# matter-labs/era-zkevm_test_harness

Measured on AMD Instinct MI355X. Metric: base-layer circuits/sec (2^20 rows); full-block synth wall-time 1/8 GPU, higher is better.
Workload: dtype u64 (Goldilocks, p = 2^64 - 2^32 + 1)

## Files before the change

### era_zkevm_test_harness_amd/csrc/ram_circuit_kernels.cuh

```cuda
#pragma once
#include "../../include/zkw_ram_circuit_spec.h"
#include "../../include/zkw_decommit_sorter_circuit_spec.h"
#include "../../include/zkw_events_sorter_circuit_spec.h"
#include "ram_kernels.cuh"
#include "public_input_kernels.cuh"
#include "closed_form_kernels.cuh"

namespace zkw {

struct SynthJob {
    const zkw_ram_instance* inst;
    const zkw_mem_query* sorted_q;
    const zkw_mem_query* unsorted_q;
    const u64* unsorted_caps;
    const u64* sorted_caps;
    const u64* u_mark;
    const u64* s_mark;
    const u64* challenges;
    const u64* gp_ckpt;
    u64* trace;
    u32* hist;
    u32* nd_tiles;
    const u64* public_input;
    const zkw_ram_instance* first_inst;
    u32 tail_clean;
};

constexpr int ROW_SLOTS[RC_NUM_ROW_TYPES] = RC_ROW_NUM_SLOTS_INIT;
constexpr int ROW_LOOKUPS[RC_NUM_ROW_TYPES] = RC_ROW_NUM_LOOKUPS_INIT;
static_assert(ROW_SLOTS[RC_ROW_PU] == 133 && ROW_SLOTS[RC_ROW_PS] == 130, "Poseidon2 rows: 130 gate variables (+3 spare in PU)");
static_assert(ROW_LOOKUPS[RC_ROW_PU] == 12 && ROW_LOOKUPS[RC_ROW_PS] == 12 && ROW_LOOKUPS[RC_ROW_A] == 12 &&
              ROW_LOOKUPS[RC_ROW_B] == 12 && ROW_LOOKUPS[RC_ROW_C] == 8 && ROW_LOOKUPS[RC_ROW_D] == 0,
              "lookup cells per cycle (56) are hard-wired in the fill kernels");
constexpr int LOOKUPS_PER_CYCLE = 56;

__device__ __forceinline__ u64 inv_or_zero(u64 x) { return gl::canon(x) ? gl::inv(x) : 0; }

struct RegsIn {
    const u64* uh;
    const u64* sh;
    u32 len;
};
__device__ __forceinline__ RegsIn regs_in(const zkw_ram_instance* in) {
    RegsIn r;
    const bool start = in->start_flag != 0;
    r.uh = start ? in->unsorted_queue_initial_state.head : in->hidden_fsm_input.current_unsorted_queue_state.head;
    r.sh = start ? in->sorted_queue_initial_state.head : in->hidden_fsm_input.current_sorted_queue_state.head;
    r.len = start ? in->unsorted_queue_initial_state.length : in->hidden_fsm_input.current_unsorted_queue_state.length;
    return r;
}

#define TR(col, row) trace[(size_t)(col) * n_rows + (row)]

__device__ __forceinline__ void zero_gap_row(u64* trace, size_t n_rows, size_t row) {
    for (int col = 0; col < RC_G + RC_L; col++) TR(col, row) = 0;
}
__device__ __forceinline__ void zero_gap_row_n(u64* trace, size_t n_rows, size_t row, int n_cols) {
    for (int col = 0; col < n_cols; col++) TR(col, row) = 0;
}

__device__ __forceinline__ void hist_bytes(u32* sh_hist, u32 x) {
    atomicAdd(&sh_hist[x & 0xFF], 1u);
    atomicAdd(&sh_hist[(x >> 8) & 0xFF], 1u);
    atomicAdd(&sh_hist[(x >> 16) & 0xFF], 1u);
    atomicAdd(&sh_hist[x >> 24], 1u);
}
__device__ __forceinline__ void put_bytes(u64* trace, size_t n_rows, size_t row, int col0, u32 x) {
    TR(col0, row) = x & 0xFF;
    TR(col0 + 1, row) = (x >> 8) & 0xFF;
    TR(col0 + 2, row) = (x >> 16) & 0xFF;
    TR(col0 + 3, row) = x >> 24;
}
__device__ __forceinline__ void hist_flush(u32* sh_hist, u32* g_hist) {
    __syncthreads();
    for (int t = threadIdx.x; t < 256; t += blockDim.x)
        if (sh_hist[t]) atomicAdd(&g_hist[t], sh_hist[t]);
}

__device__ __forceinline__ void fill_flattened_poseidon(u64* trace, size_t n_rows, size_t row, u64 s[12]) {
    int pos = 0;
#pragma unroll
    for (int k = 0; k < 12; k++) TR(pos++, row) = gl::canon(s[k]);
    p2::external(s);
    int r = 0;
    for (int k = 0; k < P2_HALF_FULL_ROUNDS; k++, r++) {
        p2::full_round(s, r);
#pragma unroll
        for (int j = 0; j < 12; j++) TR(pos + j, row) = gl::canon(s[j]);
        pos += 12;
    }
    for (int k = 0; k < P2_PARTIAL_ROUNDS; k++, r++) {
        s[0] = gl::pow7(gl::add_canon(s[0], p2::rc_at(12 * r)));
        TR(pos++, row) = gl::canon(s[0]);
        p2::internal(s);
    }
    for (int k = 0; k < P2_HALF_FULL_ROUNDS; k++, r++) {
        p2::full_round(s, r);
#pragma unroll
        for (int j = 0; j < 12; j++) TR(pos + j, row) = gl::canon(s[j]);
        pos += 12;
    }
}

struct CycleCtx {
    bool can_pop;
    zkw_mem_query q, pq;
    u64 es[8];
    u64 p_val[5];
    u32 p_ptr;
};

__device__ __forceinline__ void load_query(const zkw_mem_query* src, zkw_mem_query& dst) {
    const uint4* s = reinterpret_cast<const uint4*>(src);
    uint4* d = reinterpret_cast<uint4*>(&dst);
    d[0] = s[0]; d[1] = s[1]; d[2] = s[2];
}

__device__ __forceinline__ void cycle_ctx(const SynthJob& job, u32 i, CycleCtx& c) {
    const zkw_ram_instance* in = job.inst;
    const size_t first = in->first_item, m = in->num_items;
    c.can_pop = i < m;
    memset(&c.q, 0, sizeof c.q);
    memset(&c.pq, 0, sizeof c.pq);
#pragma unroll
    for (int k = 0; k < 8; k++) c.es[k] = 0;
    if (c.can_pop) {
        load_query(job.sorted_q + first + i, c.q);
        encode_mem_query(c.q, c.es);
    }
    if (i == 0) {
        const zkw_ram_fsm& f = in->hidden_fsm_input;
        c.pq.timestamp = f.previous_sorting_key[0]; c.pq.index = f.previous_sorting_key[1]; c.pq.page = f.previous_sorting_key[2];
        for (int k = 0; k < 8; k++) c.pq.value[k] = f.previous_value[k];
        c.pq.value_is_pointer = f.previous_is_ptr ? 1 : 0;
    } else if (i - 1 < m) {
        load_query(job.sorted_q + first + i - 1, c.pq);
    }
    u64 pe[8];
    encode_mem_query(c.pq, pe);
#pragma unroll
    for (int k = 0; k < 5; k++) c.p_val[k] = pe[3 + k];
    c.p_ptr = c.pq.value_is_pointer ? 1 : 0;
}

__device__ __forceinline__ void acc_before_pair(u64 fl, u64 fr, u64 ckpt_l, u64 ckpt_r, int lane, u64& pl, u64& pr) {
#pragma unroll
    for (int d = 1; d < 64; d <<= 1) {
        const u64 ol = __shfl_up(fl, d, 64), orr = __shfl_up(fr, d, 64);
        if (lane >= d) { fl = gl::mul(fl, ol); fr = gl::mul(fr, orr); }
        __builtin_amdgcn_sched_barrier(0);
    }
    const u64 el = __shfl_up(fl, 1, 64), er = __shfl_up(fr, 1, 64);
    pl = lane == 0 ? ckpt_l : gl::canon(gl::mul(ckpt_l, el));
    pr = lane == 0 ? ckpt_r : gl::canon(gl::mul(ckpt_r, er));
    __builtin_amdgcn_sched_barrier(0);
}

__device__ __forceinline__ void fill_row_A(const SynthJob& job, u32 i, u32 capacity, size_t n_rows, const zkw_mem_query& q,
                                           const u64 eu[8], const u64 es[8], u32* sh_hist) {
    u64* trace = job.trace;
    const size_t row = (size_t)RC_ROW_A * RC_REGION_STRIDE(capacity) + i;
    const bool live = i < capacity;
    const bool can_pop = live && i < job.inst->num_items;
    const int lane = threadIdx.x & 63;
    const u64* ckpt = job.gp_ckpt + 4 * (size_t)((u32)__builtin_amdgcn_readfirstlane((int)i) >> 6);
    if (live) {
#pragma unroll
        for (int k = 0; k < 8; k++) { TR(RC_A_eu0 + k, row) = eu[k]; TR(RC_A_ts + k, row) = es[k]; }
    }
    for (int r = 0; r < 2; r++) {
        const u64* ch = job.challenges + 9 * r;
        u64 lc = ch[8], rc = ch[8];
#pragma unroll
        for (int k = 0; k < 8; k++) {
            lc = gl::add(lc, gl::mul(eu[k], ch[k]));
            rc = gl::add(rc, gl::mul(es[k], ch[k]));
            __builtin_amdgcn_sched_barrier(0);
        }
        u64 pl, pr;
        acc_before_pair(can_pop ? lc : 1, can_pop ? rc : 1, ckpt[r], ckpt[2 + r], lane, pl, pr);
        if (live) {
            const u64 nl = gl::canon(gl::mul(pl, lc)), nr = gl::canon(gl::mul(pr, rc));
            const int o = r * (RC_A_lc1 - RC_A_lc0);
#pragma unroll
            for (int k = 1; k < 9; k++) TR(RC_A_G_c0_1 + (k - 1) + r * (RC_A_G_c1_1 - RC_A_G_c0_1), row) = ch[k];
            __builtin_amdgcn_sched_barrier(0);
            TR(RC_A_lc0 + o, row) = gl::canon(lc); TR(RC_A_P_lhs0 + o, row) = pl; TR(RC_A_nl0 + o, row) = nl;
            TR(RC_A_lhs0 + o, row) = can_pop ? nl : pl;
            TR(RC_A_rc0 + o, row) = gl::canon(rc); TR(RC_A_P_rhs0 + o, row) = pr; TR(RC_A_nr0 + o, row) = nr;
            TR(RC_A_rhs0 + o, row) = can_pop ? nr : pr;
        }
        __builtin_amdgcn_sched_barrier(0);
    }
    if (live) {
        const u64 rw = q.rw_flag ? 1 : 0, ptr = q.value_is_pointer ? 1 : 0;
        TR(RC_A_rw, row) = rw; TR(RC_A_ptr, row) = ptr; TR(RC_A_idx, row) = q.index;
        TR(RC_A_v2, row) = q.value[2]; TR(RC_A_v3, row) = q.value[3]; TR(RC_A_v0, row) = q.value[0];
        TR(RC_A_v5_b3c, row) = q.value[5] >> 24; TR(RC_A_can_pop, row) = can_pop ? 1 : 0;
        put_bytes(trace, n_rows, row, RC_A_v2_b0, q.value[2]);
        put_bytes(trace, n_rows, row, RC_A_v3_b0, q.value[3]);
        put_bytes(trace, n_rows, row, RC_A_v5_b0, q.value[5]);
        hist_bytes(sh_hist, q.value[2]); hist_bytes(sh_hist, q.value[3]); hist_bytes(sh_hist, q.value[5]);
        constexpr int NA = ROW_SLOTS[RC_ROW_A];
        if (!job.tail_clean) {
            for (int col = NA; col < RC_G; col++) TR(col, row) = 0;
            for (int col = RC_G + 12; col < RC_G + RC_L; col++) TR(col, row) = 0;
        }
    } else if (i < RC_REGION_STRIDE(capacity)) {
        if (!job.tail_clean) zero_gap_row(trace, n_rows, row);
    }
}

__device__ __forceinline__ void fill_row_B(const SynthJob& job, u32 i, u32 capacity, size_t n_rows, const zkw_mem_query& q,
                                           const u64 es[8], u32* sh_hist) {
    u64* trace = job.trace;
    const size_t row = (size_t)RC_ROW_B * RC_REGION_STRIDE(capacity) + i;
    if (i < capacity) {
        const zkw_ram_instance* in = job.inst;
        u32 p_ts = 0;
        if (i == 0) p_ts = in->hidden_fsm_input.previous_sorting_key[0];
        else if (i - 1 < in->num_items) p_ts = job.sorted_q[in->first_item + i - 1].timestamp;
        put_bytes(trace, n_rows, row, RC_B_v6_b0, q.value[6]);
        put_bytes(trace, n_rows, row, RC_B_v7_b0, q.value[7]);
        TR(RC_B_es4, row) = es[4]; TR(RC_B_v1, row) = q.value[1]; TR(RC_B_v5_b3c, row) = q.value[5] >> 24;
        TR(RC_B_es5, row) = es[5]; TR(RC_B_v2, row) = q.value[2];
        TR(RC_B_es6, row) = es[6]; TR(RC_B_v3, row) = q.value[3];
        const u32 d0 = q.timestamp - p_ts;
        TR(RC_B_d0, row) = d0; put_bytes(trace, n_rows, row, RC_B_d0_b0, d0);
        TR(RC_B_bw0, row) = q.timestamp < p_ts ? 1 : 0;
        TR(RC_B_ts, row) = q.timestamp; TR(RC_B_P_ts, row) = p_ts;
        hist_bytes(sh_hist, q.value[6]); hist_bytes(sh_hist, q.value[7]); hist_bytes(sh_hist, d0);
        constexpr int NB = ROW_SLOTS[RC_ROW_B];
        if (!job.tail_clean) {
            for (int col = NB; col < RC_G; col++) TR(col, row) = 0;
            for (int col = RC_G + 12; col < RC_G + RC_L; col++) TR(col, row) = 0;
        }
    } else if (i < RC_REGION_STRIDE(capacity)) {
        if (!job.tail_clean) zero_gap_row(trace, n_rows, row);
    }
}

template <int SIDE>
static __device__ __forceinline__ void k_ram_fill_poseidon(const VB& vb, const SynthJob* __restrict__ jobs, u32 capacity,
                                                          size_t n_rows) {
    __shared__ u32 sh_hist[256];
    for (int t = threadIdx.x; t < 256; t += blockDim.x) sh_hist[t] = 0;
    __syncthreads();
    const SynthJob job = jobs[vb.y];
    const u32 i = vb.x * blockDim.x + threadIdx.x;
    u64* trace = job.trace;
    const zkw_ram_instance* in = job.inst;
    const size_t first = in->first_item, m = in->num_items;
    const bool can_pop = i < capacity && i < m;
    const size_t row = (size_t)(SIDE == 0 ? RC_ROW_PU : RC_ROW_PS) * RC_REGION_STRIDE(capacity) + i;
    zkw_mem_query q;
    memset(&q, 0, sizeof q);
    u64 s[12];
#pragma unroll
    for (int k = 0; k < 8; k++) s[k] = 0;
    if (can_pop) {
        load_query(job.sorted_q + first + i, q);
        if (SIDE == 0) encode_raw_query(load_raw_query(job.unsorted_q + first + i), s); else encode_mem_query(q, s);
    }
    if (SIDE == 0) {
        u64 es[8];
        encode_mem_query(q, es);
        fill_row_A(job, i, capacity, n_rows, q, s, es, sh_hist);
    } else {
        fill_row_B(job, i, capacity, n_rows, q, s, sh_hist);
    }
    if (i < capacity) {
        if (SIDE == 0) {
            TR(RC_PU_idx, row) = q.index; TR(RC_PU_v0, row) = q.value[0]; TR(RC_PU_v1, row) = q.value[1];
            put_bytes(trace, n_rows, row, RC_PU_idx_b0, q.index);
            put_bytes(trace, n_rows, row, RC_PU_v0_b0, q.value[0]);
            put_bytes(trace, n_rows, row, RC_PU_v1_b0, q.value[1]);
            hist_bytes(sh_hist, q.index); hist_bytes(sh_hist, q.value[0]); hist_bytes(sh_hist, q.value[1]);
        } else {
            if (!job.tail_clean) for (int c = 130; c < RC_G; c++) TR(c, row) = 0;
            put_bytes(trace, n_rows, row, RC_PS_ts_b0, q.timestamp);
            put_bytes(trace, n_rows, row, RC_PS_page_b0, q.page);
            put_bytes(trace, n_rows, row, RC_PS_v4_b0, q.value[4]);
            hist_bytes(sh_hist, q.timestamp); hist_bytes(sh_hist, q.page); hist_bytes(sh_hist, q.value[4]);
        }
        if (!job.tail_clean) for (int c = RC_G + 12; c < RC_G + RC_L; c++) TR(c, row) = 0;
        __builtin_amdgcn_sched_barrier(0);
        const RegsIn ri = regs_in(in);
        const u64* caps = SIDE == 0 ? job.unsorted_caps : job.sorted_caps;
        const u64* prev_cap = i == 0 ? (SIDE == 0 ? ri.uh : ri.sh) + 8 : caps + 4 * (first + (i - 1 < m ? i - 1 : m - 1));
#pragma unroll
        for (int k = 0; k < 4; k++) s[8 + k] = prev_cap[k];
        fill_flattened_poseidon(trace, n_rows, row, s);
    } else if (i < RC_REGION_STRIDE(capacity)) {
        if (!job.tail_clean) zero_gap_row(trace, n_rows, row);
    }
    hist_flush(sh_hist, job.hist);
}

__device__ __forceinline__ bool nd_flag(bool can_pop, const zkw_mem_query& q) {
    return can_pop && q.timestamp == 0 && q.page == RC_HEAP_PAGE && q.rw_flag && !q.value_is_pointer;
}

static __device__ __forceinline__ void k_ram_nd_tiles(const VB& vb, const SynthJob* __restrict__ jobs, u32 capacity) {
    __shared__ u32 sh[4];
    const SynthJob job = jobs[vb.y];
    const u32 i = vb.x * blockDim.x + threadIdx.x;
    const zkw_ram_instance* in = job.inst;
    bool f = false;
    if (i < capacity && i < in->num_items) {
        zkw_mem_query q;
        load_query(job.sorted_q + in->first_item + i, q);
        f = nd_flag(true, q);
    }
    u32 cnt = __popcll(__ballot(f));
    if ((threadIdx.x & 63) == 0) sh[threadIdx.x >> 6] = cnt;
    __syncthreads();
    if (threadIdx.x == 0) job.nd_tiles[vb.x] = sh[0] + sh[1] + sh[2] + sh[3];
}
static __device__ __forceinline__ void k_ram_nd_scan(const VB& vb, const SynthJob* __restrict__ jobs, int n_jobs, u32 n_tiles) {
    u32* t = jobs[vb.x].nd_tiles;
    const int lane = threadIdx.x;
    u32 acc = 0;
    for (u32 base = 0; base < n_tiles; base += 64) {
        const u32 k = base + lane;
        const u32 v = k < n_tiles ? t[k] : 0;
        u32 incl = v;
        for (int off = 1; off < 64; off <<= 1) {
            const u32 up = __shfl_up(incl, off);
            if (lane >= off) incl += up;
        }
        if (k < n_tiles) t[k] = acc + incl - v;
        acc += __shfl(incl, 63);
    }
}

static __device__ __forceinline__ void k_ram_fill_C(const VB& vb, const SynthJob* __restrict__ jobs, u32 capacity, size_t n_rows) {
    __shared__ u32 sh_hist[256];
    __shared__ u32 sh_wave[4];
    sh_hist[threadIdx.x] = 0;
    __syncthreads();
    const SynthJob job = jobs[vb.y];
    const u32 i = vb.x * blockDim.x + threadIdx.x;
    const bool live = i < capacity;
    CycleCtx c;
    c.can_pop = false;
    bool nd = false;
    if (live) {
        cycle_ctx(job, i, c);
        nd = nd_flag(c.can_pop, c.q);
    }
    const unsigned long long bal = __ballot(nd);
    const int lane = threadIdx.x & 63, wave = threadIdx.x >> 6;
    if (lane == 0) sh_wave[wave] = __popcll(bal);
    __syncthreads();
    u32 before = __popcll(bal & ((1ull << lane) - 1));
    for (int w = 0; w < wave; w++) before += sh_wave[w];
    if (live) {
        u64* trace = job.trace;
        const zkw_ram_instance* in = job.inst;
        const size_t row = (size_t)RC_ROW_C * RC_REGION_STRIDE(capacity) + i;
        const u64 rw = c.q.rw_flag ? 1 : 0, ptr = c.q.value_is_pointer ? 1 : 0;
        const u64 bw0 = c.q.timestamp < c.pq.timestamp ? 1 : 0;
        const u64 t1 = (u64)c.pq.index + bw0, bw1 = (u64)c.q.index < t1 ? 1 : 0;
        const u32 d1 = (u32)((u64)c.q.index - t1);
        const u64 t2 = (u64)c.pq.page + bw1, bw2 = (u64)c.q.page < t2 ? 1 : 0;
        const u32 d2 = (u32)((u64)c.q.page - t2);
        TR(RC_C_d1, row) = d1; put_bytes(trace, n_rows, row, RC_C_d1_b0, d1);
        TR(RC_C_d2, row) = d2; put_bytes(trace, n_rows, row, RC_C_d2_b0, d2);
        hist_bytes(sh_hist, d1); hist_bytes(sh_hist, d2);
        TR(RC_C_bw1, row) = bw1; TR(RC_C_bw2, row) = bw2; TR(RC_C_bw0, row) = bw0;
        TR(RC_C_idx, row) = c.q.index; TR(RC_C_P_idx, row) = c.pq.index;
        TR(RC_C_page, row) = c.q.page; TR(RC_C_P_page, row) = c.pq.page;
        TR(RC_C_can_pop, row) = c.can_pop ? 1 : 0;
        u64 x[14];
        x[0] = gl::canon(gl::sub(c.q.index, c.pq.index));
        x[1] = gl::canon(gl::sub(c.q.page, c.pq.page));
        const u64 val[5] = {c.es[3], c.es[4], c.es[5], c.es[6], c.es[7]};
#pragma unroll
        for (int k = 0; k < 5; k++) { x[2 + k] = gl::canon(gl::sub(val[k], c.p_val[k])); x[7 + k] = val[k]; }
        x[12] = c.q.timestamp;
        x[13] = gl::canon(gl::sub(c.q.page, RC_HEAP_PAGE));
        u64 pre[14], acc = 1;
#pragma unroll
        for (int k = 0; k < 14; k++) { pre[k] = acc; acc = gl::mul(acc, x[k] ? x[k] : 1); }
        u64 inv = gl::inv(acc), w[14];
#pragma unroll
        for (int k = 13; k >= 0; k--) {
            w[k] = x[k] ? gl::canon(gl::mul(inv, pre[k])) : 0;
            inv = gl::mul(inv, x[k] ? x[k] : 1);
        }
        const u64 z_idx = x[0] == 0, z_page = x[1] == 0, same = z_idx & z_page;
        TR(RC_C_w_idx, row) = w[0]; TR(RC_C_z_idx, row) = z_idx;
        TR(RC_C_w_page, row) = w[1]; TR(RC_C_z_page, row) = z_page; TR(RC_C_same, row) = same;
        const int C_VAL[5] = {RC_C_es3, RC_C_es4, RC_C_es5, RC_C_es6, RC_C_v4};
        const int C_PVAL[5] = {RC_C_P_es3, RC_C_P_es4, RC_C_P_es5, RC_C_P_es6, RC_C_P_v4};
        const int C_WEQ[5] = {RC_C_w_eq0, RC_C_w_eq1, RC_C_w_eq2, RC_C_w_eq3, RC_C_w_eq4};
        const int C_ZEQ[5] = {RC_C_z_eq0, RC_C_z_eq1, RC_C_z_eq2, RC_C_z_eq3, RC_C_z_eq4};
        const int C_WZ[5] = {RC_C_w_z0, RC_C_w_z1, RC_C_w_z2, RC_C_w_z3, RC_C_w_z4};
        const int C_ZZ[5] = {RC_C_z_z0, RC_C_z_z1, RC_C_z_z2, RC_C_z_z3, RC_C_z_z4};
        u64 zeq[5], zz[5];
#pragma unroll
        for (int k = 0; k < 5; k++) {
            zeq[k] = x[2 + k] == 0; zz[k] = x[7 + k] == 0;
            TR(C_VAL[k], row) = val[k]; TR(C_PVAL[k], row) = c.p_val[k];
            TR(C_WEQ[k], row) = w[2 + k]; TR(C_ZEQ[k], row) = zeq[k];
            TR(C_WZ[k], row) = w[7 + k]; TR(C_ZZ[k], row) = zz[k];
        }
        const u64 peq = ptr == c.p_ptr, eq_a = zeq[0] & zeq[1] & zeq[2], value_equal = eq_a & zeq[3] & zeq[4] & peq;
        const u64 zz_a = zz[0] & zz[1] & zz[2], all_zero = zz_a & zz[3] & zz[4] & (1 - ptr);
        TR(RC_C_ptr, row) = ptr; TR(RC_C_P_ptr, row) = c.p_ptr; TR(RC_C_peq, row) = peq;
        TR(RC_C_eq_a, row) = eq_a; TR(RC_C_value_equal, row) = value_equal;
        TR(RC_C_zz_a, row) = zz_a; TR(RC_C_all_zero, row) = all_zero; TR(RC_C_rw, row) = rw;
        TR(RC_C_ts, row) = c.q.timestamp; TR(RC_C_w_ts, row) = w[12]; TR(RC_C_z_ts, row) = x[12] == 0;
        TR(RC_C_w_heap, row) = w[13]; TR(RC_C_z_heap, row) = x[13] == 0; TR(RC_C_nd, row) = nd ? 1 : 0;
        const u64 p_cnt = (u64)in->hidden_fsm_input.num_nondeterministic_writes + job.nd_tiles[vb.x] + before;
        TR(RC_C_P_cnt, row) = p_cnt; TR(RC_C_cnt, row) = p_cnt + (nd ? 1 : 0);
        constexpr int NC = ROW_SLOTS[RC_ROW_C];
        if (!job.tail_clean) {
            for (int col = NC; col < RC_G; col++) TR(col, row) = 0;
            for (int col = RC_G + 8; col < RC_G + RC_L; col++) TR(col, row) = 0;
        }
    } else if (i < RC_REGION_STRIDE(capacity)) {
        if (!job.tail_clean) zero_gap_row(job.trace, n_rows, (size_t)RC_ROW_C * RC_REGION_STRIDE(capacity) + i);
    }
    if (vb.x == 0 && threadIdx.x == 0)
        for (int l = 5; l < 8; l++) { hist_bytes(sh_hist, job.inst->hidden_fsm_input.previous_value[l]); hist_bytes(sh_hist, job.inst->hidden_fsm_output.previous_value[l]); }
    hist_flush(sh_hist, job.hist);
}

__device__ __forceinline__ void ram_boundary_block(const SynthJob& job, u32 capacity, size_t n_rows);
constexpr int RC_D_TILES = 4;
static __device__ __forceinline__ void k_ram_fill_D(const VB& vb, const SynthJob* __restrict__ jobs, u32 n_jobs, u32 n_tiles, u32 capacity, size_t n_rows) {
    if (vb.x < n_jobs) {
        __builtin_amdgcn_s_setprio(3);
        ram_boundary_block(jobs[vb.x], capacity, n_rows);
        return;
    }
    const SynthJob& job = jobs[(vb.x - n_jobs) / n_tiles];
    const u32 i0 = ((vb.x - n_jobs) % n_tiles) * (RC_D_TILES * 256) + threadIdx.x;
    const size_t rs = RC_REGION_STRIDE(capacity);
    u64* trace = job.trace;
    const zkw_ram_instance* in = job.inst;
    const size_t m = in->num_items;
    const RegsIn ri = regs_in(in);
    u64 len[RC_D_TILES], pre[RC_D_TILES], w[RC_D_TILES];
    u64 acc = 1;
#pragma unroll
    for (int k = 0; k < RC_D_TILES; k++) {
        const u32 i = i0 + 256 * k;
        len[k] = (u64)ri.len - (i < m ? i : m);
        pre[k] = acc;
        acc = gl::mul(acc, len[k] ? len[k] : 1);
    }
    acc = gl::inv(acc);
#pragma unroll
    for (int k = RC_D_TILES - 1; k >= 0; k--) {
        w[k] = len[k] ? gl::canon(gl::mul(acc, pre[k])) : 0;
        acc = gl::mul(acc, len[k] ? len[k] : 1);
    }
#pragma unroll
    for (int k = 0; k < RC_D_TILES; k++) {
        const u32 i = i0 + 256 * k;
        if (i >= capacity) {
            if (i < rs && !job.tail_clean) zero_gap_row(job.trace, n_rows, (size_t)RC_ROW_D * rs + i);
            continue;
        }
        const size_t row = (size_t)RC_ROW_D * rs + i;
        const size_t rPU = (size_t)RC_ROW_PU * rs + i, rPS = (size_t)RC_ROW_PS * rs + i;
        const bool can_pop = i < m;
        const u64 p_len = len[k];
        const u64 w_len = w[k], z_len = p_len == 0;
        TR(RC_D_P_len_u, row) = p_len; TR(RC_D_w_lu, row) = w_len; TR(RC_D_z_lu, row) = z_len;
        TR(RC_D_P_len_s, row) = p_len; TR(RC_D_w_ls, row) = w_len; TR(RC_D_z_ls, row) = z_len;
        TR(RC_D_can_pop, row) = can_pop ? 1 : 0;
        TR(RC_D_len_u, row) = p_len - (can_pop ? 1 : 0); TR(RC_D_len_s, row) = p_len - (can_pop ? 1 : 0);
        const size_t p = i - 1 < m ? i - 1 : m - 1, rPUp = (size_t)RC_ROW_PU * rs + p, rPSp = (size_t)RC_ROW_PS * rs + p;
#pragma unroll
        for (int e = 0; e < 12; e++) {
            const u64 uo = TR(RC_PU_uo0 + e, rPU);
            const u64 so = TR(RC_PS_so0 + e, rPS);
            const u64 a = i == 0 ? ri.uh[e] : TR(RC_PU_uo0 + e, rPUp), b = i == 0 ? ri.sh[e] : TR(RC_PS_so0 + e, rPSp);
            const int o = 3 * e;
            TR(RC_D_uo0 + o, row) = uo; TR(RC_D_P_uh0 + o, row) = a; TR(RC_D_uh0 + o, row) = can_pop ? uo : a;
            TR(RC_D_so0 + o, row) = so; TR(RC_D_P_sh0 + o, row) = b; TR(RC_D_sh0 + o, row) = can_pop ? so : b;
        }
        constexpr int ND = ROW_SLOTS[RC_ROW_D];
        if (!job.tail_clean) for (int col = ND; col < RC_G + RC_L; col++) TR(col, row) = 0;
    }
}

constexpr int TAIL_CHUNKS = 8;
constexpr int RC_BOUNDARY_ROWS = RC_NUM_ROW_TYPES - RC_ROWS_PER_CYCLE;
constexpr int RC_CF_LOOKUP_CELLS = 24;
static_assert(RC_BOUNDARY_ROWS % 2 == 0, "the tail's 16-byte stores start below the boundary rows");
static __device__ __forceinline__ void k_ram_fill_tail(const VB& vb, const SynthJob* __restrict__ jobs, u32 capacity, size_t n_rows) {
    constexpr u32 PER_JOB = (RC_G + RC_L + 1) * TAIL_CHUNKS;
    const u32 bid = vb.x % PER_JOB;
    const SynthJob& job = jobs[vb.x / PER_JOB];
    u64* trace = job.trace;
    const int col = bid / TAIL_CHUNKS, ch = bid % TAIL_CHUNKS;
    if (col < RC_G + RC_L) {
        if (job.tail_clean) return;
        const size_t bnd = (size_t)RC_BOUNDARY_ROW(capacity) + RC_BOUNDARY_ROWS;
        const size_t n_pairs = (n_rows - bnd) / 2;
        const size_t per = (n_pairs + TAIL_CHUNKS - 1) / TAIL_CHUNKS, lo = ch * per, hi = lo + per < n_pairs ? lo + per : n_pairs;
        ulonglong2* c2 = reinterpret_cast<ulonglong2*>(trace + (size_t)col * n_rows + bnd);
        const ulonglong2 z = make_ulonglong2(0, 0);
        for (size_t k = lo + threadIdx.x; k < hi; k += 256) c2[k] = z;
        return;
    }
    u64* m = trace + (size_t)RC_MULT_COL * n_rows;
    const size_t per = (n_rows + TAIL_CHUNKS - 1) / TAIL_CHUNKS, lo = ch * per, hi = lo + per < n_rows ? lo + per : n_rows;
    for (size_t r = lo + threadIdx.x; r < (job.tail_clean && hi > 256 ? (lo < 256 ? 256 : lo) : hi); r += 256) {
        u64 v = 0;
        if (r < 256) {
            v = job.hist[r];
            if (r == 0) v += (u64)RC_L * n_rows - (u64)LOOKUPS_PER_CYCLE * capacity - RC_CF_LOOKUP_CELLS;
        }
        m[r] = v;
    }
}

static __constant__ rc_link c_links[RC_NUM_LINKS] = RC_LINKS_INIT;
static __constant__ uint8_t c_is_poseidon[RC_NUM_ROW_TYPES] = RC_ROW_IS_POSEIDON_INIT;
ZKW_CF_TABLES(RC, rc)

__device__ __forceinline__ void ram_fill_register_rows(const SynthJob& job, u32 capacity, size_t n_rows) {
    u64* trace = job.trace;
    const zkw_ram_instance* in = job.inst;
    const zkw_ram_fsm& fi = in->hidden_fsm_input;
    const size_t first = in->first_item, m = in->num_items;
    const size_t bin = (size_t)RC_BOUNDARY_ROW(capacity) + RC_ROWOFF_BND_IN, bout = bin - RC_ROWOFF_BND_IN + RC_ROWOFF_BND_OUT;
    const RegsIn ri = regs_in(in);
    for (int k = 0; k < 12; k++) { TR(RC_BND_IN_uh0 + k, bin) = ri.uh[k]; TR(RC_BND_IN_sh0 + k, bin) = ri.sh[k]; }
    TR(RC_BND_IN_len_u, bin) = ri.len; TR(RC_BND_IN_len_s, bin) = ri.len;
    for (int r = 0; r < 2; r++) { TR(RC_BND_IN_lhs0 + r, bin) = fi.lhs_accumulator[r]; TR(RC_BND_IN_rhs0 + r, bin) = fi.rhs_accumulator[r]; }
    zkw_mem_query pq;
    memset(&pq, 0, sizeof pq);
    for (int k = 0; k < 8; k++) pq.value[k] = fi.previous_value[k];
    u64 pe[8];
    encode_mem_query(pq, pe);
    TR(RC_BND_IN_ts, bin) = fi.previous_sorting_key[0]; TR(RC_BND_IN_idx, bin) = fi.previous_sorting_key[1];
    TR(RC_BND_IN_page, bin) = fi.previous_sorting_key[2];
    TR(RC_BND_IN_es3, bin) = pe[3]; TR(RC_BND_IN_es4, bin) = pe[4]; TR(RC_BND_IN_es5, bin) = pe[5];
    TR(RC_BND_IN_es6, bin) = pe[6]; TR(RC_BND_IN_v4, bin) = pe[7];
    TR(RC_BND_IN_ptr, bin) = fi.previous_is_ptr ? 1 : 0; TR(RC_BND_IN_cnt, bin) = fi.num_nondeterministic_writes;
    for (int r = 0; r < 2; r++)
        for (int k = 1; k < 9; k++) TR(RC_BND_IN_G_c0_1 + 8 * r + (k - 1), bin) = job.challenges[9 * r + k];
    const size_t last = first + m - 1;
    const bool padded = m < capacity;
    const u64 len_out = (u64)ri.len - m;
    for (int k = 0; k < 12; k++) {
        TR(RC_BND_OUT_uh0 + k, bout) = job.u_mark[k];
        TR(RC_BND_OUT_sh0 + k, bout) = job.s_mark[k];
        TR(RC_BND_OUT_tail_u0 + k, bout) = in->unsorted_queue_initial_state.tail[k];
        TR(RC_BND_OUT_tail_s0 + k, bout) = in->sorted_queue_initial_state.tail[k];
    }
    TR(RC_BND_OUT_len_u, bout) = len_out; TR(RC_BND_OUT_len_s, bout) = len_out;
    for (int r = 0; r < 2; r++) {
        TR(RC_BND_OUT_lhs0 + r, bout) = in->hidden_fsm_output.lhs_accumulator[r];
        TR(RC_BND_OUT_rhs0 + r, bout) = in->hidden_fsm_output.rhs_accumulator[r];
    }
    zkw_mem_query lq;
    memset(&lq, 0, sizeof lq);
    if (!padded) lq = job.sorted_q[last];
    u64 le[8];
    encode_mem_query(lq, le);
    TR(RC_BND_OUT_ts, bout) = lq.timestamp; TR(RC_BND_OUT_idx, bout) = lq.index; TR(RC_BND_OUT_page, bout) = lq.page;
    TR(RC_BND_OUT_es3, bout) = le[3]; TR(RC_BND_OUT_es4, bout) = le[4]; TR(RC_BND_OUT_es5, bout) = le[5];
    TR(RC_BND_OUT_es6, bout) = le[6]; TR(RC_BND_OUT_v4, bout) = le[7];
    TR(RC_BND_OUT_ptr, bout) = lq.value_is_pointer ? 1 : 0;
    TR(RC_BND_OUT_cnt, bout) = TR(RC_C_cnt, (size_t)RC_ROW_C * RC_REGION_STRIDE(capacity) + capacity - 1);
    TR(RC_BND_OUT_completion, bout) = in->completion_flag ? 1 : 0;
    TR(RC_BND_OUT_w_end, bout) = inv_or_zero(len_out); TR(RC_BND_OUT_z_end, bout) = len_out == 0;
}

__device__ __forceinline__ void ram_value_row(u64* trace, size_t n_rows, size_t row, int v0, int b0, int e3) {
    zkw_mem_query q;
    memset(&q, 0, sizeof q);
    for (int k = 0; k < 8; k++) q.value[k] = (u32)TR(v0 + k, row);
    for (int l = 5; l < 8; l++)
        for (int k = 0; k < 4; k++) {
            const u64 b = (q.value[l] >> (8 * k)) & 0xFF;
            TR(b0 + 4 * (l - 5) + k, row) = b;
        }
    if (e3 < 0) return;
    u64 e[8];
    encode_mem_query(q, e);
    for (int k = 0; k < 4; k++) TR(e3 + k, row) = e[3 + k];
}

__device__ __forceinline__ void ram_boundary_block(const SynthJob& job, u32 capacity, size_t n_rows) {
    {
        u64* trace = job.trace;
        const size_t bnd = (size_t)RC_BOUNDARY_ROW(capacity);
        for (int k = threadIdx.x; k < (RC_G + RC_L) * RC_BOUNDARY_ROWS; k += CF_THREADS) TR(k / RC_BOUNDARY_ROWS, bnd + k % RC_BOUNDARY_ROWS) = 0;
    }
    __syncthreads();
    __shared__ u64 sh_oi[RAM_INPUT_ENC_LEN], sh_fi[RAM_FSM_ENC_LEN], sh_fo[RAM_FSM_ENC_LEN], sh_flags[2];
    if (threadIdx.x == 0) ram_fill_register_rows(job, capacity, n_rows);
    if (threadIdx.x == 64) {
        int m = put_queue12(job.first_inst->unsorted_queue_initial_state, sh_oi);
        m += put_queue12(job.first_inst->sorted_queue_initial_state, sh_oi + m);
        sh_oi[m] = job.first_inst->non_deterministic_bootloader_memory_snapshot_length;
    }
    if (threadIdx.x == 128) ram_encode_fsm(job.inst->hidden_fsm_input, sh_fi);
    if (threadIdx.x == 192) {
        ram_encode_fsm(job.inst->hidden_fsm_output, sh_fo);
        sh_flags[0] = job.inst->start_flag ? 1 : 0;
        sh_flags[1] = job.inst->completion_flag ? 1 : 0;
    }
    __syncthreads();
    const CfSpec S = ZKW_CF_SPEC(RC, rc, c_is_poseidon);
    const CfSources src = {sh_oi, sh_fi, sh_fo, sh_flags, nullptr};
    u64* trace = job.trace;
    cf_fill_block(S, trace, n_rows, (size_t)RC_BOUNDARY_ROW(capacity), src, [&](int rt, size_t row) {
        if (threadIdx.x != 0) return;
        if (rt == RC_ROW_VIN) ram_value_row(trace, n_rows, row, RC_VIN_VIN_v0, RC_VIN_VIN_v5_b0, RC_VIN_VIN_e3);
        if (rt == RC_ROW_VOUT) ram_value_row(trace, n_rows, row, RC_VOUT_VOUT_v0, RC_VOUT_VOUT_v5_b0, -1);
    });
}

static __constant__ rc_term c_terms[RC_NUM_TERMS] = RC_TERMS_INIT;
static __constant__ rc_constraint c_cons[RC_NUM_CONSTRAINTS] = RC_CONSTRAINTS_INIT;
static __constant__ uint16_t c_row_first[RC_NUM_ROW_TYPES + 1] = RC_ROW_FIRST_CONSTRAINT_INIT;
static __constant__ rc_term c_ds_terms[DS_NUM_TERMS] = DS_TERMS_INIT;
static __constant__ rc_constraint c_ds_cons[DS_NUM_CONSTRAINTS] = DS_CONSTRAINTS_INIT;
static __constant__ uint16_t c_ds_row_first[DS_NUM_ROW_TYPES + 1] = DS_ROW_FIRST_CONSTRAINT_INIT;
static __constant__ uint8_t c_ds_is_poseidon[DS_NUM_ROW_TYPES] = DS_ROW_IS_POSEIDON_INIT;
static __constant__ rc_link c_ds_links[DS_NUM_LINKS] = DS_LINKS_INIT;

struct SpecRam {
    static constexpr int G = RC_G, L = RC_L, ROWS_PER_CYCLE = RC_ROWS_PER_CYCLE, NUM_ROW_TYPES = RC_NUM_ROW_TYPES, NUM_LINKS = RC_NUM_LINKS;
    static constexpr int OFF_BIN = RC_ROWOFF_BND_IN, OFF_BOUT = RC_ROWOFF_BND_OUT;
    __device__ static const rc_term* terms() { return c_terms; }
    __device__ static const rc_constraint* cons() { return c_cons; }
    __device__ static const uint16_t* row_first() { return c_row_first; }
    __device__ static const uint8_t* is_poseidon() { return c_is_poseidon; }
    __device__ static const rc_link* links() { return c_links; }
};
ZKW_CF_TABLES(DS, ds)
struct SpecDecommitSorter {
    static constexpr int G = DS_G, L = DS_L, ROWS_PER_CYCLE = DS_ROWS_PER_CYCLE, NUM_ROW_TYPES = DS_NUM_ROW_TYPES, NUM_LINKS = DS_NUM_LINKS;
    static constexpr int OFF_BIN = DS_ROWOFF_BND_IN, OFF_BOUT = DS_ROWOFF_BND_OUT;
    __device__ static const rc_term* terms() { return c_ds_terms; }
    __device__ static const rc_constraint* cons() { return c_ds_cons; }
    __device__ static const uint16_t* row_first() { return c_ds_row_first; }
    __device__ static const uint8_t* is_poseidon() { return c_ds_is_poseidon; }
    __device__ static const rc_link* links() { return c_ds_links; }
    ZKW_CF_SPEC_MEMBERS(DS, ds)
};
static __constant__ rc_term c_es_terms[ES_NUM_TERMS] = ES_TERMS_INIT;
static __constant__ rc_constraint c_es_cons[ES_NUM_CONSTRAINTS] = ES_CONSTRAINTS_INIT;
static __constant__ uint16_t c_es_row_first[ES_NUM_ROW_TYPES + 1] = ES_ROW_FIRST_CONSTRAINT_INIT;
static __constant__ uint8_t c_es_is_poseidon[ES_NUM_ROW_TYPES] = ES_ROW_IS_POSEIDON_INIT;
static __constant__ rc_link c_es_links[ES_NUM_LINKS] = ES_LINKS_INIT;
ZKW_CF_TABLES(ES, es)
struct SpecEventsSorter {
    static constexpr int G = ES_G, L = ES_L, ROWS_PER_CYCLE = ES_ROWS_PER_CYCLE, NUM_ROW_TYPES = ES_NUM_ROW_TYPES, NUM_LINKS = ES_NUM_LINKS;
    static constexpr int OFF_BIN = ES_ROWOFF_BND_IN, OFF_BOUT = ES_ROWOFF_BND_OUT;
    __device__ static const rc_term* terms() { return c_es_terms; }
    __device__ static const rc_constraint* cons() { return c_es_cons; }
    __device__ static const uint16_t* row_first() { return c_es_row_first; }
    __device__ static const uint8_t* is_poseidon() { return c_es_is_poseidon; }
    __device__ static const rc_link* links() { return c_es_links; }
    ZKW_CF_SPEC_MEMBERS(ES, es)
};

struct CheckResult {
    unsigned long long violations;
    unsigned long long first_bad;
};

// ... 136 lines not shown
```

### era_zkevm_test_harness_amd/csrc/ram_kernels.cuh

```cuda
#pragma once
#include "../../include/zkw_types.h"
#include "poseidon2.cuh"

namespace zkw {
using gl::u32;
using gl::u64;

__device__ __forceinline__ void encode_mem_query(const zkw_mem_query& q, u64 out[8]) {
    const u32* v = q.value;
    out[0] = q.timestamp;
    out[1] = q.page;
    out[2] = (u64)q.index | ((u64)(q.rw_flag ? 1 : 0) << 32) | ((u64)(q.value_is_pointer ? 1 : 0) << 33);
    u64 b5 = v[5], b6 = v[6], b7 = v[7];
    out[3] = (u64)v[0] | ((b5 & 0xFFFFFF) << 32);
    out[4] = (u64)v[1] | ((b5 >> 24) << 32) | ((b6 & 0xFFFF) << 40);
    out[5] = (u64)v[2] | ((b6 >> 16) << 32) | ((b7 & 0xFF) << 48);
    out[6] = (u64)v[3] | ((b7 >> 8) << 32);
    out[7] = v[4];
}

static __device__ __forceinline__ void k_encode_mem(const VB& vb, const zkw_mem_query* __restrict__ q, size_t n,
                                                    u64* __restrict__ enc) {
    size_t i = (size_t)vb.x * blockDim.x + threadIdx.x;
    size_t stride = (size_t)vb.nx * blockDim.x;
// ... 286 lines not shown
    }
    return v;
}

template <int W, int REPS>
static __device__ __forceinline__ void k_gp_local(const VB& vb, const GpSeg* __restrict__ segs,
                                                       const GpTile* __restrict__ tiles,
                                                       u64* __restrict__ tile_aggr ) {
    __shared__ u64 sh_ch[REPS][W + 1];
    __shared__ u64 sh_wave[REPS][GP_BLOCK / 64];
    const GpTile t = tiles[vb.x];
    const GpSeg seg = segs[t.seg];
    const int tid = threadIdx.x, lane = tid & 63, wave = tid >> 6;
    for (int k = tid; k < REPS * (W + 1); k += GP_BLOCK) sh_ch[k / (W + 1)][k % (W + 1)] = seg.chal[k];
    __syncthreads();
    u64 carry[REPS];
#pragma unroll
    for (int r = 0; r < REPS; r++) carry[r] = 1;
    const u64 base = (u64)t.tile * GP_TILE;
    for (int slab = 0; slab < GP_SLABS; slab++) {
        const u64 row = base + (u64)slab * GP_BLOCK + tid;
        const bool live = row < seg.n;
        u64 term[REPS];
#pragma unroll
        for (int r = 0; r < REPS; r++) term[r] = 1;
        if (live) {
            u64 e[W];
            if (W == 8 && seg.rows == nullptr) {
                u64 e8[8];
                encode_raw_query(load_raw_query(seg.mem_q + (seg.perm ? seg.perm[row] : row)), e8);
#pragma unroll
                for (int k = 0; k < (W < 8 ? W : 8); k++) e[k] = e8[k];
            } else {
                const ulonglong2* src = reinterpret_cast<const ulonglong2*>(seg.rows + row * W);
#pragma unroll
                for (int k = 0; k < W / 2; k++) { ulonglong2 w = src[k]; e[2 * k] = w.x; e[2 * k + 1] = w.y; }
            }
#pragma unroll
            for (int r = 0; r < REPS; r++) {
                u64 acc = sh_ch[r][W];
#pragma unroll
                for (int k = 0; k < W; k++) acc = gl::add(acc, gl::mul(e[k], sh_ch[r][k]));
                term[r] = acc;
            }
        }
#pragma unroll
        for (int r = 0; r < REPS; r++) {
            u64 v = wave_scan_mul(term[r], lane);
            if (lane == 63) sh_wave[r][wave] = v;
            __syncthreads();
            u64 pre = carry[r];
            for (int w = 0; w < wave; w++) pre = gl::mul(pre, sh_wave[r][w]);
            v = gl::mul(v, pre);
            if (live) seg.z[(u64)r * seg.n + row] = v;
            u64 tot = carry[r];
            for (int w = 0; w < GP_BLOCK / 64; w++) tot = gl::mul(tot, sh_wave[r][w]);
            carry[r] = tot;
            __syncthreads();
        }
    }
    if (tid == 0) {
#pragma unroll
        for (int r = 0; r < REPS; r++) tile_aggr[(u64)vb.x * REPS + r] = carry[r];
    }
}

template <int REPS>
static __device__ __forceinline__ void k_gp_tiles(const VB& vb, const GpSeg* __restrict__ segs, int n_segs, u64* __restrict__ tile_aggr) {
    int j = vb.x * blockDim.x + threadIdx.x;
    if (j >= n_segs * REPS) return;
    const GpSeg seg = segs[j / REPS];
    const int r = j % REPS;
    u64 acc = 1;
    for (u32 t = 0; t < seg.n_tiles; t++) {
        u64* p = tile_aggr + (u64)(seg.first_tile + t) * REPS + r;
        u64 v = *p;
        *p = acc;
        acc = gl::mul(acc, v);
    }
}

template <int REPS>
static __device__ __forceinline__ void k_gp_apply(const VB& vb, const GpSeg* __restrict__ segs,
                                                       const GpTile* __restrict__ tiles,
                                                       const u64* __restrict__ tile_prefix) {
    const GpTile t = tiles[vb.x];
    const GpSeg seg = segs[t.seg];
    const u64 base = (u64)t.tile * GP_TILE;
#pragma unroll
    for (int r = 0; r < REPS; r++) {
        const u64 pre = tile_prefix[(u64)vb.x * REPS + r];
        u64* z = seg.z + (u64)r * seg.n;
        for (int slab = 0; slab < GP_SLABS; slab++) {
            const u64 row = base + (u64)slab * GP_BLOCK + threadIdx.x;
            if (row < seg.n) z[row] = gl::canon(gl::mul(z[row], pre));
        }
    }
}

static __device__ __forceinline__ void k_ram_sort_keys(const VB& vb, const zkw_mem_query* __restrict__ q, size_t n, u32* __restrict__ ts,
                                u64* __restrict__ cell, u32* __restrict__ iota, const u64* __restrict__ seg_off,
                                int n_segs) {
    size_t i = (size_t)vb.x * blockDim.x + threadIdx.x;
    if (i >= n) return;
    ts[i] = q[i].timestamp;
    cell[i] = ((u64)q[i].page << 32) | q[i].index;
    iota[i] = (u32)i;
    (void)seg_off; (void)n_segs;
}

static __device__ __forceinline__ void k_gather_u32_by_u32(const VB& vb, const u32* __restrict__ src, const u32* __restrict__ idx, size_t n,
                                    u32* __restrict__ dst) {
    size_t i = (size_t)vb.x * blockDim.x + threadIdx.x;
    if (i < n) dst[i] = src[idx[i]];
}

static __device__ __forceinline__ void k_gather_u64_by_u32(const VB& vb, const u64* __restrict__ src, const u32* __restrict__ idx, size_t n,
                                    u64* __restrict__ dst) {
    size_t i = (size_t)vb.x * blockDim.x + threadIdx.x;
    if (i < n) dst[i] = src[idx[i]];
}

static __device__ __forceinline__ void k_gather_encode(const VB& vb, const zkw_mem_query* __restrict__ q,
                                                       const u32* __restrict__ perm, size_t n,
                                                       zkw_mem_query* __restrict__ sorted_q,
                                                       u64* __restrict__ sorted_enc) {
    size_t i = (size_t)vb.x * blockDim.x + threadIdx.x;
    if (i >= n) return;
    const uint4* src = reinterpret_cast<const uint4*>(q + perm[i]);
    uint4 w0 = src[0], w1 = src[1], w2 = src[2];
    uint4* dq = reinterpret_cast<uint4*>(sorted_q + i);
    dq[0] = w0; dq[1] = w1; dq[2] = w2;
    zkw_mem_query m;
    uint4* dm = reinterpret_cast<uint4*>(&m);
    dm[0] = w0; dm[1] = w1; dm[2] = w2;
    if (!sorted_enc) return;
    u64 e[8];
    encode_mem_query(m, e);
    ulonglong2* o = reinterpret_cast<ulonglong2*>(sorted_enc + 8 * i);
    o[0] = make_ulonglong2(e[0], e[1]); o[1] = make_ulonglong2(e[2], e[3]);
    o[2] = make_ulonglong2(e[4], e[5]); o[3] = make_ulonglong2(e[6], e[7]);
}

struct RamBlock {
    const zkw_mem_query* sorted_q;
    const u32* sorted_perm;
    const u64* u_marks;
    const u64* s_marks;
    const u64* lhs_z;
    const u64* rhs_z;
    zkw_ram_instance* instances;
    u32* nondet_prefix;
    u64* gp_ckpt;
    u64 n;
    u32 capacity;
    u32 num_nondet_heap_queries;
};

__device__ __forceinline__ void copy12(u64* dst, const u64* src) {
    for (int k = 0; k < 12; k++) dst[k] = src[k];
}

static __device__ __forceinline__ void k_ram_count_nondet(const VB& vb, const RamBlock* __restrict__ blocks) {
    const RamBlock b = blocks[vb.y];
    const u64 n_inst = (b.n + b.capacity - 1) / b.capacity;
    __shared__ u32 sh[4];
    for (u64 inst = vb.x; inst < n_inst; inst += vb.nx) {
        const u64 lo = inst * b.capacity, hi = lo + b.capacity < b.n ? lo + b.capacity : b.n;
        u32 cnt = 0;
        for (u64 i = lo + threadIdx.x; i < hi; i += blockDim.x) {
            const zkw_mem_query* q = b.sorted_q + b.sorted_perm[i];
            cnt += (q->rw_flag && q->timestamp == 0 && q->page == ZKW_BOOTLOADER_HEAP_PAGE) ? 1u : 0u;
        }
        for (int d = 32; d > 0; d >>= 1) cnt += __shfl_down(cnt, d, 64);
        if ((threadIdx.x & 63) == 0) sh[threadIdx.x >> 6] = cnt;
        __syncthreads();
        if (threadIdx.x == 0) b.nondet_prefix[inst] = sh[0] + sh[1] + sh[2] + sh[3];
        __syncthreads();
    }
}

static __device__ __forceinline__ void k_ram_instances(const VB& vb, const RamBlock* __restrict__ blocks) {
    const RamBlock b = blocks[vb.y];
    const u64 n_inst = (b.n + b.capacity - 1) / b.capacity;
    const u64 idx = (u64)vb.x * blockDim.x + threadIdx.x;
    if (idx >= n_inst) return;
    const u64 n = b.n, lo = idx * b.capacity, hi = lo + b.capacity < n ? lo + b.capacity : n;
    zkw_ram_instance& w = b.instances[idx];
    memset(&w, 0, sizeof w);
    w.start_flag = idx == 0;
    w.completion_flag = idx == n_inst - 1;
    w.first_item = lo;
    w.num_items = hi - lo;
    const u64* u_final = b.u_marks + 12 * (n_inst - 1);
    const u64* s_final = b.s_marks + 12 * (n_inst - 1);
    copy12(w.unsorted_queue_initial_state.tail, u_final);
    w.unsorted_queue_initial_state.length = (u32)n;
    copy12(w.sorted_queue_initial_state.tail, s_final);
    w.sorted_queue_initial_state.length = (u32)n;
    w.non_deterministic_bootloader_memory_snapshot_length = b.num_nondet_heap_queries;

    u32 nondet_before = 0;
    for (u64 k = 0; k < idx; k++) nondet_before += b.nondet_prefix[k];

    auto fill = [&](zkw_ram_fsm& f, u64 end , u32 nondet) {
        const u64 l = end - 1;
        for (int r = 0; r < 2; r++) { f.lhs_accumulator[r] = b.lhs_z[r * n + l]; f.rhs_accumulator[r] = b.rhs_z[r * n + l]; }
        copy12(f.current_unsorted_queue_state.head, b.u_marks + 12 * (l / b.capacity));
        copy12(f.current_unsorted_queue_state.tail, u_final);
        f.current_unsorted_queue_state.length = (u32)(n - end);
        copy12(f.current_sorted_queue_state.head, b.s_marks + 12 * (l / b.capacity));
        copy12(f.current_sorted_queue_state.tail, s_final);
        f.current_sorted_queue_state.length = (u32)(n - end);
        const zkw_mem_query* q = b.sorted_q + b.sorted_perm[l];
        f.previous_sorting_key[0] = q->timestamp; f.previous_sorting_key[1] = q->index; f.previous_sorting_key[2] = q->page;
        f.previous_full_key[0] = q->index; f.previous_full_key[1] = q->page;
        for (int k = 0; k < 8; k++) f.previous_value[k] = q->value[k];
        f.previous_is_ptr = q->value_is_pointer ? 1 : 0;
        f.num_nondeterministic_writes = nondet;
    };
    if (idx == 0) {
        for (int r = 0; r < 2; r++) { w.hidden_fsm_input.lhs_accumulator[r] = 1; w.hidden_fsm_input.rhs_accumulator[r] = 1; }
    } else {
        fill(w.hidden_fsm_input, lo, nondet_before);
    }
    fill(w.hidden_fsm_output, hi, nondet_before + b.nondet_prefix[idx]);
    if ((hi - lo) % b.capacity != 0) {
        zkw_ram_fsm& f = w.hidden_fsm_output;
        for (int k = 0; k < 3; k++) f.previous_sorting_key[k] = 0;
        for (int k = 0; k < 2; k++) f.previous_full_key[k] = 0;
        for (int k = 0; k < 8; k++) f.previous_value[k] = 0;
        f.previous_is_ptr = 0;
    }
}

static __device__ __forceinline__ void k_ram_gp_ckpt(const VB& vb, const RamBlock* __restrict__ blocks) {
    const RamBlock b = blocks[vb.y];
    const u64 n_inst = (b.n + b.capacity - 1) / b.capacity, groups = (b.capacity + 63) / 64;
    const u64 j = (u64)vb.x * blockDim.x + threadIdx.x;
    if (j >= n_inst * groups) return;
    const u64 idx = j / groups, g = j % groups;
    const zkw_ram_instance& in = b.instances[idx];
    const u64 first = in.first_item, m = in.num_items;
    u64* out = b.gp_ckpt + 4 * j;
    for (int r = 0; r < 2; r++) {
        const u64 at = (u64)r * b.n + first + (64 * g - 1 < m ? 64 * g - 1 : m - 1);
        out[r] = g == 0 ? in.hidden_fsm_input.lhs_accumulator[r] : b.lhs_z[at];
        out[2 + r] = g == 0 ? in.hidden_fsm_input.rhs_accumulator[r] : b.rhs_z[at];
    }
}

static __device__ __forceinline__ void k_tails_expand(const VB& vb, const u64* __restrict__ enc, const u64* __restrict__ caps,
                                                     const u64* __restrict__ offsets, int n_queues, size_t n,
                                                     u64* __restrict__ tails) {
    const size_t i = (size_t)vb.x * blockDim.x + threadIdx.x;
    if (i >= n) return;
    int lo = 0, hi = n_queues;
    while (hi - lo > 1) {
        const int mid = (lo + hi) >> 1;
        if (offsets[mid] <= i) lo = mid; else hi = mid;
    }
    u64 s[12];
#pragma unroll
    for (int k = 0; k < 8; k++) s[k] = enc[8 * i + k];
    const bool first = offsets[lo] == i;
#pragma unroll
    for (int k = 0; k < 4; k++) s[8 + k] = first ? 0 : caps[4 * (i - 1) + k];
    p2::permute(s);
#pragma unroll
    for (int k = 0; k < 12; k++) tails[12 * i + k] = gl::canon(s[k]);
}

}
```

### era_zkevm_test_harness_amd/csrc/zkw_api.hip

```cpp
#include "zkw_ctx.h"
#include "circuit_check_host.h"
#include "closed_forms_host.h"
#include "callstack_kernels.cuh"
#include "vm_kernels.cuh"
#include "radix_sort.cuh"

static thread_local std::string g_last_error;

#undef fail
int zkw_fail(int code, const char* fmt, ...) {
    char buf[512];
    va_list ap;
    va_start(ap, fmt);
    vsnprintf(buf, sizeof buf, fmt, ap);
    va_end(ap);
    g_last_error = buf;
    return code;
}

#define fail zkw_fail

struct AllocCache {
    static constexpr size_t SMALL_MAX = size_t(256) << 20;
    static constexpr int MAX_DEV = 16;
// ... 783 lines not shown
                                         uint64_t* tails) {
    uint64_t offsets[2] = {0, n};
    return zkw_queue_push_chain_full_batch(ctx, enc, offsets, 1, tail_in, tails);
}

extern "C" int zkw_fs_challenges(zkw_ctx* ctx, const uint64_t* tail_u, uint32_t len_u, const uint64_t* tail_s,
                                 uint32_t len_s, int state_w, int n_chal, uint64_t* out) {
    if (!ctx || !tail_u || !tail_s || !out) return fail(ZKW_ERR_INVALID, "zkw_fs_challenges: null argument");
    if ((state_w != 4 && state_w != 12) || n_chal < 1 || n_chal > 64)
        return fail(ZKW_ERR_INVALID, "zkw_fs_challenges: state_w must be 4 or 12, 1 <= n_chal <= 64");
    HIP_TRY(hipSetDevice(ctx->device));
    const u64 *d_u = nullptr, *d_s = nullptr;
    u64* d_out = nullptr;
    ZKW_TRY(ctx->in("fs_u", tail_u, (size_t)state_w, &d_u));
    ZKW_TRY(ctx->in("fs_s", tail_s, (size_t)state_w, &d_s));
    ZKW_TRY(ctx->out("fs_out", out, (size_t)2 * n_chal, &d_out));
    std::vector<FsJob> jobs(1);
    jobs[0] = FsJob{d_u, d_s, len_u, len_s, d_out};
    ZKW_TRY(dev_fs(ctx, jobs, state_w, n_chal));
    ZKW_TRY(ctx->finish_out(out, d_out, (size_t)2 * n_chal));
    return ctx->sync_if_host();
}

extern "C" int zkw_grand_product_chains(zkw_ctx* ctx, const uint64_t* lhs, const uint64_t* rhs, size_t n, int width,
                                        const uint64_t* challenges, int n_reps, uint64_t* lhs_z, uint64_t* rhs_z) {
    if (!ctx || !challenges || (n && (!lhs || !rhs || !lhs_z || !rhs_z)))
        return fail(ZKW_ERR_INVALID, "zkw_grand_product_chains: null argument");
    if ((width != 8 && width != 20) || (n_reps != 1 && n_reps != 2))
        return fail(ZKW_ERR_INVALID, "zkw_grand_product_chains: width must be 8 or 20, n_reps 1 or 2");
    HIP_TRY(hipSetDevice(ctx->device));
    if (n == 0) return ZKW_OK;
    const u64 *d_l = nullptr, *d_r = nullptr, *d_c = nullptr;
    u64 *d_lz = nullptr, *d_rz = nullptr;
    ZKW_TRY(ctx->in("gp_lhs", lhs, n * width, &d_l));
    ZKW_TRY(ctx->in("gp_rhs", rhs, n * width, &d_r));
    ZKW_TRY(ctx->in("gp_chal", challenges, (size_t)n_reps * (width + 1), &d_c));
    ZKW_TRY(ctx->out("gp_lz", lhs_z, n * n_reps, &d_lz));
    ZKW_TRY(ctx->out("gp_rz", rhs_z, n * n_reps, &d_rz));
    std::vector<GpSeg> segs(2);
    segs[0] = GpSeg{d_l, d_lz, d_c, n, 0, 0};
    segs[1] = GpSeg{d_r, d_rz, d_c, n, 0, 0};
    ZKW_TRY(dev_grand_products(ctx, segs, width, n_reps));
    ZKW_TRY(ctx->finish_out(lhs_z, d_lz, n * n_reps));
    ZKW_TRY(ctx->finish_out(rhs_z, d_rz, n * n_reps));
    ZKW_TRY(ctx->sync_if_host());
    if (ctx->ptr_mode == ZKW_PTR_HOST)
        for (int r = 0; r < n_reps; r++)
            if (lhs_z[(size_t)r * n + n - 1] != rhs_z[(size_t)r * n + n - 1])
                return fail(ZKW_ERR_CHECK_FAILED, "grand products differ in repetition %d (utils.rs:685-696)", r);
    return ZKW_OK;
}

extern "C" int zkw_encode_log_queries(zkw_ctx* ctx, const zkw_log_query* q, size_t n, const uint32_t* ext_ts,
                                      uint64_t* enc) {
    if (!ctx || (n && (!q || !enc))) return fail(ZKW_ERR_INVALID, "zkw_encode_log_queries: null argument");
    HIP_TRY(hipSetDevice(ctx->device));
    if (n == 0) return ZKW_OK;
    const zkw_log_query* d_q = nullptr;
    const u32* d_e = nullptr;
    u64* d_enc = nullptr;
    ZKW_TRY(ctx->in("lenc_q", q, n, &d_q));
    if (ext_ts) ZKW_TRY(ctx->in("lenc_ts", ext_ts, n, &d_e));
    ZKW_TRY(ctx->out("lenc_out", enc, n * 20, &d_enc));
    { Prof _p(ctx, "k_encode_log"); ZKW_LAUNCH(ctx, k_encode_log, blocks_for(n, 256), 256, d_q, n, d_e, d_enc); }
    ZKW_TRY(launch_check("k_encode_log"));
    ZKW_TRY(ctx->finish_out(enc, d_enc, n * 20));
    return ctx->sync_if_host();
}

extern "C" int zkw_encode_decommit_queries(zkw_ctx* ctx, const zkw_decommit_query* q, size_t n, uint64_t* enc) {
    if (!ctx || (n && (!q || !enc))) return fail(ZKW_ERR_INVALID, "zkw_encode_decommit_queries: null argument");
    HIP_TRY(hipSetDevice(ctx->device));
    if (n == 0) return ZKW_OK;
    const zkw_decommit_query* d_q = nullptr;
    u64* d_enc = nullptr;
    ZKW_TRY(ctx->in("denc_q", q, n, &d_q));
    ZKW_TRY(ctx->out("denc_out", enc, n * 8, &d_enc));
    { Prof _p(ctx, "k_encode_decommit"); ZKW_LAUNCH(ctx, k_encode_decommit, blocks_for(n, 256), 256, d_q, n, d_enc); }
    ZKW_TRY(launch_check("k_encode_decommit"));
    ZKW_TRY(ctx->finish_out(enc, d_enc, n * 8));
    return ctx->sync_if_host();
}

int dev_log_chains(zkw_ctx* ctx, const u64* d_enc, size_t total, std::vector<LogChainJob>& jobs) {
    const int key = ctx->chain_service && !ctx->batched() ? ctx->next_chain_key() : 0;
    if (total == 0 || jobs.empty()) { if (ctx->chain_service && !ctx->batched()) chain_service_of(ctx->device)->skip(key); return ZKW_OK; }
    u64* d_pre = nullptr;
    ZKW_TRY(ctx->scratch_t<u64>("log_pre", total * 4, &d_pre));
    { Prof _p(ctx, "k_log_prehash"); ZKW_LAUNCH(ctx, k_log_prehash, blocks_for(total, 128), 128, d_enc, total, d_pre); }
    ZKW_TRY(launch_check("k_log_prehash"));
    for (auto& j : jobs) j.pre = d_pre + (j.enc - d_enc) / 20 * 4;
    if (ctx->batched()) return zkw_batch_chains(ctx->batch, nullptr, 0, jobs.data(), jobs.size());
    if (ctx->chain_service) return chain_service_run(ctx, nullptr, &jobs, "k_chain_log", key);
    LogChainJob* d_jobs = nullptr;
    ZKW_TRY(ctx->upload("log_chain_jobs", jobs, &d_jobs));
    const int n_jobs = (int)jobs.size();
    { Prof _p(ctx, "k_chain_log"); hipLaunchKernelGGL(k_chain_log, dim3((n_jobs + 3) / 4), dim3(64), 0, ctx->stream, d_jobs, n_jobs); }
    return launch_check("k_chain_log");
}

extern "C" int zkw_queue_push_chain_log_batch(zkw_ctx* ctx, const uint64_t* enc, const uint64_t* offsets,
                                              size_t n_queues, const uint64_t* tails_in, uint64_t* old_tails,
                                              uint64_t* new_tails) {
    if (!ctx || !offsets) return fail(ZKW_ERR_INVALID, "zkw_queue_push_chain_log_batch: null argument");
    HIP_TRY(hipSetDevice(ctx->device));
    for (size_t k = 0; k < n_queues; k++)
        if (offsets[k + 1] < offsets[k]) return fail(ZKW_ERR_INVALID, "offsets must be non-decreasing");
    const size_t base = n_queues ? offsets[0] : 0, total = n_queues ? offsets[n_queues] - base : 0;
    if (total && (!enc || !new_tails)) return fail(ZKW_ERR_INVALID, "null enc/new_tails");
    const u64 *d_enc = nullptr, *d_tin = nullptr;
    u64 *d_old = nullptr, *d_new = nullptr;
    ZKW_TRY(ctx->in("lchain_enc", enc + base * 20, total * 20, &d_enc));
    if (tails_in) ZKW_TRY(ctx->in("lchain_tin", tails_in, n_queues * 4, &d_tin));
    if (old_tails) ZKW_TRY(ctx->out("lchain_old", old_tails + base * 4, total * 4, &d_old));
    ZKW_TRY(ctx->out("lchain_new", new_tails + base * 4, total * 4, &d_new));
    std::vector<LogChainJob> jobs(n_queues);
    for (size_t k = 0; k < n_queues; k++) {
        const size_t lo = offsets[k] - base;
        jobs[k] = LogChainJob{d_enc + lo * 20, nullptr, d_old ? d_old + lo * 4 : nullptr, d_new + lo * 4,
                              d_tin ? d_tin + 4 * k : nullptr, offsets[k + 1] - offsets[k]};
    }
    ZKW_TRY(dev_log_chains(ctx, d_enc, total, jobs));
    if (old_tails) ZKW_TRY(ctx->finish_out(old_tails + base * 4, d_old, total * 4));
    ZKW_TRY(ctx->finish_out(new_tails + base * 4, d_new, total * 4));
    return ctx->sync_if_host();
}

extern "C" int zkw_queue_push_chain_log(zkw_ctx* ctx, const uint64_t* enc, size_t n, const uint64_t tail_in[4],
                                        uint64_t* old_tails, uint64_t* new_tails) {
    uint64_t offsets[2] = {0, n};
    return zkw_queue_push_chain_log_batch(ctx, enc, offsets, 1, tail_in, old_tails, new_tails);
}

struct zkw_ram_witness {
    zkw_ctx* ctx = nullptr;
    std::vector<uint64_t> offsets;
    std::vector<uint64_t> inst_offsets;
    uint32_t capacity = 0;
    size_t total = 0, n_instances = 0;
    zkw_mem_query* sorted_q = nullptr;
    bool sorted_valid = false;
    u32* perm = nullptr;
    const zkw_mem_query* unsorted_q = nullptr;
    zkw_mem_query* owned_q = nullptr;
    u64 *unsorted_enc = nullptr, *sorted_enc = nullptr;
    bool enc_valid = false;
    u64 *unsorted_caps = nullptr, *sorted_caps = nullptr, *unsorted_marks = nullptr, *sorted_marks = nullptr;
    u64 *unsorted_tails = nullptr, *sorted_tails = nullptr;
    bool tails_valid = false;
    u64 *challenges = nullptr, *lhs_z = nullptr, *rhs_z = nullptr;
    bool z_valid = false;
    u64 *zbuf_l = nullptr, *zbuf_r = nullptr;
    u64* gp_ckpt = nullptr;
    zkw_mem_query* sq_win = nullptr;
    size_t zcap = 0, sqcap = 0;
    zkw_ram_instance* instances = nullptr;
    u32* nondet_counts = nullptr;
    u64 *compact_forms = nullptr, *public_inputs = nullptr;

    void release() {
        void* ptrs[] = {sorted_q, perm, owned_q, unsorted_enc, sorted_enc, unsorted_caps, sorted_caps, unsorted_marks, sorted_marks,
                        unsorted_tails, sorted_tails, challenges,
                        lhs_z,    rhs_z,        instances,  nondet_counts, compact_forms, public_inputs, zbuf_l, zbuf_r, sq_win, gp_ckpt};
        for (void* p : ptrs)
            if (p) dev_free(p);
        sorted_q = nullptr;
        sorted_valid = false;
        perm = nullptr;
        owned_q = nullptr;
        unsorted_q = nullptr;
        enc_valid = false;
        unsorted_enc = sorted_enc = unsorted_tails = sorted_tails = challenges = lhs_z = rhs_z = nullptr;
        unsorted_caps = sorted_caps = unsorted_marks = sorted_marks = nullptr;
        tails_valid = false;
        z_valid = false;
        zbuf_l = zbuf_r = nullptr;
        gp_ckpt = nullptr;
        sq_win = nullptr;
        zcap = sqcap = 0;
        instances = nullptr;
        nondet_counts = nullptr;
        compact_forms = public_inputs = nullptr;
    }
};

extern "C" void zkw_ram_witness_free(zkw_ram_witness* w);
static inline size_t ram_gp_groups(uint32_t capacity) { return ((size_t)capacity + 63) / 64; }
static int ram_alloc(zkw_ram_witness* w, size_t n_blocks) {
    const size_t t = w->total, ni = w->n_instances;
    HIP_TRY(dev_malloc((void**)&w->perm, (t + 1) * sizeof(u32)));
    HIP_TRY(dev_malloc((void**)&w->unsorted_caps, (t + 1) * 4 * sizeof(u64)));
    HIP_TRY(dev_malloc((void**)&w->sorted_caps, (t + 1) * 4 * sizeof(u64)));
    HIP_TRY(dev_malloc((void**)&w->unsorted_marks, (ni + 1) * 12 * sizeof(u64)));
    HIP_TRY(dev_malloc((void**)&w->sorted_marks, (ni + 1) * 12 * sizeof(u64)));
    HIP_TRY(dev_malloc((void**)&w->challenges, (n_blocks + 1) * 18 * sizeof(u64)));
    {
        size_t max_block = 0;
        for (size_t b = 0; b + 1 < w->offsets.size(); b++) max_block = std::max(max_block, (size_t)(w->offsets[b + 1] - w->offsets[b]));
        size_t window = (size_t)1 << 26, sq_window = (size_t)1 << 22;
        if (const char* e = getenv("ZKW_Z_WINDOW_ITEMS")) window = sq_window = (size_t)strtoull(e, nullptr, 10);
        w->zcap = std::max(max_block, std::min(t, window));
        w->sqcap = std::max(max_block, std::min(t, sq_window));
        HIP_TRY(dev_malloc((void**)&w->zbuf_l, (w->zcap + 1) * 2 * sizeof(u64)));
        HIP_TRY(dev_malloc((void**)&w->zbuf_r, (w->zcap + 1) * 2 * sizeof(u64)));
        HIP_TRY(dev_malloc((void**)&w->sq_win, (w->sqcap + 1) * sizeof(zkw_mem_query)));
    }
    HIP_TRY(dev_malloc((void**)&w->gp_ckpt, (ni * ram_gp_groups(w->capacity) + 1) * 4 * sizeof(u64)));
    HIP_TRY(dev_malloc((void**)&w->instances, (ni + 1) * sizeof(zkw_ram_instance)));
    HIP_TRY(dev_malloc((void**)&w->nondet_counts, (ni + 1) * sizeof(u32)));
    HIP_TRY(dev_malloc((void**)&w->compact_forms, (ni + 1) * COMPACT_FORM_LEN * sizeof(u64)));
    HIP_TRY(dev_malloc((void**)&w->public_inputs, (ni + 1) * 4 * sizeof(u64)));
    return ZKW_OK;
}

__device__ __forceinline__ u32 block_of_position(const u64* __restrict__ offsets, int n_blocks, size_t i) {
    int lo = 0, hi = n_blocks;
    while (hi - lo > 1) {
        int mid = (lo + hi) >> 1;
        if (offsets[mid] <= i) lo = mid; else hi = mid;
    }
    return (u32)lo;
}

static __device__ __forceinline__ void k_ram_key_ranges(const VB& vb, const zkw_mem_query* __restrict__ q, size_t n, u32* __restrict__ maxima) {
    u32 t = 0, p = 0, x = 0;
    for (size_t i = (size_t)vb.x * blockDim.x + threadIdx.x; i < n; i += (size_t)vb.nx * blockDim.x) {
        t = max(t, q[i].timestamp);
        p = max(p, q[i].page);
        x = max(x, q[i].index);
    }
    for (int o = 32; o > 0; o >>= 1) {
        t = max(t, (u32)__shfl_xor((int)t, o));
        p = max(p, (u32)__shfl_xor((int)p, o));
        x = max(x, (u32)__shfl_xor((int)x, o));
    }
    if ((threadIdx.x & 63) == 0) {
        atomicMax(maxima + 0, t);
        atomicMax(maxima + 1, p);
        atomicMax(maxima + 2, x);
    }
}

static __device__ __forceinline__ void k_ram_packed_keys(const VB& vb, const zkw_mem_query* __restrict__ q, size_t n, const u64* __restrict__ offsets,
                                  int n_blocks, unsigned bits_p, unsigned bits_i, unsigned bits_t,
                                  u64* __restrict__ key, u32* __restrict__ iota) {
    size_t i = (size_t)vb.x * blockDim.x + threadIdx.x;
    if (i >= n) return;
    u64 k = n_blocks > 1 ? block_of_position(offsets, n_blocks, i) : 0;
    k = (k << bits_p) | q[i].page;
    k = (k << bits_i) | q[i].index;
    k = (k << bits_t) | q[i].timestamp;
    key[i] = k;
    iota[i] = (u32)i;
}

static __device__ __forceinline__ void k_ram_packed_cells(const VB& vb, const u64* __restrict__ cell, const u32* __restrict__ perm, size_t n,
                                   const u64* __restrict__ offsets, int n_blocks, unsigned bits_p, unsigned bits_i,
                                   u64* __restrict__ key) {
    size_t i = (size_t)vb.x * blockDim.x + threadIdx.x;
    if (i >= n) return;
    const u32 src = perm[i];
    const u64 c = cell[src];
    u64 k = n_blocks > 1 ? block_of_position(offsets, n_blocks, src) : 0;
    k = (k << bits_p) | (c >> 32);
    k = (k << bits_i) | (c & 0xFFFFFFFFu);
    key[i] = k;
}

static __device__ __forceinline__ void k_block_ids(const VB& vb, const u64* __restrict__ offsets, int n_blocks, size_t n, u32* __restrict__ ids) {
    size_t i = (size_t)vb.x * blockDim.x + threadIdx.x;
    if (i < n) ids[i] = block_of_position(offsets, n_blocks, i);
}

static unsigned bits_in_use(u32 x) { return x ? 32u - (unsigned)__builtin_clz(x) : 0u; }

static int ram_sort(zkw_ctx* ctx, const zkw_mem_query* d_q, size_t total, const std::vector<uint64_t>& offsets,
                    void* work_a, void* work_b, u32** perm_out) {
    const size_t n_blocks = offsets.size() - 1;
    size_t tmp_bytes = radix_temp_bytes(total);
    u32* ts = static_cast<u32*>(work_a);
    u32 *k32 = ts + total, *v0 = k32 + total, *v1 = v0 + total;
    u64* cell = reinterpret_cast<u64*>(v1 + total);
    u64* k64a = cell + total;
    u64* k64b = static_cast<u64*>(work_b);
    void* tmp = nullptr;
    const size_t tmp_off = (total * 8 + 255) & ~(size_t)255;
    if (tmp_off + tmp_bytes <= total * 32) tmp = static_cast<char*>(work_b) + tmp_off;
    else ZKW_TRY(ctx->scratch("sort_tmp", tmp_bytes + 256, &tmp));
    const unsigned grid = blocks_for(total, 256);

    void* d_max_v = nullptr;
    ZKW_TRY(ctx->scratch("sort_max", 256, &d_max_v));
    u32* d_max = static_cast<u32*>(d_max_v);
    HIP_TRY(ctx->memset_async(d_max, 0, 16));
    { Prof _p(ctx, "k_ram_key_ranges");
      const unsigned g = grid < 4096 ? grid : 4096;
      ZKW_LAUNCH(ctx, k_ram_key_ranges, g, 256, d_q, total, d_max); }
    ZKW_TRY(launch_check("k_ram_key_ranges"));
    u32 maxima[4];
    ZKW_TRY(ctx->read_small(maxima, d_max, 16));
    const unsigned bits_t = bits_in_use(maxima[0]), bits_p = bits_in_use(maxima[1]), bits_i = bits_in_use(maxima[2]);
    unsigned bits_b = 0;
    while ((1ull << bits_b) < n_blocks) bits_b++;
    u64* d_off = nullptr;
    if (n_blocks > 1) ZKW_TRY(ctx->upload("sort_off", offsets, &d_off));

    if (bits_b + bits_p + bits_i + bits_t <= 64) {
        const unsigned bits = bits_b + bits_p + bits_i + bits_t;
        { Prof _p(ctx, "k_ram_packed_keys");
          ZKW_LAUNCH(ctx, k_ram_packed_keys, grid, 256, d_q, total, d_off, (int)n_blocks, bits_p, bits_i, bits_t, k64a, v0); }
        ZKW_TRY(launch_check("k_ram_packed_keys"));
        { Prof _p(ctx, "radix_sort"); ZKW_TRY(radix_sort_pairs<u64>(ctx, tmp, tmp_bytes, k64a, k64b, v0, v1, total, bits ? bits : 1)); }
        *perm_out = v1;
        return ZKW_OK;
    }

    { Prof _p(ctx, "k_ram_sort_keys"); ZKW_LAUNCH(ctx, k_ram_sort_keys, grid, 256, d_q, total, ts, cell, v0, (const u64*)nullptr, 0); }
    ZKW_TRY(launch_check("k_ram_sort_keys"));
    { Prof _p(ctx, "radix_sort"); ZKW_TRY(radix_sort_pairs<u32>(ctx, tmp, tmp_bytes, ts, k32, v0, v1, total, bits_t ? bits_t : 1)); }
    if (bits_b + bits_p + bits_i <= 64) {
        const unsigned bits = bits_b + bits_p + bits_i;
        { Prof _p(ctx, "k_ram_packed_cells");
          ZKW_LAUNCH(ctx, k_ram_packed_cells, grid, 256, cell, v1, total, d_off, (int)n_blocks, bits_p, bits_i, k64a); }
        ZKW_TRY(launch_check("k_ram_packed_cells"));
        { Prof _p(ctx, "radix_sort"); ZKW_TRY(radix_sort_pairs<u64>(ctx, tmp, tmp_bytes, k64a, k64b, v1, v0, total, bits ? bits : 1)); }
        *perm_out = v0;
        return ZKW_OK;
    }
    { Prof _p(ctx, "k_gather_u64_by_u32"); ZKW_LAUNCH(ctx, k_gather_u64_by_u32, grid, 256, cell, v1, total, k64a); }
    ZKW_TRY(launch_check("k_gather_u64_by_u32"));
    { Prof _p(ctx, "radix_sort"); ZKW_TRY(radix_sort_pairs<u64>(ctx, tmp, tmp_bytes, k64a, k64b, v1, v0, total, 64)); }
    { Prof _p(ctx, "k_block_ids"); ZKW_LAUNCH(ctx, k_block_ids, grid, 256, d_off, (int)n_blocks, total, ts); }
    ZKW_TRY(launch_check("k_block_ids"));
    { Prof _p(ctx, "k_gather_u32_by_u32"); ZKW_LAUNCH(ctx, k_gather_u32_by_u32, grid, 256, ts, v0, total, k32); }
    ZKW_TRY(launch_check("k_gather_u32_by_u32"));
    { Prof _p(ctx, "radix_sort"); ZKW_TRY(radix_sort_pairs<u32>(ctx, tmp, tmp_bytes, k32, ts, v0, v1, total, bits_b)); }
    *perm_out = v1;
    return ZKW_OK;
}

static int ram_gp_blocks(zkw_ctx* ctx, const zkw_ram_witness* w, size_t b0, size_t b1, u64* dst_l, u64* dst_r) {
    std::vector<GpSeg> segs;
    segs.reserve(2 * (b1 - b0));
    const size_t base = w->offsets[b0];
    for (size_t b = b0; b < b1; b++) {
        const size_t lo = w->offsets[b], n = w->offsets[b + 1] - lo;
        segs.push_back(GpSeg{nullptr, dst_l + 2 * (lo - base), w->challenges + 18 * b, n, 0, 0, w->unsorted_q + lo});
        segs.push_back(GpSeg{nullptr, dst_r + 2 * (lo - base), w->challenges + 18 * b, n, 0, 0, w->unsorted_q, w->perm + lo});
    }
    return dev_grand_products(ctx, segs, 8, 2);
}

static int ram_run(zkw_ctx* ctx, zkw_ram_witness* w, const zkw_mem_query* d_q, const uint32_t* n_nondet) {
    const size_t n_blocks = w->offsets.size() - 1, total = w->total;
    if (ctx->ptr_mode == ZKW_PTR_DEVICE) {
        w->unsorted_q = d_q;
    } else {
        if (!w->owned_q) HIP_TRY(dev_malloc((void**)&w->owned_q, (total + 1) * sizeof(zkw_mem_query)));
        HIP_TRY(ctx->copy_async(w->owned_q, d_q, total * sizeof(zkw_mem_query), hipMemcpyDeviceToDevice));
        w->unsorted_q = w->owned_q;
    }
    u32* perm = nullptr;
    ZKW_TRY(ram_sort(ctx, d_q, total, w->offsets, w->unsorted_caps, w->sorted_caps, &perm));
    w->tails_valid = false;
    w->enc_valid = false;
    w->sorted_valid = false;
    HIP_TRY(ctx->copy_async(w->perm, perm, total * sizeof(u32), hipMemcpyDeviceToDevice));
    std::vector<ChainJob> chains;
    chains.reserve(2 * n_blocks);
    for (size_t b = 0; b < n_blocks; b++) {
        const size_t lo = w->offsets[b], n = w->offsets[b + 1] - lo;
        const size_t io = w->inst_offsets[b];
        chains.push_back(ChainJob{nullptr, nullptr, nullptr, n, w->unsorted_caps + 4 * lo, w->unsorted_marks + 12 * io, w->capacity, w->unsorted_q + lo});
        chains.push_back(ChainJob{nullptr, nullptr, nullptr, n, w->sorted_caps + 4 * lo, w->sorted_marks + 12 * io, w->capacity, w->unsorted_q, w->perm + lo});
    }
    ZKW_TRY(dev_chains(ctx, chains));
    std::vector<FsJob> fs(n_blocks);
    for (size_t b = 0; b < n_blocks; b++) {
        const size_t lo = w->offsets[b], n = w->offsets[b + 1] - lo;
        const size_t last_inst = w->inst_offsets[b + 1] - 1;
        fs[b] = FsJob{w->unsorted_marks + 12 * last_inst, w->sorted_marks + 12 * last_inst, (u32)n, (u32)n,
                      w->challenges + 18 * b};
    }
    ZKW_TRY(dev_fs(ctx, fs, 12, 9));
    w->z_valid = false;
    for (size_t b0 = 0; b0 < n_blocks;) {
        size_t b1 = b0 + 1;
        while (b1 < n_blocks && w->offsets[b1 + 1] - w->offsets[b0] <= w->zcap) b1++;
        ZKW_TRY(ram_gp_blocks(ctx, w, b0, b1, w->zbuf_l, w->zbuf_r));
        const size_t base = w->offsets[b0];
        std::vector<RamBlock> blocks(b1 - b0);
        size_t max_inst = 0;
        for (size_t b = b0; b < b1; b++) {
            const size_t lo = w->offsets[b], n = w->offsets[b + 1] - lo;
            const size_t n_inst = w->inst_offsets[b + 1] - w->inst_offsets[b];
            if (n_inst > max_inst) max_inst = n_inst;
            blocks[b - b0] = RamBlock{w->unsorted_q,
                                      w->perm + lo,
                                      w->unsorted_marks + 12 * w->inst_offsets[b],
                                      w->sorted_marks + 12 * w->inst_offsets[b],
                                      w->zbuf_l + 2 * (lo - base),
                                      w->zbuf_r + 2 * (lo - base),
                                      w->instances + w->inst_offsets[b],
                                      w->nondet_counts + w->inst_offsets[b],
                                      w->gp_ckpt + 4 * ram_gp_groups(w->capacity) * w->inst_offsets[b],
                                      n,
                                      w->capacity,
                                      n_nondet ? n_nondet[b] : 0u};
        }
        RamBlock* d_blocks = nullptr;
        ZKW_TRY(ctx->upload("ram_blocks", blocks, &d_blocks));
        const unsigned gx = (unsigned)(max_inst < 64 ? max_inst : 64), gy = (unsigned)(b1 - b0);
        { Prof _p(ctx, "k_ram_count_nondet"); ZKW_LAUNCH_2D(ctx, k_ram_count_nondet, gx, gy, 256, d_blocks); }
        ZKW_TRY(launch_check("k_ram_count_nondet"));
        { Prof _p(ctx, "k_ram_instances"); ZKW_LAUNCH_2D(ctx, k_ram_instances, blocks_for(max_inst, 64), gy, 64, d_blocks); }
        ZKW_TRY(launch_check("k_ram_instances"));
        { Prof _p(ctx, "k_ram_gp_ckpt"); ZKW_LAUNCH_2D(ctx, k_ram_gp_ckpt, blocks_for(max_inst * ram_gp_groups(w->capacity), 256), gy, 256, d_blocks); }
        ZKW_TRY(launch_check("k_ram_gp_ckpt"));
        b0 = b1;
    }
    const size_t ni = w->n_instances;
    { Prof _p(ctx, "k_ram_commitments"); ZKW_LAUNCH(ctx, k_ram_commitments, blocks_for(4 * ni, 64), 64, w->instances, ni, w->compact_forms); }
    ZKW_TRY(launch_check("k_ram_commitments"));
    { Prof _p(ctx, "k_commit_encodings"); ZKW_LAUNCH(ctx, k_commit_encodings, blocks_for(ni, 64), 64, w->compact_forms, ni, (u32)COMPACT_FORM_LEN, w->public_inputs); }
    return launch_check("k_commit_encodings");
}

extern "C" int zkw_ram_build_instances_batch(zkw_ctx* ctx, const zkw_mem_query* q, const uint64_t* block_offsets,
                                             size_t n_blocks, uint32_t capacity, const uint32_t* n_nondet,
                                             zkw_ram_witness** out) {
    if (!ctx || !q || !block_offsets || !out || n_blocks == 0 || capacity == 0)
        return fail(ZKW_ERR_INVALID, "zkw_ram_build_instances_batch: bad argument");
    HIP_TRY(hipSetDevice(ctx->device));
    const uint64_t base = block_offsets[0];
    std::vector<uint64_t> offs(n_blocks + 1), ioffs(n_blocks + 1, 0);
    for (size_t b = 0; b <= n_blocks; b++) offs[b] = block_offsets[b] - base;
    for (size_t b = 0; b < n_blocks; b++) {
        if (block_offsets[b + 1] <= block_offsets[b])
            return fail(ZKW_ERR_INVALID, "block %zu is empty: the VM must have made memory requests "
                                         "(W/ram_permutation.rs:43-46)", b);
        ioffs[b + 1] = ioffs[b] + (offs[b + 1] - offs[b] + capacity - 1) / capacity;
    }
    const size_t total = offs[n_blocks];
    if (total >= (1ull << 32)) return fail(ZKW_ERR_INVALID, "more than 2^32-1 queries in one batch");
    zkw_ram_witness* w = *out;
    if (w && (w->ctx != ctx || w->offsets != offs || w->capacity != capacity)) {
        zkw_ram_witness_free(w);
        w = nullptr;
        *out = nullptr;
    }
    if (!w) {
        w = new zkw_ram_witness();
        w->ctx = ctx;
        w->offsets = offs;
        w->inst_offsets = ioffs;
        w->capacity = capacity;
        w->total = total;
        w->n_instances = ioffs[n_blocks];
        int rc = ram_alloc(w, n_blocks);
        if (rc != ZKW_OK) {
            w->release();
            delete w;
            return rc;
        }
    }
    const zkw_mem_query* d_q = nullptr;
    int rc = ctx->in("ram_q", q + base, total, &d_q);
    if (rc == ZKW_OK) rc = ram_run(ctx, w, d_q, n_nondet);
    if (rc == ZKW_OK) rc = ctx->sync_if_host();
    if (rc != ZKW_OK) {
        if (!*out) {
            w->release();
            delete w;
        }
        return rc;
    }
    if (!*out) ctx_retain(ctx);
    *out = w;
    return ZKW_OK;
}

extern "C" int zkw_ram_build_instances(zkw_ctx* ctx, const zkw_mem_query* q, size_t n, uint32_t capacity,
                                       uint32_t num_non_deterministic_heap_queries, zkw_ram_witness** out) {
    uint64_t offsets[2] = {0, n};
    return zkw_ram_build_instances_batch(ctx, q, offsets, 1, capacity, &num_non_deterministic_heap_queries, out);
}

extern "C" size_t zkw_ram_witness_num_instances(const zkw_ram_witness* w) { return w ? w->n_instances : 0; }
extern "C" size_t zkw_ram_witness_num_items(const zkw_ram_witness* w) { return w ? w->total : 0; }

static int ram_sorted_queries(const zkw_ram_witness* cw) {
    zkw_ram_witness* w = const_cast<zkw_ram_witness*>(cw);
    if (w->sorted_valid) return ZKW_OK;
    zkw_ctx* ctx = w->ctx;
    HIP_TRY(hipSetDevice(ctx->device));
    const size_t t = w->total;
    if (!w->sorted_q && dev_malloc((void**)&w->sorted_q, (t + 1) * sizeof(zkw_mem_query)) != hipSuccess)
        return fail(ZKW_ERR_OOM, "no room for the sorted queries (%zu bytes): read ZKW_RAM_SORTED_QUERIES from a smaller batch", t * sizeof(zkw_mem_query));
    { Prof _p(ctx, "k_gather_encode"); ZKW_LAUNCH(ctx, k_gather_encode, blocks_for(t, 256), 256, w->unsorted_q, w->perm, t, w->sorted_q, (u64*)nullptr); }
    ZKW_TRY(launch_check("k_gather_encode"));
    w->sorted_valid = true;
    return ZKW_OK;
}

static int ram_full_chains(const zkw_ram_witness* cw) {
    zkw_ram_witness* w = const_cast<zkw_ram_witness*>(cw);
    if (w->z_valid) return ZKW_OK;
    zkw_ctx* ctx = w->ctx;
    HIP_TRY(hipSetDevice(ctx->device));
    const size_t t = w->total;
    if (!w->lhs_z) {
        if (dev_malloc((void**)&w->lhs_z, (t + 1) * 16) != hipSuccess || dev_malloc((void**)&w->rhs_z, (t + 1) * 16) != hipSuccess)
            return fail(ZKW_ERR_OOM, "no room for the grand-product chains (%zu bytes): read ZKW_RAM_*_Z from a smaller batch", 2 * t * 16);
    }
    ZKW_TRY(ram_gp_blocks(ctx, w, 0, w->offsets.size() - 1, w->lhs_z, w->rhs_z));
    w->z_valid = true;
    return ZKW_OK;
}

static int ram_encodings(const zkw_ram_witness* cw) {
    zkw_ram_witness* w = const_cast<zkw_ram_witness*>(cw);
    if (w->enc_valid) return ZKW_OK;
    zkw_ctx* ctx = w->ctx;
    HIP_TRY(hipSetDevice(ctx->device));
    const size_t t = w->total;
    if (!w->unsorted_enc) {
        if (dev_malloc((void**)&w->unsorted_enc, (t + 1) * 64) != hipSuccess || dev_malloc((void**)&w->sorted_enc, (t + 1) * 64) != hipSuccess)
            return fail(ZKW_ERR_OOM, "no room for the materialised encodings (%zu bytes): read ZKW_RAM_*_ENC from a smaller batch", 2 * t * 64);
    }
    ZKW_TRY(ram_sorted_queries(cw));
    ZKW_TRY(dev_encode(ctx, w->unsorted_q, t, w->unsorted_enc));
    ZKW_TRY(dev_encode(ctx, w->sorted_q, t, w->sorted_enc));
    w->enc_valid = true;
    return ZKW_OK;
}

static int ram_full_tails(const zkw_ram_witness* cw) {
    zkw_ram_witness* w = const_cast<zkw_ram_witness*>(cw);
    if (w->tails_valid) return ZKW_OK;
    ZKW_TRY(ram_encodings(cw));
    zkw_ctx* ctx = w->ctx;
    HIP_TRY(hipSetDevice(ctx->device));
    const size_t t = w->total;
    if (!w->unsorted_tails) {
        if (dev_malloc((void**)&w->unsorted_tails, (t + 1) * 96) != hipSuccess || dev_malloc((void**)&w->sorted_tails, (t + 1) * 96) != hipSuccess)
            return fail(ZKW_ERR_OOM, "no room for the expanded queue tails (%zu bytes): read ZKW_RAM_*_TAILS from a smaller batch", 2 * t * 96);
    }
    u64* d_off = nullptr;
    ZKW_TRY(ctx->upload("tails_off", w->offsets, &d_off));
    const int nq = (int)(w->offsets.size() - 1);
    { Prof _p(ctx, "k_tails_expand"); ZKW_LAUNCH(ctx, k_tails_expand, blocks_for(t, 64), 64, w->unsorted_enc, w->unsorted_caps, d_off, nq, t, w->unsorted_tails); }
    ZKW_TRY(launch_check("k_tails_expand"));
    { Prof _p(ctx, "k_tails_expand"); ZKW_LAUNCH(ctx, k_tails_expand, blocks_for(t, 64), 64, w->sorted_enc, w->sorted_caps, d_off, nq, t, w->sorted_tails); }
    ZKW_TRY(launch_check("k_tails_expand"));
    w->tails_valid = true;
    return ZKW_OK;
}

static const void* ram_array(const zkw_ram_witness* w, int what, size_t* bytes, bool materialize = true, int* rc = nullptr) {
    const size_t t = w->total, nb = w->offsets.size() - 1;
    int st = ZKW_OK;
    const void* p = nullptr;
#define RAM_LAZY(fn, field) do { if (materialize) { st = fn(w); if (st == ZKW_OK) p = w->field; } } while (0)
    switch (what) {
        case ZKW_RAM_SORTED_QUERIES: *bytes = t * sizeof(zkw_mem_query); RAM_LAZY(ram_sorted_queries, sorted_q); break;
        case ZKW_RAM_UNSORTED_ENC: *bytes = t * 64; RAM_LAZY(ram_encodings, unsorted_enc); break;
        case ZKW_RAM_SORTED_ENC: *bytes = t * 64; RAM_LAZY(ram_encodings, sorted_enc); break;
        case ZKW_RAM_UNSORTED_TAILS: *bytes = t * 96; RAM_LAZY(ram_full_tails, unsorted_tails); break;
        case ZKW_RAM_SORTED_TAILS: *bytes = t * 96; RAM_LAZY(ram_full_tails, sorted_tails); break;
        case ZKW_RAM_CHALLENGES: *bytes = nb * 18 * 8; p = w->challenges; break;
        case ZKW_RAM_LHS_Z: *bytes = t * 16; RAM_LAZY(ram_full_chains, lhs_z); break;
        case ZKW_RAM_RHS_Z: *bytes = t * 16; RAM_LAZY(ram_full_chains, rhs_z); break;
        case ZKW_RAM_INSTANCES: *bytes = w->n_instances * sizeof(zkw_ram_instance); p = w->instances; break;
        case ZKW_RAM_COMPACT_FORMS: *bytes = w->n_instances * COMPACT_FORM_LEN * 8; p = w->compact_forms; break;
        case ZKW_RAM_PUBLIC_INPUTS: *bytes = w->n_instances * 32; p = w->public_inputs; break;
        case ZKW_RAM_GP_CKPT: *bytes = w->n_instances * ram_gp_groups(w->capacity) * 32; p = w->gp_ckpt; break;
        default: *bytes = 0; st = ZKW_ERR_INVALID; break;
    }
#undef RAM_LAZY
    if (rc) *rc = st;
    return p;
}

extern "C" size_t zkw_ram_witness_bytes(const zkw_ram_witness* w, int what) {
    size_t b = 0;
    if (w) (void)ram_array(w, what, &b, false);
    return b;
}

extern "C" const void* zkw_ram_witness_device_ptr(const zkw_ram_witness* w, int what) {
    size_t b = 0;
    return w ? ram_array(w, what, &b) : nullptr;
}

extern "C" int zkw_ram_witness_get(const zkw_ram_witness* w, int what, void* dst, size_t dst_bytes) {
    if (!w || !dst) return fail(ZKW_ERR_INVALID, "zkw_ram_witness_get: null argument");
    size_t bytes = 0;
    int st = ZKW_OK;
    const void* src = ram_array(w, what, &bytes, true, &st);
    if (st == ZKW_ERR_INVALID) return fail(ZKW_ERR_INVALID, "zkw_ram_witness_get: unknown array %d", what);
    if (st != ZKW_OK) return st;
    if (!src) return fail(ZKW_ERR_INVALID, "zkw_ram_witness_get: array %d is empty", what);
    if (dst_bytes < bytes) return fail(ZKW_ERR_INVALID, "zkw_ram_witness_get: need %zu bytes, got %zu", bytes, dst_bytes);
    zkw_ctx* ctx = w->ctx;
    HIP_TRY(hipSetDevice(ctx->device));
    HIP_TRY(ctx->copy_async(dst, src, bytes, ctx->ptr_mode == ZKW_PTR_DEVICE ? hipMemcpyDeviceToDevice : hipMemcpyDeviceToHost));
    return ctx->sync_if_host();
}

extern "C" void zkw_ram_witness_free(zkw_ram_witness* w) {
    if (!w) return;
    (void)hipSetDevice(w->ctx->device);
    (void)hipStreamSynchronize(w->ctx->stream);
    w->release();
    zkw_ctx* owner = w->ctx;
    delete w;
    ctx_release(owner);
}


extern "C" int zkw_trace_create_with_columns(zkw_ctx* ctx, size_t n_rows, size_t n_cols, size_t n_slots, zkw_trace** out) {
    if (!ctx || !out || n_rows < 256 || n_slots == 0 || n_cols == 0 || n_cols > 4096)
        return fail(ZKW_ERR_INVALID, "zkw_trace_create: bad argument");
    HIP_TRY(hipSetDevice(ctx->device));
    zkw_trace* t = new zkw_trace();
    t->ctx = ctx;
    t->n_rows = n_rows;
    t->n_cols = n_cols;
    t->n_slots = n_slots;
    t->slot_tag.reset(new std::atomic<uint64_t>[n_slots]);
    for (size_t k = 0; k < n_slots; k++) t->slot_tag[k].store(0, std::memory_order_relaxed);
    hipError_t e = dev_malloc((void**)&t->data, t->slot_elems() * n_slots * sizeof(u64));
    if (e != hipSuccess) {
        delete t;
        return fail(ZKW_ERR_OOM, "zkw_trace_create: hipMalloc of %zu bytes failed: %s",
                    n_cols * n_rows * n_slots * 8, hipGetErrorString(e));
    }
    ctx_retain(ctx);
    *out = t;
    return ZKW_OK;
}

extern "C" int zkw_trace_create(zkw_ctx* ctx, size_t n_rows, size_t n_slots, zkw_trace** out) {
    return zkw_trace_create_with_columns(ctx, n_rows, RC_COLS, n_slots, out);
}

extern "C" void zkw_trace_free(zkw_trace* t) {
    if (!t) return;
    (void)hipSetDevice(t->ctx->device);
    (void)hipStreamSynchronize(t->ctx->stream);
    if (t->data) dev_free(t->data);
    zkw_ctx* owner = t->ctx;
    delete t;
    ctx_release(owner);
}

extern "C" size_t zkw_trace_num_rows(const zkw_trace* t) { return t ? t->n_rows : 0; }
extern "C" size_t zkw_trace_num_cols(const zkw_trace* t) { return t ? t->n_cols : 0; }
extern "C" size_t zkw_trace_num_slots(const zkw_trace* t) { return t ? t->n_slots : 0; }
extern "C" const uint64_t* zkw_trace_device_ptr(const zkw_trace* t, size_t slot) {
    if (!t || slot >= t->n_slots) return nullptr;
    return t->slot_for_write(slot, 0);
}

extern "C" int zkw_trace_get(const zkw_trace* t, size_t slot, uint32_t first_col, uint32_t n_cols, uint64_t* dst) {
    if (!t || !dst || slot >= t->n_slots || (size_t)first_col + n_cols > t->n_cols) return fail(ZKW_ERR_INVALID, "zkw_trace_get: bad argument");
    zkw_ctx* ctx = t->ctx;
    HIP_TRY(hipSetDevice(ctx->device));
    const u64* src = t->data + slot * t->slot_elems() + (size_t)first_col * t->n_rows;
    HIP_TRY(ctx->copy_async(dst, src, (size_t)n_cols * t->n_rows * sizeof(u64), ctx->ptr_mode == ZKW_PTR_DEVICE ? hipMemcpyDeviceToDevice : hipMemcpyDeviceToHost));
    return ctx->sync_if_host();
}

extern "C" int zkw_ram_synthesize(zkw_ctx* ctx, const zkw_ram_witness* w, size_t first_instance, size_t n_instances,
                                  zkw_trace* t, size_t first_slot) {
    if (!ctx || !w || !t || w->ctx != ctx || t->ctx->device != ctx->device) return fail(ZKW_ERR_INVALID, "zkw_ram_synthesize: bad argument");
    if (first_instance + n_instances > w->n_instances) return fail(ZKW_ERR_INVALID, "instance range out of bounds");
    if (n_instances > t->n_slots) return fail(ZKW_ERR_INVALID, "more instances (%zu) than trace slots (%zu)", n_instances, t->n_slots);
    const u32 capacity = w->capacity;
    const size_t n_rows = t->n_rows;
    if (RC_MIN_ROWS(capacity) > n_rows)
        return fail(ZKW_ERR_INVALID, "capacity %u needs %llu rows, trace has %zu", capacity,
                    (unsigned long long)RC_MIN_ROWS(capacity), n_rows);
    if (n_rows & 1) return fail(ZKW_ERR_INVALID, "trace length must be even (it is a power of two in every circuit)");
    if (n_instances == 0) return ZKW_OK;
    HIP_TRY(hipSetDevice(ctx->device));
    const size_t n_blocks = w->offsets.size() - 1;
    size_t b_first = 0;
    while (b_first + 1 < n_blocks && w->inst_offsets[b_first + 1] <= first_instance) b_first++;
    size_t b_end = b_first + 1;
    while (b_end < n_blocks && w->inst_offsets[b_end] < first_instance + n_instances) b_end++;
    const size_t win = w->sqcap;
    if (w->offsets[b_end] - w->offsets[b_first] > win) {
        size_t b_mid = b_first + 1;
        while (b_mid + 1 < b_end && w->offsets[b_mid + 1] - w->offsets[b_first] <= win) b_mid++;
        const size_t n_head = w->inst_offsets[b_mid] - first_instance;
        ZKW_TRY(zkw_ram_synthesize(ctx, w, first_instance, n_head, t, first_slot));
        return zkw_ram_synthesize(ctx, w, first_instance + n_head, n_instances - n_head, t, first_slot + n_head);
    }
    const size_t z_base = w->offsets[b_first];
    {
        const size_t cnt = w->offsets[b_end] - z_base;
        Prof _p(ctx, "k_gather_encode");
        ZKW_LAUNCH(ctx, k_gather_encode, blocks_for(cnt, 256), 256, w->unsorted_q, w->perm + z_base, cnt, w->sq_win, (u64*)nullptr);
    }
    ZKW_TRY(launch_check("k_gather_encode"));
    const u32 rstride = (u32)RC_REGION_STRIDE(capacity);
    const u32 n_tiles = (rstride + 255) / 256;
    u32 *d_hist = nullptr, *d_nd = nullptr;
    ZKW_TRY(ctx->scratch_t<u32>("synth_hist", n_instances * 256, &d_hist));
    ZKW_TRY(ctx->scratch_t<u32>("synth_nd", n_instances * n_tiles, &d_nd));
    HIP_TRY(ctx->memset_async(d_hist, 0, n_instances * 256 * sizeof(u32)));
    SlotClaims claims(t);
    std::vector<SynthJob> jobs(n_instances);
    size_t b = b_first;
    for (size_t k = 0; k < n_instances; k++) {
        const size_t idx = first_instance + k;
        while (b + 1 < n_blocks && w->inst_offsets[b + 1] <= idx) b++;
        const size_t lo = w->offsets[b];
        SynthJob& j = jobs[k];
        j.inst = w->instances + idx;
        j.sorted_q = w->sq_win + (lo - z_base);
        j.unsorted_q = w->unsorted_q + lo;
        j.unsorted_caps = w->unsorted_caps + 4 * lo;
        j.sorted_caps = w->sorted_caps + 4 * lo;
        j.u_mark = w->unsorted_marks + 12 * idx;
        j.s_mark = w->sorted_marks + 12 * idx;
        j.challenges = w->challenges + 18 * b;
        j.gp_ckpt = w->gp_ckpt + 4 * ram_gp_groups(capacity) * idx;
        {
            const uint64_t tag = ((uint64_t)ZKW_CIRCUIT_RAM_PERMUTATION << 56) ^ ((uint64_t)capacity << 24) ^ (uint64_t)n_rows ^ 0x5A00000000000000ull;
            const size_t slot = (first_slot + k) % t->n_slots;
            bool clean = false;
            j.trace = claims.claim(slot, tag, &clean);
            j.tail_clean = clean;
        }
        j.hist = d_hist + 256 * k;
        j.nd_tiles = d_nd + (size_t)n_tiles * k;
        j.public_input = w->public_inputs + 4 * idx;
        j.first_inst = w->instances + w->inst_offsets[b];
    }
    SynthJob* d_jobs = nullptr;
    ZKW_TRY(ctx->upload("synth_jobs", jobs, &d_jobs));
    const unsigned nj = (unsigned)n_instances;
    const dim3 g64((rstride + 63) / 64, nj), g256(n_tiles, nj);
    { Prof _p(ctx, "k_ram_nd_tiles"); ZKW_LAUNCH_D(ctx, (k_ram_nd_tiles), "k_ram_nd_tiles", g256, 256, 0, d_jobs, capacity); }
    ZKW_TRY(launch_check("k_ram_nd_tiles"));
    { Prof _p(ctx, "k_ram_nd_scan"); ZKW_LAUNCH(ctx, k_ram_nd_scan, nj, 64, d_jobs, (int)nj, n_tiles); }
    ZKW_TRY(launch_check("k_ram_nd_scan"));
    { Prof _p(ctx, "k_ram_fill_poseidon"); ZKW_LAUNCH_D(ctx, (k_ram_fill_poseidon<0>), "k_ram_fill_poseidon", g64, 64, 0, d_jobs, capacity, n_rows); }
    ZKW_TRY(launch_check("k_ram_fill_poseidon<0>"));
    { Prof _p(ctx, "k_ram_fill_poseidon"); ZKW_LAUNCH_D(ctx, (k_ram_fill_poseidon<1>), "k_ram_fill_poseidon", g64, 64, 0, d_jobs, capacity, n_rows); }
    ZKW_TRY(launch_check("k_ram_fill_poseidon<1>"));
    { Prof _p(ctx, "k_ram_fill_C"); ZKW_LAUNCH_D(ctx, (k_ram_fill_C), "k_ram_fill_C", g256, 256, 0, d_jobs, capacity, n_rows); }
    ZKW_TRY(launch_check("k_ram_fill_C"));
    { Prof _p(ctx, "k_ram_fill_D"); const unsigned d_tiles = (unsigned)((rstride + RC_D_TILES * 256 - 1) / (RC_D_TILES * 256));
      ZKW_LAUNCH(ctx, k_ram_fill_D, nj * (d_tiles + 1), 256, d_jobs, nj, d_tiles, capacity, n_rows); }
    ZKW_TRY(launch_check("k_ram_fill_D"));
    { Prof _p(ctx, "k_ram_fill_tail"); ZKW_LAUNCH(ctx, k_ram_fill_tail, nj * ((RC_G + RC_L + 1) * TAIL_CHUNKS), 256, d_jobs, capacity, n_rows); }
    ZKW_TRY(launch_check("k_ram_fill_tail"));
    return claims.commit_if(ctx->sync_if_host());
}


extern "C" int zkw_ram_check_satisfied(zkw_ctx* ctx, const zkw_trace* t, size_t slot, uint32_t capacity,
                                       uint64_t* n_violations, uint64_t* first_bad) {
    if (!ctx || !t || t->ctx->device != ctx->device || slot >= t->n_slots || !n_violations)
        return fail(ZKW_ERR_INVALID, "zkw_ram_check_satisfied: bad argument");
    if (RC_MIN_ROWS(capacity) > t->n_rows) return fail(ZKW_ERR_INVALID, "capacity does not fit the trace");
    return check_satisfied<SpecRam>(ctx, t, slot, capacity, n_violations, first_bad);
}

extern "C" int zkw_decommit_sorter_check_satisfied(zkw_ctx* ctx, const zkw_trace* t, size_t slot, uint32_t capacity,
                                                   uint64_t* n_violations, uint64_t* first_bad) {
    if (!ctx || !t || t->ctx->device != ctx->device || slot >= t->n_slots || !n_violations)
        return fail(ZKW_ERR_INVALID, "zkw_decommit_sorter_check_satisfied: bad argument");
    if (DS_MIN_ROWS(capacity) > t->n_rows) return fail(ZKW_ERR_INVALID, "capacity does not fit the trace");
    return check_satisfied<SpecDecommitSorter>(ctx, t, slot, capacity, n_violations, first_bad);
}

extern "C" int zkw_closed_form_public_inputs(zkw_ctx* ctx, uint8_t circuit_type, const void* instances, size_t n, uint64_t* compact,
                                             uint64_t* public_inputs) {
    if (!ctx || !compact || !public_inputs || (n && !instances)) return fail(ZKW_ERR_INVALID, "zkw_closed_form_public_inputs: null argument");
    if (n == 0) return ZKW_OK;
    HIP_TRY(hipSetDevice(ctx->device));
    switch (circuit_type) {
        case 3: return closed_form_from_records<CfDecommitter>(ctx, instances, n, compact, public_inputs);
        case 5: return closed_form_from_records<CfPrecompile<ZKW_PRECOMPILE_KECCAK256>>(ctx, instances, n, compact, public_inputs);
        case 6: return closed_form_from_records<CfPrecompile<ZKW_PRECOMPILE_SHA256>>(ctx, instances, n, compact, public_inputs);
        case 7: return closed_form_from_records<CfPrecompile<ZKW_PRECOMPILE_ECRECOVER>>(ctx, instances, n, compact, public_inputs);
        case 10: return closed_form_from_records<CfStorageApplication>(ctx, instances, n, compact, public_inputs);
        case 13: return closed_form_from_records<CfLinearHasher>(ctx, instances, n, compact, public_inputs);
        default: break;
    }
    return fail(ZKW_ERR_INVALID, "zkw_closed_form_public_inputs: circuit type %u keeps its compact forms in its witness (2, 4, 8, 9, 11, 12) "
                                 "or is not a base-layer circuit with a closed form here", (unsigned)circuit_type);
}

extern "C" int zkw_commit_encodings(zkw_ctx* ctx, const uint64_t* enc, size_t n_items, uint32_t item_len, uint64_t* out) {
    if (!ctx || !out || (n_items && item_len && !enc)) return fail(ZKW_ERR_INVALID, "zkw_commit_encodings: null argument");
    if (n_items == 0) return ZKW_OK;
    HIP_TRY(hipSetDevice(ctx->device));
    const u64* d_enc = nullptr;
    u64* d_out = nullptr;
    ZKW_TRY(ctx->in("ce_enc", enc, n_items * item_len + 1, &d_enc));
    ZKW_TRY(ctx->out("ce_out", out, n_items * 4, &d_out));
    { Prof _p(ctx, "k_commit_encodings"); ZKW_LAUNCH(ctx, k_commit_encodings, blocks_for(n_items, 64), 64, d_enc, n_items, item_len, d_out); }
    ZKW_TRY(launch_check("k_commit_encodings"));
    ZKW_TRY(ctx->finish_out(out, d_out, n_items * 4));
    return ctx->sync_if_host();
}

extern "C" int zkw_encode_recursion_requests(zkw_ctx* ctx, uint64_t circuit_type, const uint64_t* public_inputs, size_t n,
                                             uint64_t* enc) {
    if (!ctx || !enc || !public_inputs) return fail(ZKW_ERR_INVALID, "zkw_encode_recursion_requests: null argument");
    if (n == 0) return ZKW_OK;
    HIP_TRY(hipSetDevice(ctx->device));
    const u64* d_pi = nullptr;
    u64* d_enc = nullptr;
    ZKW_TRY(ctx->in("rr_pi", public_inputs, n * 4, &d_pi));
    ZKW_TRY(ctx->out("rr_enc", enc, n * 8, &d_enc));
    { Prof _p(ctx, "k_encode_recursion"); ZKW_LAUNCH(ctx, k_encode_recursion, blocks_for(n, 64), 64, circuit_type, d_pi, n, d_enc); }
    ZKW_TRY(launch_check("k_encode_recursion"));
    ZKW_TRY(ctx->finish_out(enc, d_enc, n * 8));
    return ctx->sync_if_host();
}

extern "C" int zkw_encode_callstack_entries(zkw_ctx* ctx, const zkw_callstack_entry* entries, size_t n, uint64_t* enc) {
    if (!ctx || !enc || !entries) return fail(ZKW_ERR_INVALID, "zkw_encode_callstack_entries: null argument");
    if (n == 0) return ZKW_OK;
    HIP_TRY(hipSetDevice(ctx->device));
    const zkw_callstack_entry* d_e = nullptr;
    u64* d_enc = nullptr;
    ZKW_TRY(ctx->in("cs_e", entries, n, &d_e));
    ZKW_TRY(ctx->out("cs_enc", enc, n * 32, &d_enc));
    { Prof _p(ctx, "k_encode_callstack"); hipLaunchKernelGGL(k_encode_callstack, dim3(blocks_for(n, 64)), dim3(64), 0, ctx->stream, d_e, n, d_enc); }
    ZKW_TRY(launch_check("k_encode_callstack"));
    ZKW_TRY(ctx->finish_out(enc, d_enc, n * 32));
    return ctx->sync_if_host();
}

extern "C" int zkw_callstack_simulate(zkw_ctx* ctx, const uint8_t* is_push, size_t n_ops, const zkw_callstack_entry* pushed,
                                      size_t n_pushed, uint64_t* previous_state, uint64_t* new_state, uint32_t* depth,
                                      uint64_t* round_states, uint32_t* entry_index) {
    if (!ctx || !is_push || !previous_state || !new_state || !depth || !round_states || !entry_index || (n_pushed && !pushed))
        return fail(ZKW_ERR_INVALID, "zkw_callstack_simulate: null argument");
    if (n_ops == 0) return ZKW_OK;
    if (n_ops >= (1ull << 31)) return fail(ZKW_ERR_INVALID, "too many stack operations");
    HIP_TRY(hipSetDevice(ctx->device));
    const uint8_t* d_ops = nullptr;
    const zkw_callstack_entry* d_e = nullptr;
    ZKW_TRY(ctx->in("st_ops", is_push, n_ops, &d_ops));
    if (n_pushed) ZKW_TRY(ctx->in("st_e", pushed, n_pushed, &d_e));
    u32 *d_depth = nullptr, *d_rank = nullptr, *d_meta = nullptr, *d_pd = nullptr, *d_pid = nullptr, *d_sd = nullptr, *d_sid = nullptr,
        *d_parent = nullptr, *d_node = nullptr;
    u64* d_rounds = nullptr;
    void* tmp = nullptr;
    const size_t tmp_bytes = radix_temp_bytes(n_ops);
    ZKW_TRY(ctx->scratch_t<u32>("st_depth", n_ops, &d_depth));
    ZKW_TRY(ctx->scratch_t<u32>("st_rank", n_ops, &d_rank));
    ZKW_TRY(ctx->scratch_t<u32>("st_meta", 4, &d_meta));
    ZKW_TRY(ctx->scratch_t<u32>("st_pd", n_ops, &d_pd));
    ZKW_TRY(ctx->scratch_t<u32>("st_pid", n_ops, &d_pid));
    ZKW_TRY(ctx->scratch_t<u32>("st_sd", n_ops, &d_sd));
    ZKW_TRY(ctx->scratch_t<u32>("st_sid", n_ops, &d_sid));
    ZKW_TRY(ctx->scratch_t<u32>("st_parent", n_ops, &d_parent));
    ZKW_TRY(ctx->scratch_t<u32>("st_node", n_ops, &d_node));
    ZKW_TRY(ctx->scratch_t<u64>("st_rounds", n_ops * 48, &d_rounds));
    ZKW_TRY(ctx->scratch("st_tmp", tmp_bytes + 256, &tmp));
    u64 *d_prefix = nullptr, *d_totals = nullptr;
    ZKW_TRY(ctx->scratch_t<u64>("st_prefix", 2 * (n_ops + 1), &d_prefix));
    ZKW_TRY(ctx->scratch_t<u64>("st_totals", 2, &d_totals));
    HIP_TRY(ctx->memset_async(d_meta, 0, 4 * sizeof(u32)));
    ZKW_TRY((sum_prefix<2>(ctx, "k_stack_prefix", StackDelta{d_ops}, n_ops, d_prefix, d_totals)));
    { Prof _p(ctx, "k_stack_depth"); hipLaunchKernelGGL(k_stack_depth, dim3(blocks_for(n_ops, 256)), dim3(256), 0, ctx->stream, d_ops, n_ops, d_prefix, d_depth, d_rank, d_meta); }
    ZKW_TRY(launch_check("k_stack_depth"));
    u32 meta[3];
    ZKW_TRY(ctx->read_small(meta, d_meta, sizeof meta));
    if (meta[2]) return fail(ZKW_ERR_INVALID, "pop from the empty callstack (circuit_encodings/src/lib.rs:619)");
    const u32 n_push = meta[0], max_depth = meta[1];
    if (n_push > n_pushed) return fail(ZKW_ERR_INVALID, "%u pushes but only %zu entries", n_push, n_pushed);
    const unsigned grid = blocks_for(n_ops, 256);
    if (n_push) {
        { Prof _p(ctx, "k_stack_push_keys"); hipLaunchKernelGGL(k_stack_push_keys, dim3(grid), dim3(256), 0, ctx->stream, d_ops, n_ops, d_depth, d_rank, d_pd, d_pid); }
        ZKW_TRY(launch_check("k_stack_push_keys"));
        unsigned bits = 1;
        while ((1ull << bits) <= max_depth) bits++;
        { Prof _p(ctx, "radix_sort"); ZKW_TRY(radix_sort_pairs<u32>(ctx, tmp, tmp_bytes, d_pd, d_sd, d_pid, d_sid, n_push, bits)); }
    }
    { Prof _p(ctx, "k_stack_links"); hipLaunchKernelGGL(k_stack_links, dim3(grid), dim3(256), 0, ctx->stream, d_ops, n_ops, d_depth, d_rank, d_sd, d_sid, d_meta, d_parent, d_node); }
    ZKW_TRY(launch_check("k_stack_links"));
    for (u32 d = 1; d <= max_depth; d++) {
        Prof _p(ctx, "k_stack_level");
        hipLaunchKernelGGL(k_stack_level, dim3(blocks_for(n_push, 64)), dim3(64), 0, ctx->stream, d_e, d_pd, d_parent, d_meta, d, d_rounds);
    }
    ZKW_TRY(launch_check("k_stack_level"));
    u64 *d_prev = nullptr, *d_new = nullptr, *d_rs = nullptr;
    u32 *d_dep = nullptr, *d_idx = nullptr;
    ZKW_TRY(ctx->out("st_o_prev", previous_state, n_ops * 12, &d_prev));
    ZKW_TRY(ctx->out("st_o_new", new_state, n_ops * 12, &d_new));
    ZKW_TRY(ctx->out("st_o_rs", round_states, n_ops * 48, &d_rs));
    ZKW_TRY(ctx->out("st_o_dep", depth, n_ops, &d_dep));
    ZKW_TRY(ctx->out("st_o_idx", entry_index, n_ops, &d_idx));
    { Prof _p(ctx, "k_stack_emit"); hipLaunchKernelGGL(k_stack_emit, dim3(grid), dim3(256), 0, ctx->stream, d_ops, n_ops, d_depth, d_parent, d_node, d_rounds, d_meta, d_prev, d_new, d_dep, d_rs, d_idx); }
    ZKW_TRY(launch_check("k_stack_emit"));
    ZKW_TRY(ctx->finish_out(previous_state, d_prev, n_ops * 12));
    ZKW_TRY(ctx->finish_out(new_state, d_new, n_ops * 12));
    ZKW_TRY(ctx->finish_out(round_states, d_rs, n_ops * 48));
    ZKW_TRY(ctx->finish_out(depth, d_dep, n_ops));
    ZKW_TRY(ctx->finish_out(entry_index, d_idx, n_ops));
    return ctx->sync_if_host();
}

// ... 63 lines not shown
```

### era_zkevm_test_harness_amd/csrc/zkw_ctx.h

```cpp
#pragma once
#include <hip/hip_runtime.h>

#include <algorithm>
#include <atomic>
#include <chrono>
#include <condition_variable>
#include <memory>
#include <mutex>
#include <thread>

#include <cstdarg>
#include <cstdio>
#include <cstdlib>
#include <cstring>
#include <map>
#include <string>
#include <vector>

#include "../../include/zkw.h"
#include "zkw_internal.h"
#include "zkw_batch.h"
#include "ram_kernels.cuh"
#include "log_kernels.cuh"
#include "../../include/zkw_ram_circuit_spec.h"

using namespace zkw;

#define fail zkw_fail

hipError_t zkw_cache_alloc(int pinned_host, void** p, size_t bytes);
void zkw_cache_release(int pinned_host, void* p);
static inline hipError_t dev_malloc(void** p, size_t bytes) { return zkw_cache_alloc(0, p, bytes); }
template <class T> static inline hipError_t dev_malloc(T** p, size_t bytes) { return zkw_cache_alloc(0, (void**)p, bytes); }
static inline void dev_free(void* p) { zkw_cache_release(0, p); }
static inline hipError_t pin_malloc(void** p, size_t bytes) { return zkw_cache_alloc(1, p, bytes); }
static inline void pin_free(void* p) { zkw_cache_release(1, p); }
hipError_t zkw_pool_stream_acquire(hipStream_t* s);
void zkw_pool_stream_release(hipStream_t s);

#define HIP_TRY(expr)                                                                               \
    do {                                                                                            \
        hipError_t _e = (expr);                                                                     \
        if (_e != hipSuccess)                                                                       \
            return fail(_e == hipErrorOutOfMemory ? ZKW_ERR_OOM : ZKW_ERR_HIP, "%s failed: %s (%s:%d)", \
                        #expr, hipGetErrorString(_e), __FILE__, __LINE__);                          \
    } while (0)

#define ZKW_TRY(expr)            \
    do {                         \
        int _rc = (expr);        \
        if (_rc != ZKW_OK) return _rc; \
    } while (0)

struct DevBuf {
    void* p = nullptr;
    size_t cap = 0;
};

struct HostStage {
    void* p = nullptr;
    size_t cap = 0;
    hipEvent_t ev = nullptr;
    bool pending = false;
};

struct zkw_ctx {
    int device = 0;
    hipStream_t own_stream = nullptr;
    hipStream_t stream = nullptr;
    int ptr_mode = ZKW_PTR_HOST;
    zkw_batch* batch = nullptr;
    bool batched() const { return batch && zkw_batch_in_fiber(batch); }
    hipError_t memset_async(void* p, int value, size_t bytes) {
        if (batched()) { zkw_batch_memset(batch, p, value, bytes); return hipSuccess; }
        return hipMemsetAsync(p, value, bytes, stream);
    }
    hipError_t copy_async(void* dst, const void* src, size_t bytes, hipMemcpyKind kind) {
        if (batched()) {
            if (kind == hipMemcpyDeviceToDevice) zkw_batch_copy_d2d(batch, dst, src, bytes);
            else if (kind == hipMemcpyHostToDevice) zkw_batch_copy_h2d(batch, dst, src, bytes);
            else if (kind == hipMemcpyDeviceToHost) zkw_batch_copy_d2h(batch, dst, src, bytes);
            else return hipErrorInvalidValue;
            return hipSuccess;
        }
        return hipMemcpyAsync(dst, src, bytes, kind, stream);
    }
    hipError_t sync_stream() {
        if (batched()) return zkw_batch_sync(batch) == ZKW_OK ? hipSuccess : hipErrorUnknown;
        if (side_stream && side_join() != ZKW_OK) return hipErrorUnknown;
        return hipStreamSynchronize(stream);
    }
    hipStream_t chain_stream = nullptr;
    hipEvent_t chain_ev_a = nullptr, chain_ev_b = nullptr;
    hipStream_t side_stream = nullptr;
    hipEvent_t side_ev_fork = nullptr, side_ev_join = nullptr;
    int side_fork(hipStream_t* out) {
        if (!side_ev_fork) {
            HIP_TRY(hipEventCreateWithFlags(&side_ev_fork, hipEventDisableTiming));
            HIP_TRY(hipEventCreateWithFlags(&side_ev_join, hipEventDisableTiming));
        }
        if (!side_stream) HIP_TRY(zkw_pool_stream_acquire(&side_stream));
        HIP_TRY(hipEventRecord(side_ev_fork, stream));
        HIP_TRY(hipStreamWaitEvent(side_stream, side_ev_fork, 0));
        *out = side_stream;
        return ZKW_OK;
    }
    int side_join() {
        if (!side_stream) return ZKW_OK;
        hipStream_t s = side_stream;
        side_stream = nullptr;
        const hipError_t e1 = hipEventRecord(side_ev_join, s);
        const hipError_t e2 = e1 == hipSuccess ? hipStreamWaitEvent(stream, side_ev_join, 0) : e1;
        if (e2 != hipSuccess) (void)hipStreamSynchronize(s);
        zkw_pool_stream_release(s);
        HIP_TRY(e2);
        return ZKW_OK;
    }
    std::atomic<long> children{0};
    std::atomic<bool> destroy_requested{false};
    std::atomic<bool> destroying{false};
    bool chain_service = false;
    int chain_tag = 0, chain_seq = 0;
    int next_chain_key() { return chain_tag ? chain_tag * 4096 + (chain_seq++ & 4095) : 0; }
    int chain_form = 0;
    int netlist_fill_form = 0;
    std::map<std::string, DevBuf> pool;
    std::map<std::string, HostStage> stages;
    bool profiling = false;
    struct ProfSpan { const char* name; hipEvent_t a, b; };
    std::vector<ProfSpan> spans;
    std::vector<hipEvent_t> free_events;
    std::map<std::string, std::pair<double, uint64_t>> prof_totals;

    hipEvent_t prof_event() {
        if (!free_events.empty()) { hipEvent_t e = free_events.back(); free_events.pop_back(); return e; }
        hipEvent_t e = nullptr;
        (void)hipEventCreate(&e);
        return e;
    }
    int prof_collect() {
        if (spans.empty()) return ZKW_OK;
        HIP_TRY(hipStreamSynchronize(stream));
        for (auto& sp : spans) {
            float ms = 0;
            if (hipEventElapsedTime(&ms, sp.a, sp.b) == hipSuccess) {
                auto& t = prof_totals[sp.name];
                t.first += ms;
                t.second += 1;
            }
            free_events.push_back(sp.a);
            free_events.push_back(sp.b);
        }
        spans.clear();
        return ZKW_OK;
    }

    int scratch(const char* name, size_t bytes, void** out) {
        DevBuf& b = pool[name];
        if (b.cap < bytes) {
            if (b.p) {
                retired_dev.push_back(b.p);
                b.p = nullptr;
                b.cap = 0;
            }
            size_t want = bytes + bytes / 8 + 256;
            HIP_TRY(dev_malloc(&b.p, want));
            b.cap = want;
        }
        *out = b.p;
        return ZKW_OK;
    }
    template <class T>
    int scratch_t(const char* name, size_t count, T** out) {
        void* p = nullptr;
        ZKW_TRY(scratch(name, count * sizeof(T) + 16, &p));
        *out = static_cast<T*>(p);
        return ZKW_OK;
    }
    template <class T>
    int upload(const char* name, const std::vector<T>& h, T** out) {
        if (batched()) {
            *out = static_cast<T*>(zkw_batch_upload(batch, h.data(), h.size() * sizeof(T), alignof(T) > 16 ? alignof(T) : 16));
            return *out ? ZKW_OK : ZKW_ERR_OOM;
        }
        ZKW_TRY(scratch_t<T>(name, h.size() ? h.size() : 1, out));
        if (h.empty()) return ZKW_OK;
        const size_t bytes = h.size() * sizeof(T);
        HostStage& st = stages[name];
        if (st.pending) {
            HIP_TRY(hipEventSynchronize(st.ev));
            st.pending = false;
        }
        if (st.cap < bytes) {
            if (st.p) retired_host.push_back(st.p);
            st.p = nullptr;
            st.cap = 0;
            HIP_TRY(pin_malloc(&st.p, bytes + bytes / 2 + 256));
            st.cap = bytes + bytes / 2 + 256;
        }
        if (!st.ev) HIP_TRY(hipEventCreateWithFlags(&st.ev, hipEventDisableTiming));
        memcpy(st.p, h.data(), bytes);
        HIP_TRY(hipMemcpyAsync(*out, st.p, bytes, hipMemcpyHostToDevice, stream));
        HIP_TRY(hipEventRecord(st.ev, stream));
        st.pending = true;
        return ZKW_OK;
    }
    template <class T>
    int in(const char* name, const T* src, size_t count, const T** out) {
        if (ptr_mode == ZKW_PTR_DEVICE || count == 0) {
            *out = src;
            return ZKW_OK;
        }
        T* d = nullptr;
        ZKW_TRY(scratch_t<T>(name, count, &d));
        HIP_TRY(copy_async(d, src, count * sizeof(T), hipMemcpyHostToDevice));
        *out = d;
        return ZKW_OK;
    }
    template <class T>
    int out(const char* name, T* dst, size_t count, T** dev) {
        if (ptr_mode == ZKW_PTR_DEVICE) {
            *dev = dst;
            return ZKW_OK;
        }
        return scratch_t<T>(name, count ? count : 1, dev);
    }
    template <class T>
    int finish_out(T* dst, const T* dev, size_t count) {
        if (ptr_mode == ZKW_PTR_DEVICE || count == 0) return ZKW_OK;
        HIP_TRY(copy_async(dst, dev, count * sizeof(T), hipMemcpyDeviceToHost));
        return ZKW_OK;
    }
    int sync_if_host() {
        if (ptr_mode == ZKW_PTR_HOST) HIP_TRY(sync_stream());
        return ZKW_OK;
    }
    void* pinned_rb = nullptr;
    size_t pinned_rb_cap = 0;
    int read_small(void* dst, const void* src, size_t bytes) {
        if (batched()) {
            zkw_batch_copy_d2h(batch, dst, src, bytes);
            return zkw_batch_sync(batch);
        }
        if (pinned_rb_cap < bytes) {
            if (pinned_rb) retired_host.push_back(pinned_rb);
            pinned_rb = nullptr;
            pinned_rb_cap = 0;
            const size_t want = bytes < 4096 ? 4096 : bytes;
            HIP_TRY(pin_malloc(&pinned_rb, want));
            pinned_rb_cap = want;
        }
        HIP_TRY(hipMemcpyAsync(pinned_rb, src, bytes, hipMemcpyDeviceToHost, stream));
        HIP_TRY(hipStreamSynchronize(stream));
        memcpy(dst, pinned_rb, bytes);
        return ZKW_OK;
    }
    std::vector<void*> retired_dev, retired_host;
};

struct Prof {
    zkw_ctx* c;
    hipEvent_t b = nullptr;
    Prof(zkw_ctx* ctx, const char* name) : c(ctx) {
        if (!c->profiling || c->batched()) return;
        hipEvent_t a = c->prof_event();
        b = c->prof_event();
        (void)hipEventRecord(a, c->stream);
        c->spans.push_back(zkw_ctx::ProfSpan{name, a, b});
    }
    ~Prof() {
        if (b) (void)hipEventRecord(b, c->stream);
    }
};

static inline int launch_check(const char* what) {
    hipError_t e = hipGetLastError();
    if (e != hipSuccess) return fail(ZKW_ERR_HIP, "launch of %s failed: %s", what, hipGetErrorString(e));
    return ZKW_OK;
}

template <auto Body, int BS>
struct Launcher {
    using S = LaunchSig<decltype(Body)>;
    template <class... A>
    static int go(zkw_ctx* ctx, const char* name, dim3 grid, size_t lds_bytes, const A&... a) {
        if (grid.x == 0 || grid.y == 0 || grid.z == 0) return ZKW_OK;
        if (ctx->batched()) {
            typename S::T t;
            S::pack(t, a...);
            zkw_batch_launch(ctx->batch, S::template desc<Body, BS>(name), grid, lds_bytes, &t);
            return ZKW_OK;
        }
        S::template single<Body, BS>(ctx->stream, grid, lds_bytes, a...);
        return launch_check(name);
    }
    static int allow_dynamic_lds(int bytes) {
        HIP_TRY(hipFuncSetAttribute(S::template single_fn<Body, BS>(), hipFuncAttributeMaxDynamicSharedMemorySize, bytes));
        HIP_TRY(hipFuncSetAttribute(S::template desc<Body, BS>("")->multi_fn, hipFuncAttributeMaxDynamicSharedMemorySize, bytes));
        return ZKW_OK;
    }
};
#define ZKW_LAUNCH(ctx, kernel, gx, bs, ...) ZKW_TRY((Launcher<&kernel, bs>::go(ctx, #kernel, dim3((unsigned)(gx)), 0, __VA_ARGS__)))
#define ZKW_LAUNCH_2D(ctx, kernel, gx, gy, bs, ...) ZKW_TRY((Launcher<&kernel, bs>::go(ctx, #kernel, dim3((unsigned)(gx), (unsigned)(gy)), 0, __VA_ARGS__)))
#define ZKW_LAUNCH_T(ctx, kernel, name, gx, bs, ...) ZKW_TRY((Launcher<&kernel, bs>::go(ctx, name, dim3((unsigned)(gx)), 0, __VA_ARGS__)))
#define ZKW_LAUNCH_D(ctx, kernel, name, grid, bs, lds, ...) ZKW_TRY((Launcher<&kernel, bs>::go(ctx, name, grid, lds, __VA_ARGS__)))

static __device__ __forceinline__ void k_zero_strip(const VB& vb, u64* __restrict__ base, size_t pitch, size_t width) {
    const size_t i = (size_t)vb.x * blockDim.x + threadIdx.x;
    if (i < width) base[(size_t)vb.y * pitch + i] = 0;
}
static inline int zero_netlist_slot(zkw_ctx* ctx, u64* trace, size_t n_rows, size_t g, size_t lookup_cols, size_t n_cols, size_t used_rows) {
    HIP_TRY(hipMemsetAsync(trace, 0, g * n_rows * sizeof(u64), ctx->stream));
    if (used_rows < n_rows) {
        ZKW_LAUNCH_2D(ctx, k_zero_strip, (unsigned)((n_rows - used_rows + 255) / 256), (unsigned)lookup_cols, 256,
                           trace + g * n_rows + used_rows, n_rows, n_rows - used_rows);
        ZKW_TRY(launch_check("k_zero_strip"));
    }
    HIP_TRY(hipMemsetAsync(trace + (g + lookup_cols) * n_rows, 0, (n_cols - g - lookup_cols) * n_rows * sizeof(u64), ctx->stream));
    return ZKW_OK;
}

static inline unsigned blocks_for(size_t n, unsigned bs) { return (unsigned)((n + bs - 1) / bs); }

void ctx_retain(zkw_ctx* ctx);
zkw_ctx* zkw_ctx_create_in_batch(int device_id, zkw_batch* b);
void zkw_ctx_leave_batch(zkw_ctx* ctx, void* stream);

void ctx_release(zkw_ctx* ctx);

struct zkw_trace {
    zkw_ctx* ctx = nullptr;
    size_t n_rows = 0, n_cols = RC_COLS, n_slots = 0;
    u64* data = nullptr;
    size_t slot_elems() const { return n_cols * n_rows; }
    std::unique_ptr<std::atomic<uint64_t>[]> slot_tag;
    u64* slot_for_write(size_t slot, uint64_t tag) const {
        slot_tag[slot].store(tag, std::memory_order_relaxed);
        return data + slot * slot_elems();
    }
    uint64_t tag_of(size_t slot) const { return slot_tag[slot].load(std::memory_order_relaxed); }
};

struct SlotClaims {
    struct Claim { const zkw_trace* t; size_t slot; uint64_t tag; };
    const zkw_trace* t;
    std::vector<Claim> pending;
    explicit SlotClaims(const zkw_trace* tr = nullptr) : t(tr) {}
    u64* claim(size_t slot, uint64_t tag, bool* clean) { return claim(t, slot, tag, clean); }
    u64* claim(const zkw_trace* tr, size_t slot, uint64_t tag, bool* clean) {
        *clean = tr->tag_of(slot) == tag;
        pending.push_back(Claim{tr, slot, tag});
        return tr->slot_for_write(slot, 0);
    }
    void commit() {
        for (auto& p : pending) p.t->slot_for_write(p.slot, p.tag);
        pending.clear();
    }
    int commit_if(int rc) {
        if (rc == ZKW_OK) commit();
        return rc;
    }
};


int dev_encode(zkw_ctx* ctx, const zkw_mem_query* q, size_t n, u64* enc);
int dev_chains(zkw_ctx* ctx, const std::vector<ChainJob>& jobs);
int dev_fs(zkw_ctx* ctx, const std::vector<FsJob>& jobs, int state_w, int n_chal);
int dev_grand_products(zkw_ctx* ctx, std::vector<GpSeg>& segs, int width, int n_reps);
int dev_log_chains(zkw_ctx* ctx, const u64* d_enc, size_t total, std::vector<LogChainJob>& jobs);
int zkw_launch_chain_full(hipStream_t st, const ChainJob* d_jobs, int n_jobs);
int zkw_launch_chain_log(hipStream_t st, const LogChainJob* d_jobs, int n_jobs);
```

### era_zkevm_test_harness_amd/native.py

```python
import ctypes as C
import os

os.environ.setdefault("GPU_MAX_HW_QUEUES", "8")

import numpy as np

_HERE = os.path.dirname(os.path.abspath(__file__))
LIB_PATH = os.environ.get("ZKW_LIB", os.path.join(_HERE, "libzkw.so"))

OK, ERR_INVALID, ERR_NO_DEVICE, ERR_HIP, ERR_OOM, ERR_CHECK_FAILED = 0, -1, -2, -3, -4, -5
PTR_HOST, PTR_DEVICE = 0, 1
(RAM_SORTED_QUERIES, RAM_UNSORTED_ENC, RAM_SORTED_ENC, RAM_UNSORTED_TAILS, RAM_SORTED_TAILS, RAM_CHALLENGES,
 RAM_LHS_Z, RAM_RHS_Z, RAM_INSTANCES, RAM_COMPACT_FORMS, RAM_PUBLIC_INPUTS, RAM_GP_CKPT) = range(12)

_vp, _sz, _u32, _u64p, _int = C.c_void_p, C.c_size_t, C.c_uint32, C.c_void_p, C.c_int
SYMBOLS = [
    ("zkw_process_init", _int, []),
    ("zkw_create", _vp, [_int]),
    ("zkw_destroy", None, [_vp]),
    ("zkw_last_error", C.c_char_p, []),
    ("zkw_set_stream", _int, [_vp, _vp]),
    ("zkw_set_chain_stream", _int, [_vp, _vp]),
    ("zkw_set_pointer_mode", _int, [_vp, _int]),
    ("zkw_synchronize", _int, [_vp]),
    ("zkw_set_chain_form", _int, [_vp, _int]),
    ("zkw_set_netlist_fill_form", _int, [_vp, _int]),
    ("zkw_set_chain_service", _int, [_vp, _int]),
    ("zkw_set_chain_tag", _int, [_vp, _int]),
    ("zkw_chain_service_expect", _int, [_int, _int]),
    ("zkw_buffer_alloc", _int, [_vp, _int, C.c_size_t, C.POINTER(C.c_void_p)]),
    ("zkw_buffer_free", None, [_int, _vp]),
    ("zkw_stream_acquire", _int, [_vp, C.POINTER(C.c_void_p)]),
    ("zkw_stream_release", None, [_vp, _vp]),
    ("zkw_trim_caches", None, []),
    ("zkw_block_linear_hasher_instance", _int, [_vp, _vp]),
    ("zkw_setup_copy_permutation", _int, [C.c_uint8, C.c_uint32, _sz, _vp, _vp]),
    ("zkw_check_copy_permutation", _int, [_vp, _vp, _sz, _vp, C.c_uint32, _vp, _vp]),
    ("zkw_ntt", _int, [_vp, _vp, _vp, _u32, _sz, _int]),
    ("zkw_lde", _int, [_vp, _vp, _u32, _sz, _u32, _vp]),
    ("zkw_merkle_tree_words", _sz, [_sz, _u32]),
    ("zkw_merkle_tree_with_cap", _int, [_vp, _vp, _sz, _sz, _sz, _u32, _vp, _vp]),
    ("zkw_setup_lookup_tables", _int, [C.c_uint8, _sz, _vp, _vp]),
    ("zkw_setup_num_columns", _int, [C.c_uint8, _vp]),
    ("zkw_setup_columns", _int, [_vp, C.c_uint8, _u32, _u32, _vp]),
    ("zkw_setup_commit", _int, [_vp, C.c_uint8, _u32, _u32, _u32, _u32, _vp]),
    ("zkw_setup_row_selectors", _int, [C.c_uint8, C.c_uint32, _sz, _vp]),
    ("zkw_vm_trace_build", _int, [_vp, _vp, _sz, _vp, _sz, _vp, _sz, C.POINTER(_vp)]),
    ("zkw_vm_trace_count", _sz, [_vp, _int]),
    ("zkw_vm_trace_ptr", _vp, [_vp, _int]),
    ("zkw_vm_trace_get", _int, [_vp, _int, _vp, _sz]),
    ("zkw_vm_trace_info", _int, [_vp, _vp]),
    ("zkw_vm_trace_streams", _int, [_vp, _vp]),
    ("zkw_vm_trace_free", None, [_vp]),
    ("zkw_recursion_queue_split", _int, [_vp, _sz, C.c_uint32, _vp, _sz, _vp]),
    ("zkw_vk_commitment", _int, [_vp, _vp, _sz, _vp]),
    ("zkw_compute_leaf_params", _int, [_vp, C.c_uint8, _vp, _vp, _sz, _vp]),
    ("zkw_leaf_vks_and_params_commitment", _int, [_vp, _vp, _vp]),
    ("zkw_create_leaf_witnesses", _int, [_vp, _vp, _vp, _sz, _vp, _vp, _vp, _vp, _vp, _sz, _vp]),
    ("zkw_create_node_witnesses", _int, [_vp, C.c_uint8, _vp, _vp, _vp, _sz, _vp, _vp, _vp, _sz, _vp]),
    ("zkw_closed_form_public_inputs", _int, [_vp, C.c_uint8, _vp, C.c_size_t, _vp, _vp]),
    ("zkw_version", C.c_char_p, []),
    ("zkw_circuit_geometry_of", _int, [C.c_uint8, _vp]),
    ("zkw_circuit_layout_of", _int, [C.c_uint8, _u32, _vp]),
    ("zkw_circuit_fill_bytes", _int, [C.c_uint8, _u32, _sz, C.POINTER(C.c_uint64), C.POINTER(C.c_uint64)]),
    ("zkw_profile_enable", _int, [_vp, _int]),
    ("zkw_profile_reset", _int, [_vp]),
    ("zkw_profile_get", _int, [_vp, C.c_char_p, C.POINTER(C.c_double), C.POINTER(C.c_uint64)]),
    ("zkw_profile_names", _int, [_vp, C.c_char_p, _sz]),
    ("zkw_encode_memory_queries", _int, [_vp, _vp, _sz, _u64p]),
    ("zkw_queue_push_chain_full", _int, [_vp, _u64p, _sz, _u64p, _u64p]),
    ("zkw_queue_push_chain_full_batch", _int, [_vp, _u64p, _u64p, _sz, _u64p, _u64p]),
    ("zkw_encode_log_queries", _int, [_vp, _vp, _sz, _vp, _u64p]),
    ("zkw_encode_decommit_queries", _int, [_vp, _vp, _sz, _u64p]),
    ("zkw_queue_push_chain_log_batch", _int, [_vp, _u64p, _u64p, _sz, _u64p, _u64p, _u64p]),
    ("zkw_queue_push_chain_log", _int, [_vp, _u64p, _sz, _u64p, _u64p, _u64p]),
    ("zkw_fs_challenges", _int, [_vp, _u64p, _u32, _u64p, _u32, _int, _int, _u64p]),
    ("zkw_grand_product_chains", _int, [_vp, _u64p, _u64p, _sz, _int, _u64p, _int, _u64p, _u64p]),
    ("zkw_ram_build_instances", _int, [_vp, _vp, _sz, _u32, _u32, C.POINTER(_vp)]),
    ("zkw_ram_build_instances_batch", _int, [_vp, _vp, _u64p, _sz, _u32, _vp, C.POINTER(_vp)]),
    ("zkw_ram_witness_num_instances", _sz, [_vp]),
    ("zkw_ram_witness_num_items", _sz, [_vp]),
    ("zkw_ram_witness_bytes", _sz, [_vp, _int]),
    ("zkw_ram_witness_device_ptr", _vp, [_vp, _int]),
    ("zkw_ram_witness_get", _int, [_vp, _int, _vp, _sz]),
    ("zkw_ram_witness_free", None, [_vp]),
    ("zkw_decommit_sorter_build", _int, [_vp, _vp, _sz, _u32, _vp, C.POINTER(_vp)]),
    ("zkw_decommit_sorter_prepare", _int, [_vp, _vp, _sz, _u32, _vp, C.POINTER(_vp)]),
    ("zkw_decommit_sorter_finish", _int, [_vp, _vp]),
    ("zkw_decommit_witness_num_instances", _sz, [_vp]),
    ("zkw_decommit_witness_num_dedup", _sz, [_vp]),
    ("zkw_decommit_witness_bytes", _sz, [_vp, _int]),
    ("zkw_decommit_witness_device_ptr", _vp, [_vp, _int]),
    ("zkw_decommit_witness_get", _int, [_vp, _int, _vp, _sz]),
    ("zkw_decommit_witness_free", None, [_vp]),
    ("zkw_events_sorter_build", _int, [_vp, _vp, _sz, _u32, _vp, C.POINTER(_vp)]),
    ("zkw_events_witness_num_instances", _sz, [_vp]),
    ("zkw_events_witness_num_results", _sz, [_vp]),
    ("zkw_events_witness_bytes", _sz, [_vp, _int]),
    ("zkw_events_witness_device_ptr", _vp, [_vp, _int]),
    ("zkw_events_witness_get", _int, [_vp, _int, _vp, _sz]),
    ("zkw_events_witness_free", None, [_vp]),
    ("zkw_log_demux_build", _int, [_vp, _vp, _sz, _u32, _vp, C.POINTER(_vp)]),
    ("zkw_demux_witness_num_instances", _sz, [_vp]),
    ("zkw_demux_witness_bytes", _sz, [_vp, _int]),
    ("zkw_demux_witness_device_ptr", _vp, [_vp, _int]),
    ("zkw_demux_witness_get", _int, [_vp, _int, _vp, _sz]),
    ("zkw_demux_witness_free", None, [_vp]),
    ("zkw_storage_sorter_build", _int, [_vp, _vp, _sz, _u32, C.POINTER(_vp)]),
    ("zkw_storage_witness_num_instances", _sz, [_vp]),
    ("zkw_storage_witness_num_results", _sz, [_vp]),
    ("zkw_storage_witness_bytes", _sz, [_vp, _int]),
    ("zkw_storage_witness_device_ptr", _vp, [_vp, _int]),
    ("zkw_storage_witness_get", _int, [_vp, _int, _vp, _sz]),
    ("zkw_storage_witness_free", None, [_vp]),
    ("zkw_decommitter_build", _int, [_vp, _vp, _u64p, _sz, _vp, _u64p, _u32, _vp, C.POINTER(_vp)]),
    ("zkw_decommitter_build_with_tails", _int, [_vp, _vp, _u64p, _sz, _vp, _u64p, _u32, _vp, _vp, C.POINTER(_vp)]),
    ("zkw_decommitter_memory_queries", _int, [_vp, _vp, _sz, _vp, _u64p, _vp]),
    ("zkw_decommitter_witness_num_instances", _sz, [_vp]),
    ("zkw_decommitter_witness_bytes", _sz, [_vp, _int]),
    ("zkw_decommitter_witness_device_ptr", _vp, [_vp, _int]),
    ("zkw_decommitter_witness_get", _int, [_vp, _int, _vp, _sz]),
    ("zkw_decommitter_witness_free", None, [_vp]),
    ("zkw_linear_keccak256", _int, [_vp, _vp, _sz, _vp]),
    ("zkw_decommit_sorter_synthesize", _int, [_vp, _vp, _sz, _sz, _vp, _sz]),
    ("zkw_decommit_sorter_check_satisfied", _int, [_vp, _vp, _sz, C.c_uint32, _vp, _vp]),
    ("zkw_events_sorter_synthesize", _int, [_vp, _vp, _sz, _sz, _vp, _sz]),
    ("zkw_events_sorter_check_satisfied", _int, [_vp, _vp, _sz, C.c_uint32, _vp, _vp]),
    ("zkw_log_demux_synthesize", _int, [_vp, _vp, _sz, _sz, _vp, _sz]),
    ("zkw_storage_sorter_synthesize", _int, [_vp, _vp, _sz, _sz, _vp, _sz]),
    ("zkw_storage_sorter_check_satisfied", _int, [_vp, _vp, _sz, C.c_uint32, _vp, _vp]),
    ("zkw_log_demux_check_satisfied", _int, [_vp, _vp, _sz, C.c_uint32, _vp, _vp]),
    ("zkw_precompile_closed_forms", _int, [_vp, _vp, _vp, _vp]),
    ("zkw_keccak_round_synthesize", _int, [_vp, _vp, _sz, _sz, _vp, _sz]),
    ("zkw_sha256_round_synthesize", _int, [_vp, _vp, _sz, _sz, _vp, _sz]),
    ("zkw_code_decommitter_synthesize", _int, [_vp, _vp, _sz, _sz, _vp, _sz]),
    ("zkw_code_decommitter_check_satisfied", _int, [_vp, _vp, _sz, C.c_uint32, _vp, _vp]),
    ("zkw_sha256_round_check_satisfied", _int, [_vp, _vp, _sz, C.c_uint32, _vp, _vp]),
    ("zkw_linear_hasher_synthesize", _int, [_vp, _vp, _sz, _vp, C.c_uint32, _vp, _sz, _vp, _vp]),
    ("zkw_linear_hasher_synthesize_batch", _int, [_vp, _vp, _vp, _sz, _vp, C.c_uint32, _vp, _sz, _vp, _vp]),
    ("zkw_linear_hasher_synthesize_batch_with_tails", _int, [_vp, _vp, _vp, _sz, _vp, _vp, C.c_uint32, _vp, _sz, _vp, _vp]),
    ("zkw_linear_hasher_check_satisfied", _int, [_vp, _vp, _sz, C.c_uint32, _vp, _vp]),
    ("zkw_keccak_round_check_satisfied", _int, [_vp, _vp, _sz, C.c_uint32, _vp, _vp]),
    ("zkw_ecrecover_synthesize", _int, [_vp, _vp, _sz, _sz, _vp, _sz]),
    ("zkw_ecrecover_synthesize_multi", _int, [_vp, _vp, _sz, _vp, _sz]),
    ("zkw_ecrecover_check_satisfied", _int, [_vp, _vp, _sz, C.c_uint32, _vp, _vp]),
    ("zkw_storage_application_build", _int, [_vp, _vp, _vp, _sz, _vp, _vp, _vp, C.c_uint64, C.c_uint32, _vp]),
    ("zkw_storage_application_witness_num_instances", _sz, [_vp]),
    ("zkw_storage_application_witness_bytes", _sz, [_vp, _int]),
    ("zkw_storage_application_witness_device_ptr", _vp, [_vp, _int]),
    ("zkw_storage_application_witness_get", _int, [_vp, _int, _vp, _sz]),
    ("zkw_storage_application_witness_free", None, [_vp]),
    ("zkw_storage_tree_create", _int, [_vp, _sz, C.POINTER(_vp)]),
    ("zkw_storage_tree_free", None, [_vp]),
    ("zkw_storage_tree_bytes_per_leaf", _sz, []),
    ("zkw_storage_tree_root", _int, [_vp, _vp]),
    ("zkw_storage_tree_next_enumeration_index", C.c_uint64, [_vp]),
    ("zkw_storage_tree_set_next_enumeration_index", _int, [_vp, C.c_uint64]),
    ("zkw_storage_tree_num_leaves", _sz, [_vp]),
    ("zkw_storage_tree_capacity", _sz, [_vp]),
    ("zkw_storage_tree_insert", _int, [_vp, _vp, _vp, _sz]),
    ("zkw_storage_tree_get_leaves", _int, [_vp, _vp, _sz, _vp, _vp, _vp]),
    ("zkw_storage_tree_answer_queries", _int, [_vp, _vp, _vp, _sz, _vp, _vp]),
    ("zkw_storage_tree_apply_queries", _int, [_vp, _vp, _sz]),
    ("zkw_storage_tree_create_witness", _int, [_vp, _vp, _vp, _vp, _vp, _sz, _vp, C.c_uint64, C.POINTER(_vp)]),
    ("zkw_storage_tree_extract_witness", _int, [_vp, _vp, _vp, _sz, C.POINTER(_vp)]),
    ("zkw_storage_tree_advance_witness", _int, [_vp, _vp, _vp, _vp, _sz, C.POINTER(_vp)]),
# ... 686 lines not shown

    def eip4844_prove(self, blobs, records, ctx=None, evaluations=False):
        ctx = ctx or self.ctx
        ptr, n, _keep = self._bytes(ctx, blobs, EIP4844_BLOB_BYTES)
        if ctx.pointer_mode == PTR_DEVICE:
            import torch

            rec = records.contiguous()
            assert rec.is_cuda and rec.element_size() == 1 and rec.numel() == n * EIP4844_RECORD.itemsize
            out = torch.empty((n, EIP4844_PROOF_RECORD.itemsize), dtype=torch.uint8, device=_keep.device)
            ev = torch.empty((n, EIP4844_EVALUATION_BYTES), dtype=torch.uint8, device=_keep.device) if evaluations else None
            _check(load().zkw_eip4844_prove(self.handle, ctx.handle, ptr, n, C.c_void_p(rec.data_ptr() if n else None), C.c_void_p(out.data_ptr() if n else None),
                                            C.c_void_p(ev.data_ptr() if evaluations and n else None)))
            return (out, ev) if evaluations else out
        rec = np.ascontiguousarray(records, dtype=EIP4844_RECORD).reshape(-1)
        assert rec.size == n
        out = np.zeros(n, EIP4844_PROOF_RECORD)
        ev = np.zeros((n, EIP4844_EVALUATION_BYTES), np.uint8) if evaluations else None
        _check(load().zkw_eip4844_prove(self.handle, ctx.handle, ptr, n, _np_ptr(rec) if n else None, _np_ptr(out) if n else None,
                                        _np_ptr(ev) if evaluations and n else None))
        return (out, ev) if evaluations else out

    def free(self):
        if self.handle:
            load().zkw_kzg_settings_free(self.handle)
            self.handle = C.c_void_p(None)

    def __del__(self):
        try:
            self.free()
        except Exception:
            pass


class PrecompileWitness:

    _DTYPES = {PRC_INSTANCES: PRECOMPILE_INSTANCE, PRC_KECCAK_ROUNDS: KECCAK_ROUND_RECORD, PRC_SHA256_ROUNDS: SHA256_ROUND_RECORD}
    _SHAPES = {PRC_MEM_ENC: (-1, 8), PRC_MEM_TAILS: (-1, 12)}

    def __init__(self, ctx):
        self.ctx = ctx
        self.handle = C.c_void_p(None)

    @property
    def num_instances(self):
        return load().zkw_precompile_witness_num_instances(self.handle)

    @property
    def num_rounds(self):
        return load().zkw_precompile_witness_num_rounds(self.handle)

    def get(self, what):
        lib = load()
        nbytes = lib.zkw_precompile_witness_bytes(self.handle, what)
        dt = self._DTYPES.get(what, np.dtype("<u8"))
        out = np.zeros(nbytes // dt.itemsize, dt)
        if nbytes:
            _check(lib.zkw_precompile_witness_get(self.handle, what, _np_ptr(out), nbytes))
        shape = self._SHAPES.get(what)
        return out.reshape(shape) if shape else out

    def free(self):
        if self.handle:
            load().zkw_precompile_witness_free(self.handle)
            self.handle = C.c_void_p(None)

    def __del__(self):
        try:
            self.free()
        except Exception:
            pass



class DecommitterWitness:

    _DTYPES = {DCM_MEM_QUERIES: MEM_QUERY, DCM_INSTANCES: DECOMMITTER_INSTANCE, DCM_ROUND_STATES: np.dtype("<u4"),
               DCM_SHA256_ROUNDS: SHA256_ROUND_RECORD}
    _SHAPES = {DCM_MEM_ENC: (-1, 8), DCM_MEM_TAILS: (-1, 12), DCM_ROUND_STATES: (-1, 8)}

    def __init__(self, ctx):
        self.ctx = ctx
        self.handle = C.c_void_p(None)

    @property
    def num_instances(self):
        return load().zkw_decommitter_witness_num_instances(self.handle)

    def get(self, what):
        lib = load()
        nbytes = lib.zkw_decommitter_witness_bytes(self.handle, what)
        dt = self._DTYPES.get(what, np.dtype("<u8"))
        out = np.zeros(nbytes // dt.itemsize, dt)
        if nbytes:
            _check(lib.zkw_decommitter_witness_get(self.handle, what, _np_ptr(out), nbytes))
        shape = self._SHAPES.get(what)
        return out.reshape(shape) if shape else out

    def free(self):
        if self.handle:
            load().zkw_decommitter_witness_free(self.handle)
            self.handle = C.c_void_p(None)

    def __del__(self):
        try:
            self.free()
        except Exception:
            pass


class DecommitWitness:

    _DTYPES = {DEC_SORTED_QUERIES: DECOMMIT_QUERY, DEC_DEDUP_QUERIES: DECOMMIT_QUERY, DEC_INSTANCES: DECOMMIT_INSTANCE}
    _SHAPES = {DEC_UNSORTED_ENC: (-1, 8), DEC_SORTED_ENC: (-1, 8), DEC_UNSORTED_TAILS: (-1, 12), DEC_SORTED_TAILS: (-1, 12),
               DEC_DEDUP_TAILS: (-1, 12), DEC_CHALLENGES: (2, 9), DEC_LHS_Z: (2, -1), DEC_RHS_Z: (2, -1),
               DEC_COMPACT_FORMS: (-1, 18), DEC_PUBLIC_INPUTS: (-1, 4)}

    def __init__(self, ctx):
        self.ctx = ctx
        self.handle = C.c_void_p(None)

    @property
    def num_instances(self):
        return load().zkw_decommit_witness_num_instances(self.handle)

    @property
    def num_dedup(self):
        return load().zkw_decommit_witness_num_dedup(self.handle)

    def get(self, what):
        lib = load()
        nbytes = lib.zkw_decommit_witness_bytes(self.handle, what)
        dt = self._DTYPES.get(what, np.dtype("<u8"))
        out = np.zeros(nbytes // dt.itemsize, dt)
        if nbytes:
            _check(lib.zkw_decommit_witness_get(self.handle, what, _np_ptr(out), nbytes))
        shape = self._SHAPES.get(what)
        return out.reshape(shape) if shape else out

    def free(self):
        if self.handle:
            load().zkw_decommit_witness_free(self.handle)
            self.handle = C.c_void_p(None)

    def __del__(self):
        try:
            self.free()
        except Exception:
            pass


class RamWitness:

    _DTYPES = {RAM_SORTED_QUERIES: MEM_QUERY, RAM_INSTANCES: RAM_INSTANCE}

    def __init__(self, ctx):
        self.ctx = ctx
        self.handle = C.c_void_p(None)

    @property
    def num_instances(self):
        return load().zkw_ram_witness_num_instances(self.handle)

    @property
    def num_items(self):
        return load().zkw_ram_witness_num_items(self.handle)

    def device_ptr(self, what):
        return load().zkw_ram_witness_device_ptr(self.handle, what)

    def nbytes(self, what):
        return load().zkw_ram_witness_bytes(self.handle, what)

    def get(self, what):
        lib = load()
        nbytes = lib.zkw_ram_witness_bytes(self.handle, what)
        dt = self._DTYPES.get(what, np.dtype("<u8"))
        out = np.zeros(nbytes // dt.itemsize, dt)
        mode = self.ctx.pointer_mode
        self.ctx.set_pointer_mode(PTR_HOST)
        try:
            _check(lib.zkw_ram_witness_get(self.handle, what, _np_ptr(out), nbytes))
        finally:
            self.ctx.set_pointer_mode(mode)
        t = self.num_items
        shape = {RAM_UNSORTED_ENC: (t, 8), RAM_SORTED_ENC: (t, 8), RAM_UNSORTED_TAILS: (t, 12),
                 RAM_SORTED_TAILS: (t, 12), RAM_CHALLENGES: (-1, 2, 9), RAM_COMPACT_FORMS: (-1, 18),
                 RAM_PUBLIC_INPUTS: (-1, 4), RAM_GP_CKPT: (self.num_instances, -1, 4)}.get(what)
        return out.reshape(shape) if shape else out

    def free(self):
        if self.handle:
            load().zkw_ram_witness_free(self.handle)
            self.handle = C.c_void_p(None)

    def __del__(self):
        try:
            self.free()
        except Exception:
            pass


class Trace:

    def __init__(self, ctx, n_rows, n_slots=1, n_cols=None):
        self.ctx = ctx
        self.handle = C.c_void_p(None)
        if n_cols is None:
            _check(load().zkw_trace_create(ctx.handle, n_rows, n_slots, C.byref(self.handle)))
        else:
            _check(load().zkw_trace_create_with_columns(ctx.handle, n_rows, n_cols, n_slots, C.byref(self.handle)))
        self.n_rows, self.n_slots = n_rows, n_slots
        self.n_cols = load().zkw_trace_num_cols(self.handle)

    def device_ptr(self, slot=0):
        return load().zkw_trace_device_ptr(self.handle, slot)

    def get(self, slot=0, first_col=0, n_cols=None):
        n_cols = self.n_cols - first_col if n_cols is None else n_cols
        out = np.zeros((n_cols, self.n_rows), np.uint64)
        mode = self.ctx.pointer_mode
        self.ctx.set_pointer_mode(PTR_HOST)
        try:
            _check(load().zkw_trace_get(self.handle, slot, first_col, n_cols, _np_ptr(out)))
        finally:
            self.ctx.set_pointer_mode(mode)
        return out

    def free(self):
        if self.handle:
            load().zkw_trace_free(self.handle)
            self.handle = C.c_void_p(None)

    def __del__(self):
        try:
            self.free()
        except Exception:
            pass


class Context:

    def __init__(self, device_id=0):
        lib = load()
        self.handle = lib.zkw_create(device_id)
        if not self.handle:
            raise ZkwError(ERR_NO_DEVICE, lib.zkw_last_error().decode())
        self.pointer_mode = PTR_HOST

    def close(self):
        if self.handle:
            load().zkw_destroy(self.handle)
            self.handle = None

    def __del__(self):
        try:
            self.close()
        except Exception:
            pass

    def set_chain_stream(self, hip_stream):
        _check(load().zkw_set_chain_stream(self.handle, C.c_void_p(hip_stream)))

    def set_pointer_mode(self, mode):
        _check(load().zkw_set_pointer_mode(self.handle, mode))
        self.pointer_mode = mode

    def set_stream(self, stream_handle):
        h = C.c_void_p(-1) if stream_handle is None else C.c_void_p(stream_handle)
        _check(load().zkw_set_stream(self.handle, h))

    def set_chain_form(self, lanes_per_state):
        _check(load().zkw_set_chain_form(self.handle, lanes_per_state))

    def set_netlist_fill_form(self, form):
        _check(load().zkw_set_netlist_fill_form(self.handle, form))

    def synchronize(self):
        _check(load().zkw_synchronize(self.handle))

    def profile_enable(self, on=True):
        _check(load().zkw_profile_enable(self.handle, 1 if on else 0))

    def profile_reset(self):
        _check(load().zkw_profile_reset(self.handle))

    def profile(self):
        lib = load()
        buf = C.create_string_buffer(4096)
        _check(lib.zkw_profile_names(self.handle, buf, 4096))
        out = {}
        for name in filter(None, buf.value.decode().split(",")):
            ms, cnt = C.c_double(0), C.c_uint64(0)
            _check(lib.zkw_profile_get(self.handle, name.encode(), C.byref(ms), C.byref(cnt)))
            out[name] = (ms.value, cnt.value)
        return out

    def encode_memory_queries(self, q):
        q = np.ascontiguousarray(q, dtype=MEM_QUERY)
        enc = np.zeros((q.size, 8), np.uint64)
        _check(load().zkw_encode_memory_queries(self.handle, _np_ptr(q), q.size, _np_ptr(enc)))
        return enc

    def queue_push_chain_full(self, enc, tail_in=None):
        enc = _u64(enc)
        n = enc.shape[0]
        tails = np.zeros((n, 12), np.uint64)
        tin = None if tail_in is None else _np_ptr(_u64(tail_in))
        _check(load().zkw_queue_push_chain_full(self.handle, _np_ptr(enc), n, tin, _np_ptr(tails)))
        return tails

    def queue_push_chain_full_batch(self, enc, offsets, tails_in=None):
        enc = _u64(enc)
        offsets = _u64(offsets)
        tails = np.zeros((enc.shape[0], 12), np.uint64)
        tin = None if tails_in is None else _np_ptr(_u64(tails_in))
        _check(load().zkw_queue_push_chain_full_batch(self.handle, _np_ptr(enc), _np_ptr(offsets), offsets.size - 1,
                                                      tin, _np_ptr(tails)))
        return tails

    def encode_log_queries(self, q, ext_ts=None):
        q = np.ascontiguousarray(q, dtype=LOG_QUERY)
        enc = np.zeros((q.size, 20), np.uint64)
        e = None if ext_ts is None else np.ascontiguousarray(ext_ts, dtype=np.uint32)
        _check(load().zkw_encode_log_queries(self.handle, _np_ptr(q), q.size, None if e is None else _np_ptr(e),
                                             _np_ptr(enc)))
        return enc

    def encode_decommit_queries(self, q):
        q = np.ascontiguousarray(q, dtype=DECOMMIT_QUERY)
        enc = np.zeros((q.size, 8), np.uint64)
        _check(load().zkw_encode_decommit_queries(self.handle, _np_ptr(q), q.size, _np_ptr(enc)))
        return enc

    def queue_push_chain_log(self, enc, offsets=None, tails_in=None):
        enc = _u64(enc)
        n = enc.shape[0]
        offsets = np.array([0, n], np.uint64) if offsets is None else _u64(offsets)
        old_t, new_t = np.zeros((n, 4), np.uint64), np.zeros((n, 4), np.uint64)
        tin = None if tails_in is None else _np_ptr(_u64(tails_in))
        _check(load().zkw_queue_push_chain_log_batch(self.handle, _np_ptr(enc), _np_ptr(offsets), offsets.size - 1,
# ... 1134 lines not shown
```

### include/zkw.h

```cpp
#ifndef ZKW_H
#define ZKW_H
#include "zkw_types.h"

#ifdef __cplusplus
extern "C" {
#endif

typedef struct zkw_ctx zkw_ctx;
typedef struct zkw_ram_witness zkw_ram_witness;
typedef struct zkw_trace zkw_trace;

enum {
    ZKW_OK = 0,
    ZKW_ERR_INVALID = -1,
    ZKW_ERR_NO_DEVICE = -2,
    ZKW_ERR_HIP = -3,
    ZKW_ERR_OOM = -4,
    ZKW_ERR_CHECK_FAILED = -5
};

enum { ZKW_PTR_HOST = 0, ZKW_PTR_DEVICE = 1 };

int zkw_process_init(void);
zkw_ctx *zkw_create(int device_id);
void zkw_destroy(zkw_ctx *ctx);
const char *zkw_last_error(void);
#define ZKW_STREAM_OWN ((void *)(intptr_t)-1)
int zkw_set_stream(zkw_ctx *ctx, void *hip_stream);
int zkw_set_chain_stream(zkw_ctx *ctx, void *hip_stream);
int zkw_set_pointer_mode(zkw_ctx *ctx, int mode);
int zkw_synchronize(zkw_ctx *ctx);
int zkw_set_chain_form(zkw_ctx *ctx, int lanes_per_state);
int zkw_set_netlist_fill_form(zkw_ctx *ctx, int form);
int zkw_set_chain_service(zkw_ctx *ctx, int on);
int zkw_set_chain_tag(zkw_ctx *ctx, int tag);
int zkw_chain_service_expect(int device_id, int delta);
int zkw_buffer_alloc(zkw_ctx *ctx, int pinned_host, size_t bytes, void **out);
void zkw_buffer_free(int pinned_host, void *p);
int zkw_stream_acquire(zkw_ctx *ctx, void **hip_stream);
void zkw_stream_release(zkw_ctx *ctx, void *hip_stream);
void zkw_trim_caches(void);
const char *zkw_version(void);

typedef struct zkw_circuit_geometry {
    uint32_t num_columns_under_copy_permutation;
    uint32_t num_witness_columns;
    uint32_t num_constant_columns;
    uint32_t max_allowed_constraint_degree;
    uint32_t lookup_width;
    uint32_t lookup_repetitions;
    uint32_t capacity;
    uint32_t trace_len_log2;
    uint64_t size_hint_variables;
} zkw_circuit_geometry;
int zkw_circuit_geometry_of(uint8_t circuit_type, zkw_circuit_geometry *out);

typedef struct zkw_circuit_layout {
    uint32_t synthesizable;
    uint32_t fits;
    uint32_t capacity;
    uint32_t num_columns;
    uint32_t rows_per_cycle;
    uint32_t total_table_rows;
    uint64_t region_stride;
    uint64_t rows_used;
    uint64_t nop_rows;
    uint64_t trace_len;
    uint32_t public_input_column[4];
    uint64_t public_input_row[4];
    uint64_t queue_first_row;
    uint32_t queue_rows_per_cycle;
    uint32_t ec_rows_per_cycle;
    uint64_t ec_first_row;
    uint64_t closed_form_first_row;
    uint32_t closed_form_rows;
    uint32_t closed_form_header_rows;
} zkw_circuit_layout;
int zkw_circuit_layout_of(uint8_t circuit_type, uint32_t capacity, zkw_circuit_layout *out);
int zkw_circuit_fill_bytes(uint8_t circuit_type, uint32_t capacity, size_t n_rows, uint64_t *warm, uint64_t *cold);
#define ZKW_ROW_HAS_GATES 0x40
#define ZKW_ROW_HEADER 0x80
#define ZKW_ROW_BOUNDARY 0xC0
#define ZKW_ROW_QUEUE_BOUNDARY 0xE0
#define ZKW_ROW_QUEUE_ENCODING 0xE1
#define ZKW_ROW_QUEUE_POSEIDON2 0xE2
#define ZKW_ROW_CLOSED_FORM_WORDS 0xE4
#define ZKW_ROW_CLOSED_FORM_POSEIDON2 0xE5
#define ZKW_ROW_EC_GATES 0xF0
#define ZKW_ROW_EC_XOR8 0xF1
#define ZKW_ROW_EC_FIXED_BASE 0xF2
#define ZKW_ROW_EC_MUL 0x04
#define ZKW_ROW_PADDING 0xFF
int zkw_setup_row_selectors(uint8_t circuit_type, uint32_t capacity, size_t n_rows, uint8_t *out);
int zkw_setup_copy_permutation(uint8_t circuit_type, uint32_t capacity, size_t n_rows, uint64_t *sigma, uint32_t *n_columns);
int zkw_check_copy_permutation(zkw_ctx *ctx, const zkw_trace *t, size_t slot, const uint64_t *sigma, uint32_t n_columns,
                               uint64_t *n_violations, uint64_t *first_bad);

int zkw_ntt(zkw_ctx *ctx, const uint64_t *in, uint64_t *out, uint32_t log_n, size_t n_cols, int inverse);
int zkw_lde(zkw_ctx *ctx, const uint64_t *values, uint32_t log_n, size_t n_cols, uint32_t lde_factor, uint64_t *out);
size_t zkw_merkle_tree_words(size_t n_leaves, uint32_t cap_size);
int zkw_merkle_tree_with_cap(zkw_ctx *ctx, const uint64_t *leaf_cols, size_t n_sets, size_t n_cols, size_t n, uint32_t cap_size,
                             uint64_t *cap, uint64_t *tree);
int zkw_setup_lookup_tables(uint8_t circuit_type, size_t n_rows, uint64_t *cols, uint32_t *n_columns);
int zkw_setup_num_columns(uint8_t circuit_type, uint32_t *n_columns);
int zkw_setup_columns(zkw_ctx *ctx, uint8_t circuit_type, uint32_t capacity, uint32_t log_n, uint64_t *columns);
int zkw_setup_commit(zkw_ctx *ctx, uint8_t circuit_type, uint32_t capacity, uint32_t log_n, uint32_t lde_factor, uint32_t cap_size,
                     uint64_t *cap);

int zkw_profile_enable(zkw_ctx *ctx, int on);
int zkw_profile_reset(zkw_ctx *ctx);
int zkw_profile_get(zkw_ctx *ctx, const char *kernel, double *total_ms, uint64_t *launches);
int zkw_profile_names(zkw_ctx *ctx, char *buf, size_t buf_bytes);

int zkw_encode_memory_queries(zkw_ctx *ctx, const zkw_mem_query *q, size_t n, uint64_t *enc);

int zkw_queue_push_chain_full(zkw_ctx *ctx, const uint64_t *enc , size_t n,
                              const uint64_t tail_in[12], uint64_t *tails );
int zkw_queue_push_chain_full_batch(zkw_ctx *ctx, const uint64_t *enc, const uint64_t *offsets,
                                    size_t n_queues, const uint64_t *tails_in, uint64_t *tails);

int zkw_encode_log_queries(zkw_ctx *ctx, const zkw_log_query *q, size_t n, const uint32_t *ext_ts, uint64_t *enc);
int zkw_encode_decommit_queries(zkw_ctx *ctx, const zkw_decommit_query *q, size_t n, uint64_t *enc);

int zkw_queue_push_chain_log_batch(zkw_ctx *ctx, const uint64_t *enc, const uint64_t *offsets, size_t n_queues,
                                   const uint64_t *tails_in, uint64_t *old_tails, uint64_t *new_tails);
int zkw_queue_push_chain_log(zkw_ctx *ctx, const uint64_t *enc, size_t n, const uint64_t tail_in[4],
                             uint64_t *old_tails, uint64_t *new_tails);

int zkw_fs_challenges(zkw_ctx *ctx, const uint64_t *tail_u, uint32_t len_u, const uint64_t *tail_s,
                      uint32_t len_s, int state_w, int n_chal, uint64_t *out);

int zkw_grand_product_chains(zkw_ctx *ctx, const uint64_t *lhs, const uint64_t *rhs, size_t n, int width,
                             const uint64_t *challenges, int n_reps, uint64_t *lhs_z, uint64_t *rhs_z);

int zkw_ram_build_instances(zkw_ctx *ctx, const zkw_mem_query *q, size_t n, uint32_t capacity,
                            uint32_t num_non_deterministic_heap_queries, zkw_ram_witness **out);
int zkw_ram_build_instances_batch(zkw_ctx *ctx, const zkw_mem_query *q, const uint64_t *block_offsets,
                                  size_t n_blocks, uint32_t capacity, const uint32_t *n_nondet,
                                  zkw_ram_witness **out);

enum {
    ZKW_RAM_SORTED_QUERIES = 0,
    ZKW_RAM_UNSORTED_ENC = 1,
    ZKW_RAM_SORTED_ENC = 2,
    ZKW_RAM_UNSORTED_TAILS = 3,
    ZKW_RAM_SORTED_TAILS = 4,
    ZKW_RAM_CHALLENGES = 5,
    ZKW_RAM_LHS_Z = 6,
    ZKW_RAM_RHS_Z = 7,
    ZKW_RAM_INSTANCES = 8,
    ZKW_RAM_COMPACT_FORMS = 9,
    ZKW_RAM_PUBLIC_INPUTS = 10,
    ZKW_RAM_GP_CKPT = 11
};
size_t zkw_ram_witness_num_instances(const zkw_ram_witness *w);
size_t zkw_ram_witness_num_items(const zkw_ram_witness *w);
size_t zkw_ram_witness_bytes(const zkw_ram_witness *w, int what);
const void *zkw_ram_witness_device_ptr(const zkw_ram_witness *w, int what);
int zkw_ram_witness_get(const zkw_ram_witness *w, int what, void *dst, size_t dst_bytes);
void zkw_ram_witness_free(zkw_ram_witness *w);

typedef struct zkw_decommit_witness zkw_decommit_witness;
int zkw_decommit_sorter_build(zkw_ctx *ctx, const zkw_decommit_query *q, size_t n, uint32_t capacity,
                              const zkw_queue_state12 *dedup_in, zkw_decommit_witness **out);
int zkw_decommit_sorter_prepare(zkw_ctx *ctx, const zkw_decommit_query *q, size_t n, uint32_t capacity,
                                const zkw_queue_state12 *dedup_in, zkw_decommit_witness **out);
int zkw_decommit_sorter_finish(zkw_ctx *ctx, zkw_decommit_witness *w);
enum {
    ZKW_DEC_SORTED_QUERIES = 0,
    ZKW_DEC_UNSORTED_ENC = 1,
    ZKW_DEC_SORTED_ENC = 2,
    ZKW_DEC_UNSORTED_TAILS = 3,
    ZKW_DEC_SORTED_TAILS = 4,
    ZKW_DEC_DEDUP_QUERIES = 5,
    ZKW_DEC_DEDUP_TAILS = 6,
    ZKW_DEC_CHALLENGES = 7,
    ZKW_DEC_LHS_Z = 8,
    ZKW_DEC_RHS_Z = 9,
    ZKW_DEC_INSTANCES = 10,
    ZKW_DEC_COMPACT_FORMS = 11,
    ZKW_DEC_PUBLIC_INPUTS = 12
};
size_t zkw_decommit_witness_num_instances(const zkw_decommit_witness *w);
size_t zkw_decommit_witness_num_dedup(const zkw_decommit_witness *w);
size_t zkw_decommit_witness_bytes(const zkw_decommit_witness *w, int what);
const void *zkw_decommit_witness_device_ptr(const zkw_decommit_witness *w, int what);
int zkw_decommit_witness_get(const zkw_decommit_witness *w, int what, void *dst, size_t dst_bytes);
void zkw_decommit_witness_free(zkw_decommit_witness *w);

typedef struct zkw_events_witness zkw_events_witness;
int zkw_events_sorter_build(zkw_ctx *ctx, const zkw_log_query *q, size_t n, uint32_t capacity,
                            const zkw_queue_state4 *result_in, zkw_events_witness **out);
enum {
    ZKW_EVT_SORTED_QUERIES = 0,
    ZKW_EVT_UNSORTED_ENC = 1,
    ZKW_EVT_SORTED_ENC = 2,
    ZKW_EVT_UNSORTED_OLD_TAILS = 3,
    ZKW_EVT_UNSORTED_NEW_TAILS = 4,
    ZKW_EVT_SORTED_OLD_TAILS = 5,
    ZKW_EVT_SORTED_NEW_TAILS = 6,
    ZKW_EVT_RESULT_QUERIES = 7,
    ZKW_EVT_RESULT_NEW_TAILS = 8,
    ZKW_EVT_CHALLENGES = 9,
    ZKW_EVT_LHS_Z = 10,
    ZKW_EVT_RHS_Z = 11,
    ZKW_EVT_INSTANCES = 12,
    ZKW_EVT_COMPACT_FORMS = 13,
    ZKW_EVT_PUBLIC_INPUTS = 14
};
size_t zkw_events_witness_num_instances(const zkw_events_witness *w);
size_t zkw_events_witness_num_results(const zkw_events_witness *w);
size_t zkw_events_witness_bytes(const zkw_events_witness *w, int what);
const void *zkw_events_witness_device_ptr(const zkw_events_witness *w, int what);
int zkw_events_witness_get(const zkw_events_witness *w, int what, void *dst, size_t dst_bytes);
void zkw_events_witness_free(zkw_events_witness *w);

typedef struct zkw_demux_witness zkw_demux_witness;
int zkw_log_demux_build(zkw_ctx *ctx, const zkw_log_query *q, size_t n, uint32_t capacity,
                        const zkw_demux_params *params, zkw_demux_witness **out);
enum {
    ZKW_DMX_IN_ENC = 0,
    ZKW_DMX_IN_OLD_TAILS = 1,
    ZKW_DMX_IN_NEW_TAILS = 2,
    ZKW_DMX_OUT_QUERIES = 3,
    ZKW_DMX_OUT_ENC = 4,
    ZKW_DMX_OUT_OLD_TAILS = 5,
    ZKW_DMX_OUT_NEW_TAILS = 6,
    ZKW_DMX_OUT_OFFSETS = 7,
    ZKW_DMX_INSTANCES = 8,
    ZKW_DMX_COMPACT_FORMS = 9,
    ZKW_DMX_PUBLIC_INPUTS = 10
};
size_t zkw_demux_witness_num_instances(const zkw_demux_witness *w);
size_t zkw_demux_witness_bytes(const zkw_demux_witness *w, int what);
const void *zkw_demux_witness_device_ptr(const zkw_demux_witness *w, int what);
int zkw_demux_witness_get(const zkw_demux_witness *w, int what, void *dst, size_t dst_bytes);
void zkw_demux_witness_free(zkw_demux_witness *w);

typedef struct zkw_storage_witness zkw_storage_witness;
int zkw_storage_sorter_build(zkw_ctx *ctx, const zkw_log_query *q, size_t n, uint32_t capacity,
                             zkw_storage_witness **out);
enum {
    ZKW_STO_SORTED_QUERIES = 0,
    ZKW_STO_SORTED_EXT_TS = 1,
    ZKW_STO_UNSORTED_ENC = 2,
    ZKW_STO_LHS_ENC = 3,
    ZKW_STO_SORTED_ENC = 4,
    ZKW_STO_UNSORTED_OLD_TAILS = 5,
    ZKW_STO_UNSORTED_NEW_TAILS = 6,
    ZKW_STO_SORTED_OLD_TAILS = 7,
    ZKW_STO_SORTED_NEW_TAILS = 8,
    ZKW_STO_RESULT_QUERIES = 9,
    ZKW_STO_RESULT_NEW_TAILS = 10,
    ZKW_STO_CHALLENGES = 11,
    ZKW_STO_LHS_Z = 12,
    ZKW_STO_RHS_Z = 13,
    ZKW_STO_INSTANCES = 14,
    ZKW_STO_COMPACT_FORMS = 15,
    ZKW_STO_PUBLIC_INPUTS = 16
};
size_t zkw_storage_witness_num_instances(const zkw_storage_witness *w);
size_t zkw_storage_witness_num_results(const zkw_storage_witness *w);
size_t zkw_storage_witness_bytes(const zkw_storage_witness *w, int what);
const void *zkw_storage_witness_device_ptr(const zkw_storage_witness *w, int what);
int zkw_storage_witness_get(const zkw_storage_witness *w, int what, void *dst, size_t dst_bytes);
void zkw_storage_witness_free(zkw_storage_witness *w);

typedef struct zkw_decommitter_witness zkw_decommitter_witness;
int zkw_decommitter_build(zkw_ctx *ctx, const zkw_decommit_query *requests, const uint64_t *dedup_tails,
                          size_t n_requests, const uint32_t *words, const uint64_t *word_offsets, uint32_t capacity,
                          const zkw_queue_state12 *mem_in, zkw_decommitter_witness **out);
int zkw_decommitter_build_with_tails(zkw_ctx *ctx, const zkw_decommit_query *requests, const uint64_t *dedup_tails,
                                     size_t n_requests, const uint32_t *words, const uint64_t *word_offsets,
                                     uint32_t capacity, const zkw_queue_state12 *mem_in, const uint64_t *given_mem_tails,
                                     zkw_decommitter_witness **out);
int zkw_decommitter_memory_queries(zkw_ctx *ctx, const zkw_decommit_query *requests, size_t n_requests,
                                   const uint32_t *words, const uint64_t *word_offsets, zkw_mem_query *out);
enum {
    ZKW_DCM_MEM_QUERIES = 0,
    ZKW_DCM_MEM_ENC = 1,
    ZKW_DCM_MEM_TAILS = 2,
    ZKW_DCM_ROUND_STATES = 3,
    ZKW_DCM_INSTANCES = 4,
    ZKW_DCM_SHA256_ROUNDS = 5
};
size_t zkw_decommitter_witness_num_instances(const zkw_decommitter_witness *w);
size_t zkw_decommitter_witness_bytes(const zkw_decommitter_witness *w, int what);
const void *zkw_decommitter_witness_device_ptr(const zkw_decommitter_witness *w, int what);
int zkw_decommitter_witness_get(const zkw_decommitter_witness *w, int what, void *dst, size_t dst_bytes);
void zkw_decommitter_witness_free(zkw_decommitter_witness *w);

int zkw_decommit_sorter_synthesize(zkw_ctx *ctx, const zkw_decommit_witness *w, size_t first_instance, size_t n_instances,
                                   zkw_trace *t, size_t first_slot);
int zkw_decommit_sorter_check_satisfied(zkw_ctx *ctx, const zkw_trace *t, size_t slot, uint32_t capacity,
                                        uint64_t *n_violations, uint64_t *first_bad);

int zkw_events_sorter_synthesize(zkw_ctx *ctx, const zkw_events_witness *w, size_t first_instance, size_t n_instances,
                                 zkw_trace *t, size_t first_slot);
int zkw_events_sorter_check_satisfied(zkw_ctx *ctx, const zkw_trace *t, size_t slot, uint32_t capacity,
                                      uint64_t *n_violations, uint64_t *first_bad);

int zkw_log_demux_synthesize(zkw_ctx *ctx, const zkw_demux_witness *w, size_t first_instance, size_t n_instances,
                             zkw_trace *t, size_t first_slot);
int zkw_log_demux_check_satisfied(zkw_ctx *ctx, const zkw_trace *t, size_t slot, uint32_t capacity,
                                  uint64_t *n_violations, uint64_t *first_bad);

// ... 340 lines not shown
```

Measured before the change: 3423.

## Cut RAM synth launches: precompute nondet prefix, merge poseidon sides, inline job table

The per-tile nondeterministic-query prefix is now computed once during instance building (k_ram_count_nondet), which removes the nd_tiles and nd_scan kernels from the synth path. The two Poseidon fill kernels become one launch using grid z for the side. For small non-batched runs the job table is passed inline in kernel arguments, so no upload is needed. Multiplicity-column writes move into fill_D, and the tail kernel plus the histogram memset are skipped when slots are already clean. Together these cut per-call launches and uploads, at the cost of an extra per-instance buffer, more register pressure in the merged kernel, and new dirty-state tracking.

```diff
diff --git a/era_zkevm_test_harness_amd/csrc/ram_circuit_kernels.cuh b/era_zkevm_test_harness_amd/csrc/ram_circuit_kernels.cuh
--- a/era_zkevm_test_harness_amd/csrc/ram_circuit_kernels.cuh
+++ b/era_zkevm_test_harness_amd/csrc/ram_circuit_kernels.cuh
@@ -20,11 +20,22 @@
     const u64* gp_ckpt;
     u64* trace;
     u32* hist;
-    u32* nd_tiles;
+    const u32* nd_tiles;
     const u64* public_input;
     const zkw_ram_instance* first_inst;
     u32 tail_clean;
 };
+
+constexpr int RC_INLINE_JOBS = 32;
+struct SynthJobsRef {
+    const SynthJob* p;
+    __device__ __forceinline__ const SynthJob& operator[](unsigned k) const { return p[k]; }
+};
+struct SynthJobsInline {
+    SynthJob j[RC_INLINE_JOBS];
+    __device__ __forceinline__ const SynthJob& operator[](unsigned k) const { return j[k]; }
+};
+static_assert(sizeof(SynthJobsInline) <= 3968, "the inline job table and the scalar arguments share the 4 KB of kernel arguments");
 
 constexpr int ROW_SLOTS[RC_NUM_ROW_TYPES] = RC_ROW_NUM_SLOTS_INIT;
 constexpr int ROW_LOOKUPS[RC_NUM_ROW_TYPES] = RC_ROW_NUM_LOOKUPS_INIT;
@@ -241,23 +252,12 @@
 }
 
 template <int SIDE>
-static __device__ __forceinline__ void k_ram_fill_poseidon(const VB& vb, const SynthJob* __restrict__ jobs, u32 capacity,
-                                                          size_t n_rows) {
-    __shared__ u32 sh_hist[256];
-    for (int t = threadIdx.x; t < 256; t += blockDim.x) sh_hist[t] = 0;
-    __syncthreads();
-    const SynthJob job = jobs[vb.y];
-    const u32 i = vb.x * blockDim.x + threadIdx.x;
+__device__ __forceinline__ void ram_poseidon_prologue(const SynthJob& job, u32 i, u32 capacity, size_t n_rows, size_t row, bool can_pop,
+                                                      u64 s[12], u32* sh_hist) {
     u64* trace = job.trace;
-    const zkw_ram_instance* in = job.inst;
-    const size_t first = in->first_item, m = in->num_items;
-    const bool can_pop = i < capacity && i < m;
-    const size_t row = (size_t)(SIDE == 0 ? RC_ROW_PU : RC_ROW_PS) * RC_REGION_STRIDE(capacity) + i;
+    const size_t first = job.inst->first_item;
     zkw_mem_query q;
     memset(&q, 0, sizeof q);
-    u64 s[12];
-#pragma unroll
-    for (int k = 0; k < 8; k++) s[k] = 0;
     if (can_pop) {
         load_query(job.sorted_q + first + i, q);
         if (SIDE == 0) encode_raw_query(load_raw_query(job.unsorted_q + first + i), s); else encode_mem_query(q, s);
@@ -284,10 +284,32 @@
             hist_bytes(sh_hist, q.timestamp); hist_bytes(sh_hist, q.page); hist_bytes(sh_hist, q.value[4]);
         }
         if (!job.tail_clean) for (int c = RC_G + 12; c < RC_G + RC_L; c++) TR(c, row) = 0;
+    }
+}
+
+template <class J>
+static __device__ __forceinline__ void k_ram_fill_poseidon(const VB& vb, const J& jobs, u32 capacity, size_t n_rows) {
+    __shared__ u32 sh_hist[256];
+    for (int t = threadIdx.x; t < 256; t += blockDim.x) sh_hist[t] = 0;
+    __syncthreads();
+    const SynthJob job = jobs[vb.y];
+    const u32 side = vb.z;
+    const u32 i = vb.x * blockDim.x + threadIdx.x;
+    u64* trace = job.trace;
+    const zkw_ram_instance* in = job.inst;
+    const size_t first = in->first_item, m = in->num_items;
+    const bool can_pop = i < capacity && i < m;
+    const size_t row = (size_t)(side == 0 ? RC_ROW_PU : RC_ROW_PS) * RC_REGION_STRIDE(capacity) + i;
+    u64 s[12];
+#pragma unroll
+    for (int k = 0; k < 8; k++) s[k] = 0;
+    if (side == 0) ram_poseidon_prologue<0>(job, i, capacity, n_rows, row, can_pop, s, sh_hist);
+    else ram_poseidon_prologue<1>(job, i, capacity, n_rows, row, can_pop, s, sh_hist);
+    if (i < capacity) {
         __builtin_amdgcn_sched_barrier(0);
         const RegsIn ri = regs_in(in);
-        const u64* caps = SIDE == 0 ? job.unsorted_caps : job.sorted_caps;
-        const u64* prev_cap = i == 0 ? (SIDE == 0 ? ri.uh : ri.sh) + 8 : caps + 4 * (first + (i - 1 < m ? i - 1 : m - 1));
+        const u64* caps = side == 0 ? job.unsorted_caps : job.sorted_caps;
+        const u64* prev_cap = i == 0 ? (side == 0 ? ri.uh : ri.sh) + 8 : caps + 4 * (first + (i - 1 < m ? i - 1 : m - 1));
 #pragma unroll
         for (int k = 0; k < 4; k++) s[8 + k] = prev_cap[k];
         fill_flattened_poseidon(trace, n_rows, row, s);
@@ -301,40 +323,8 @@
     return can_pop && q.timestamp == 0 && q.page == RC_HEAP_PAGE && q.rw_flag && !q.value_is_pointer;
 }
 
-static __device__ __forceinline__ void k_ram_nd_tiles(const VB& vb, const SynthJob* __restrict__ jobs, u32 capacity) {
-    __shared__ u32 sh[4];
-    const SynthJob job = jobs[vb.y];
-    const u32 i = vb.x * blockDim.x + threadIdx.x;
-    const zkw_ram_instance* in = job.inst;
-    bool f = false;
-    if (i < capacity && i < in->num_items) {
-        zkw_mem_query q;
-        load_query(job.sorted_q + in->first_item + i, q);
-        f = nd_flag(true, q);
-    }
-    u32 cnt = __popcll(__ballot(f));
-    if ((threadIdx.x & 63) == 0) sh[threadIdx.x >> 6] = cnt;
-    __syncthreads();
-    if (threadIdx.x == 0) job.nd_tiles[vb.x] = sh[0] + sh[1] + sh[2] + sh[3];
-}
-static __device__ __forceinline__ void k_ram_nd_scan(const VB& vb, const SynthJob* __restrict__ jobs, int n_jobs, u32 n_tiles) {
-    u32* t = jobs[vb.x].nd_tiles;
-    const int lane = threadIdx.x;
-    u32 acc = 0;
-    for (u32 base = 0; base < n_tiles; base += 64) {
-        const u32 k = base + lane;
-        const u32 v = k < n_tiles ? t[k] : 0;
-        u32 incl = v;
-        for (int off = 1; off < 64; off <<= 1) {
-            const u32 up = __shfl_up(incl, off);
-            if (lane >= off) incl += up;
-        }
-        if (k < n_tiles) t[k] = acc + incl - v;
-        acc += __shfl(incl, 63);
-    }
-}
-
-static __device__ __forceinline__ void k_ram_fill_C(const VB& vb, const SynthJob* __restrict__ jobs, u32 capacity, size_t n_rows) {
+template <class J>
+static __device__ __forceinline__ void k_ram_fill_C(const VB& vb, const J& jobs, u32 capacity, size_t n_rows) {
     __shared__ u32 sh_hist[256];
     __shared__ u32 sh_wave[4];
     sh_hist[threadIdx.x] = 0;
@@ -429,10 +419,20 @@
 }
 
 __device__ __forceinline__ void ram_boundary_block(const SynthJob& job, u32 capacity, size_t n_rows);
+constexpr int RC_CF_LOOKUP_CELLS = 24;
+__device__ __forceinline__ void ram_fill_multiplicities(const SynthJob& job, u32 capacity, size_t n_rows) {
+    const u32 r = threadIdx.x;
+    u64 v = job.hist[r];
+    job.hist[r] = 0;
+    if (r == 0) v += (u64)RC_L * n_rows - (u64)LOOKUPS_PER_CYCLE * capacity - RC_CF_LOOKUP_CELLS;
+    if (r < n_rows) job.trace[(size_t)RC_MULT_COL * n_rows + r] = v;
+}
 constexpr int RC_D_TILES = 4;
-static __device__ __forceinline__ void k_ram_fill_D(const VB& vb, const SynthJob* __restrict__ jobs, u32 n_jobs, u32 n_tiles, u32 capacity, size_t n_rows) {
+template <class J>
+static __device__ __forceinline__ void k_ram_fill_D(const VB& vb, const J& jobs, u32 n_jobs, u32 n_tiles, u32 capacity, size_t n_rows) {
     if (vb.x < n_jobs) {
         __builtin_amdgcn_s_setprio(3);
+        ram_fill_multiplicities(jobs[vb.x], capacity, n_rows);
         ram_boundary_block(jobs[vb.x], capacity, n_rows);
         return;
     }
@@ -491,16 +491,16 @@
 
 constexpr int TAIL_CHUNKS = 8;
 constexpr int RC_BOUNDARY_ROWS = RC_NUM_ROW_TYPES - RC_ROWS_PER_CYCLE;
-constexpr int RC_CF_LOOKUP_CELLS = 24;
 static_assert(RC_BOUNDARY_ROWS % 2 == 0, "the tail's 16-byte stores start below the boundary rows");
-static __device__ __forceinline__ void k_ram_fill_tail(const VB& vb, const SynthJob* __restrict__ jobs, u32 capacity, size_t n_rows) {
+template <class J>
+static __device__ __forceinline__ void k_ram_fill_tail(const VB& vb, const J& jobs, u32 capacity, size_t n_rows) {
     constexpr u32 PER_JOB = (RC_G + RC_L + 1) * TAIL_CHUNKS;
     const u32 bid = vb.x % PER_JOB;
     const SynthJob& job = jobs[vb.x / PER_JOB];
+    if (job.tail_clean) return;
     u64* trace = job.trace;
     const int col = bid / TAIL_CHUNKS, ch = bid % TAIL_CHUNKS;
     if (col < RC_G + RC_L) {
-        if (job.tail_clean) return;
         const size_t bnd = (size_t)RC_BOUNDARY_ROW(capacity) + RC_BOUNDARY_ROWS;
         const size_t n_pairs = (n_rows - bnd) / 2;
         const size_t per = (n_pairs + TAIL_CHUNKS - 1) / TAIL_CHUNKS, lo = ch * per, hi = lo + per < n_pairs ? lo + per : n_pairs;
@@ -511,14 +511,7 @@
     }
     u64* m = trace + (size_t)RC_MULT_COL * n_rows;
     const size_t per = (n_rows + TAIL_CHUNKS - 1) / TAIL_CHUNKS, lo = ch * per, hi = lo + per < n_rows ? lo + per : n_rows;
-    for (size_t r = lo + threadIdx.x; r < (job.tail_clean && hi > 256 ? (lo < 256 ? 256 : lo) : hi); r += 256) {
-        u64 v = 0;
-        if (r < 256) {
-            v = job.hist[r];
-            if (r == 0) v += (u64)RC_L * n_rows - (u64)LOOKUPS_PER_CYCLE * capacity - RC_CF_LOOKUP_CELLS;
-        }
-        m[r] = v;
-    }
+    for (size_t r = (lo < 256 ? 256 : lo) + threadIdx.x; r < hi; r += 256) m[r] = 0;
 }
 
 static __constant__ rc_link c_links[RC_NUM_LINKS] = RC_LINKS_INIT;
diff --git a/era_zkevm_test_harness_amd/csrc/ram_kernels.cuh b/era_zkevm_test_harness_amd/csrc/ram_kernels.cuh
--- a/era_zkevm_test_harness_amd/csrc/ram_kernels.cuh
+++ b/era_zkevm_test_harness_amd/csrc/ram_kernels.cuh
@@ -462,6 +462,7 @@
     zkw_ram_instance* instances;
     u32* nondet_prefix;
     u64* gp_ckpt;
+    u32* nd_prefix;
     u64 n;
     u32 capacity;
     u32 num_nondet_heap_queries;
@@ -474,18 +475,31 @@
 static __device__ __forceinline__ void k_ram_count_nondet(const VB& vb, const RamBlock* __restrict__ blocks) {
     const RamBlock b = blocks[vb.y];
     const u64 n_inst = (b.n + b.capacity - 1) / b.capacity;
-    __shared__ u32 sh[4];
+    const u32 n_tiles = (b.capacity + 255) / 256;
+    __shared__ u32 sh[2][2][4];
     for (u64 inst = vb.x; inst < n_inst; inst += vb.nx) {
         const u64 lo = inst * b.capacity, hi = lo + b.capacity < b.n ? lo + b.capacity : b.n;
-        u32 cnt = 0;
-        for (u64 i = lo + threadIdx.x; i < hi; i += blockDim.x) {
-            const zkw_mem_query* q = b.sorted_q + b.sorted_perm[i];
-            cnt += (q->rw_flag && q->timestamp == 0 && q->page == ZKW_BOOTLOADER_HEAP_PAGE) ? 1u : 0u;
-        }
-        for (int d = 32; d > 0; d >>= 1) cnt += __shfl_down(cnt, d, 64);
-        if ((threadIdx.x & 63) == 0) sh[threadIdx.x >> 6] = cnt;
-        __syncthreads();
-        if (threadIdx.x == 0) b.nondet_prefix[inst] = sh[0] + sh[1] + sh[2] + sh[3];
+        u32 cnt = 0, before = 0;
+        for (u32 t = 0; t < n_tiles; t++) {
+            const u64 i = lo + 256 * (u64)t + threadIdx.x;
+            bool f = false, fc = false;
+            if (i < hi) {
+                const zkw_mem_query* q = b.sorted_q + b.sorted_perm[i];
+                f = q->rw_flag && q->timestamp == 0 && q->page == ZKW_BOOTLOADER_HEAP_PAGE;
+                fc = f && !q->value_is_pointer;
+            }
+            const u32 c = __popcll(__ballot(f)), cc = __popcll(__ballot(fc));
+            if ((threadIdx.x & 63) == 0) { sh[t & 1][0][threadIdx.x >> 6] = c; sh[t & 1][1][threadIdx.x >> 6] = cc; }
+            __syncthreads();
+            if (threadIdx.x == 0) {
+                const u32* s0 = sh[t & 1][0];
+                const u32* s1 = sh[t & 1][1];
+                b.nd_prefix[inst * n_tiles + t] = before;
+                cnt += s0[0] + s0[1] + s0[2] + s0[3];
+                before += s1[0] + s1[1] + s1[2] + s1[3];
+            }
+        }
+        if (threadIdx.x == 0) b.nondet_prefix[inst] = cnt;
         __syncthreads();
     }
 }
diff --git a/era_zkevm_test_harness_amd/csrc/zkw_api.hip b/era_zkevm_test_harness_amd/csrc/zkw_api.hip
--- a/era_zkevm_test_harness_amd/csrc/zkw_api.hip
+++ b/era_zkevm_test_harness_amd/csrc/zkw_api.hip
@@ -959,6 +959,7 @@
     bool z_valid = false;
     u64 *zbuf_l = nullptr, *zbuf_r = nullptr;
     u64* gp_ckpt = nullptr;
+    u32* nd_prefix = nullptr;
     zkw_mem_query* sq_win = nullptr;
     size_t zcap = 0, sqcap = 0;
     zkw_ram_instance* instances = nullptr;
@@ -968,7 +969,7 @@
     void release() {
         void* ptrs[] = {sorted_q, perm, owned_q, unsorted_enc, sorted_enc, unsorted_caps, sorted_caps, unsorted_marks, sorted_marks,
                         unsorted_tails, sorted_tails, challenges,
-                        lhs_z,    rhs_z,        instances,  nondet_counts, compact_forms, public_inputs, zbuf_l, zbuf_r, sq_win, gp_ckpt};
+                        lhs_z,    rhs_z,        instances,  nondet_counts, compact_forms, public_inputs, zbuf_l, zbuf_r, sq_win, gp_ckpt, nd_prefix};
         for (void* p : ptrs)
             if (p) dev_free(p);
         sorted_q = nullptr;
@@ -983,6 +984,7 @@
         z_valid = false;
         zbuf_l = zbuf_r = nullptr;
         gp_ckpt = nullptr;
+        nd_prefix = nullptr;
         sq_win = nullptr;
         zcap = sqcap = 0;
         instances = nullptr;
@@ -993,6 +995,7 @@
 
 extern "C" void zkw_ram_witness_free(zkw_ram_witness* w);
 static inline size_t ram_gp_groups(uint32_t capacity) { return ((size_t)capacity + 63) / 64; }
+static inline size_t ram_nd_tiles(uint32_t capacity) { return ((size_t)capacity + 255) / 256; }
 static int ram_alloc(zkw_ram_witness* w, size_t n_blocks) {
     const size_t t = w->total, ni = w->n_instances;
     HIP_TRY(dev_malloc((void**)&w->perm, (t + 1) * sizeof(u32)));
@@ -1013,6 +1016,7 @@
         HIP_TRY(dev_malloc((void**)&w->sq_win, (w->sqcap + 1) * sizeof(zkw_mem_query)));
     }
     HIP_TRY(dev_malloc((void**)&w->gp_ckpt, (ni * ram_gp_groups(w->capacity) + 1) * 4 * sizeof(u64)));
+    HIP_TRY(dev_malloc((void**)&w->nd_prefix, (ni * ram_nd_tiles(w->capacity) + 1) * sizeof(u32)));
     HIP_TRY(dev_malloc((void**)&w->instances, (ni + 1) * sizeof(zkw_ram_instance)));
     HIP_TRY(dev_malloc((void**)&w->nondet_counts, (ni + 1) * sizeof(u32)));
     HIP_TRY(dev_malloc((void**)&w->compact_forms, (ni + 1) * COMPACT_FORM_LEN * sizeof(u64)));
@@ -1211,6 +1215,7 @@
                                       w->instances + w->inst_offsets[b],
                                       w->nondet_counts + w->inst_offsets[b],
                                       w->gp_ckpt + 4 * ram_gp_groups(w->capacity) * w->inst_offsets[b],
+                                      w->nd_prefix + ram_nd_tiles(w->capacity) * w->inst_offsets[b],
                                       n,
                                       w->capacity,
                                       n_nondet ? n_nondet[b] : 0u};
@@ -1382,6 +1387,7 @@
         case ZKW_RAM_COMPACT_FORMS: *bytes = w->n_instances * COMPACT_FORM_LEN * 8; p = w->compact_forms; break;
         case ZKW_RAM_PUBLIC_INPUTS: *bytes = w->n_instances * 32; p = w->public_inputs; break;
         case ZKW_RAM_GP_CKPT: *bytes = w->n_instances * ram_gp_groups(w->capacity) * 32; p = w->gp_ckpt; break;
+        case ZKW_RAM_ND_PREFIX: *bytes = w->n_instances * ram_nd_tiles(w->capacity) * sizeof(u32); p = w->nd_prefix; break;
         default: *bytes = 0; st = ZKW_ERR_INVALID; break;
     }
 #undef RAM_LAZY
@@ -1514,18 +1520,25 @@
     ZKW_TRY(launch_check("k_gather_encode"));
     const u32 rstride = (u32)RC_REGION_STRIDE(capacity);
     const u32 n_tiles = (rstride + 255) / 256;
-    u32 *d_hist = nullptr, *d_nd = nullptr;
-    ZKW_TRY(ctx->scratch_t<u32>("synth_hist", n_instances * 256, &d_hist));
-    ZKW_TRY(ctx->scratch_t<u32>("synth_nd", n_instances * n_tiles, &d_nd));
-    HIP_TRY(ctx->memset_async(d_hist, 0, n_instances * 256 * sizeof(u32)));
+    u32* d_hist = nullptr;
+    {
+        const DevBuf& hb = ctx->pool["synth_hist"];
+        const void* had = hb.p;
+        ZKW_TRY(ctx->scratch_t<u32>("synth_hist", n_instances * 256, &d_hist));
+        if (hb.p != had || ctx->synth_hist_dirty) HIP_TRY(ctx->memset_async(hb.p, 0, hb.cap));
+        ctx->synth_hist_dirty = true;
+    }
     SlotClaims claims(t);
-    std::vector<SynthJob> jobs(n_instances);
+    const bool inline_jobs = n_instances <= (size_t)RC_INLINE_JOBS && !ctx->batched();
+    SynthJobsInline tab;
+    std::vector<SynthJob> jobs(inline_jobs ? 0 : n_instances);
+    bool all_clean = true;
     size_t b = b_first;
     for (size_t k = 0; k < n_instances; k++) {
         const size_t idx = first_instance + k;
         while (b + 1 < n_blocks && w->inst_offsets[b + 1] <= idx) b++;
         const size_t lo = w->offsets[b];
-        SynthJob& j = jobs[k];
+        SynthJob& j = inline_jobs ? tab.j[k] : jobs[k];
         j.inst = w->instances + idx;
         j.sorted_q = w->sq_win + (lo - z_base);
         j.unsorted_q = w->unsorted_q + lo;
@@ -1541,31 +1554,39 @@
             bool clean = false;
             j.trace = claims.claim(slot, tag, &clean);
             j.tail_clean = clean;
+            all_clean = all_clean && clean;
         }
         j.hist = d_hist + 256 * k;
-        j.nd_tiles = d_nd + (size_t)n_tiles * k;
+        j.nd_tiles = w->nd_prefix + (size_t)n_tiles * idx;
         j.public_input = w->public_inputs + 4 * idx;
         j.first_inst = w->instances + w->inst_offsets[b];
     }
-    SynthJob* d_jobs = nullptr;
-    ZKW_TRY(ctx->upload("synth_jobs", jobs, &d_jobs));
+    SynthJobsRef ref{nullptr};
+    if (!inline_jobs) {
+        SynthJob* d_jobs = nullptr;
+        ZKW_TRY(ctx->upload("synth_jobs", jobs, &d_jobs));
+        ref.p = d_jobs;
+    } else {
+        for (size_t k = n_instances; k < (size_t)RC_INLINE_JOBS; k++) tab.j[k] = tab.j[0];
+    }
+#define SYNTH_LAUNCH(kernel, name, grid, bs, ...)                                                                                  \
+    do {                                                                                                                           \
+        if (inline_jobs) {                                                                                                         \
+            LaunchSig<decltype(&kernel<SynthJobsInline>)>::template single<&kernel<SynthJobsInline>, bs>(ctx->stream, grid, 0, tab, __VA_ARGS__); \
+            ZKW_TRY(launch_check(name));                                                                                           \
+        } else {                                                                                                                   \
+            ZKW_LAUNCH_D(ctx, (kernel<SynthJobsRef>), name, grid, bs, 0, ref, __VA_ARGS__);                                        \
+        }                                                                                                                          \
+    } while (0)
     const unsigned nj = (unsigned)n_instances;
-    const dim3 g64((rstride + 63) / 64, nj), g256(n_tiles, nj);
-    { Prof _p(ctx, "k_ram_nd_tiles"); ZKW_LAUNCH_D(ctx, (k_ram_nd_tiles), "k_ram_nd_tiles", g256, 256, 0, d_jobs, capacity); }
-    ZKW_TRY(launch_check("k_ram_nd_tiles"));
-    { Prof _p(ctx, "k_ram_nd_scan"); ZKW_LAUNCH(ctx, k_ram_nd_scan, nj, 64, d_jobs, (int)nj, n_tiles); }
-    ZKW_TRY(launch_check("k_ram_nd_scan"));
-    { Prof _p(ctx, "k_ram_fill_poseidon"); ZKW_LAUNCH_D(ctx, (k_ram_fill_poseidon<0>), "k_ram_fill_poseidon", g64, 64, 0, d_jobs, capacity, n_rows); }
-    ZKW_TRY(launch_check("k_ram_fill_poseidon<0>"));
-    { Prof _p(ctx, "k_ram_fill_poseidon"); ZKW_LAUNCH_D(ctx, (k_ram_fill_poseidon<1>), "k_ram_fill_poseidon", g64, 64, 0, d_jobs, capacity, n_rows); }
-    ZKW_TRY(launch_check("k_ram_fill_poseidon<1>"));
-    { Prof _p(ctx, "k_ram_fill_C"); ZKW_LAUNCH_D(ctx, (k_ram_fill_C), "k_ram_fill_C", g256, 256, 0, d_jobs, capacity, n_rows); }
-    ZKW_TRY(launch_check("k_ram_fill_C"));
+    const dim3 g64x2((rstride + 63) / 64, nj, 2), g256(n_tiles, nj);
+    { Prof _p(ctx, "k_ram_fill_C"); SYNTH_LAUNCH(k_ram_fill_C, "k_ram_fill_C", g256, 256, capacity, n_rows); }
+    { Prof _p(ctx, "k_ram_fill_poseidon", 2); SYNTH_LAUNCH(k_ram_fill_poseidon, "k_ram_fill_poseidon", g64x2, 64, capacity, n_rows); }
     { Prof _p(ctx, "k_ram_fill_D"); const unsigned d_tiles = (unsigned)((rstride + RC_D_TILES * 256 - 1) / (RC_D_TILES * 256));
-      ZKW_LAUNCH(ctx, k_ram_fill_D, nj * (d_tiles + 1), 256, d_jobs, nj, d_tiles, capacity, n_rows); }
-    ZKW_TRY(launch_check("k_ram_fill_D"));
-    { Prof _p(ctx, "k_ram_fill_tail"); ZKW_LAUNCH(ctx, k_ram_fill_tail, nj * ((RC_G + RC_L + 1) * TAIL_CHUNKS), 256, d_jobs, capacity, n_rows); }
-    ZKW_TRY(launch_check("k_ram_fill_tail"));
+      SYNTH_LAUNCH(k_ram_fill_D, "k_ram_fill_D", dim3(nj * (d_tiles + 1)), 256, nj, d_tiles, capacity, n_rows); }
+    ctx->synth_hist_dirty = false;
+    if (!all_clean) { Prof _p(ctx, "k_ram_fill_tail"); SYNTH_LAUNCH(k_ram_fill_tail, "k_ram_fill_tail", dim3(nj * ((RC_G + RC_L + 1) * TAIL_CHUNKS)), 256, capacity, n_rows); }
+#undef SYNTH_LAUNCH
     return claims.commit_if(ctx->sync_if_host());
 }
 
diff --git a/era_zkevm_test_harness_amd/csrc/zkw_ctx.h b/era_zkevm_test_harness_amd/csrc/zkw_ctx.h
--- a/era_zkevm_test_harness_amd/csrc/zkw_ctx.h
+++ b/era_zkevm_test_harness_amd/csrc/zkw_ctx.h
@@ -125,9 +125,10 @@
     int chain_form = 0;
     int netlist_fill_form = 0;
     std::map<std::string, DevBuf> pool;
+    bool synth_hist_dirty = false;
     std::map<std::string, HostStage> stages;
     bool profiling = false;
-    struct ProfSpan { const char* name; hipEvent_t a, b; };
+    struct ProfSpan { const char* name; hipEvent_t a, b; unsigned weight; };
     std::vector<ProfSpan> spans;
     std::vector<hipEvent_t> free_events;
     std::map<std::string, std::pair<double, uint64_t>> prof_totals;
@@ -146,7 +147,7 @@
             if (hipEventElapsedTime(&ms, sp.a, sp.b) == hipSuccess) {
                 auto& t = prof_totals[sp.name];
                 t.first += ms;
-                t.second += 1;
+                t.second += sp.weight;
             }
             free_events.push_back(sp.a);
             free_events.push_back(sp.b);
@@ -261,12 +262,12 @@
 struct Prof {
     zkw_ctx* c;
     hipEvent_t b = nullptr;
-    Prof(zkw_ctx* ctx, const char* name) : c(ctx) {
+    Prof(zkw_ctx* ctx, const char* name, unsigned weight = 1) : c(ctx) {
         if (!c->profiling || c->batched()) return;
         hipEvent_t a = c->prof_event();
         b = c->prof_event();
         (void)hipEventRecord(a, c->stream);
-        c->spans.push_back(zkw_ctx::ProfSpan{name, a, b});
+        c->spans.push_back(zkw_ctx::ProfSpan{name, a, b, weight});
     }
     ~Prof() {
         if (b) (void)hipEventRecord(b, c->stream);
diff --git a/era_zkevm_test_harness_amd/native.py b/era_zkevm_test_harness_amd/native.py
--- a/era_zkevm_test_harness_amd/native.py
+++ b/era_zkevm_test_harness_amd/native.py
@@ -11,7 +11,7 @@
 OK, ERR_INVALID, ERR_NO_DEVICE, ERR_HIP, ERR_OOM, ERR_CHECK_FAILED = 0, -1, -2, -3, -4, -5
 PTR_HOST, PTR_DEVICE = 0, 1
 (RAM_SORTED_QUERIES, RAM_UNSORTED_ENC, RAM_SORTED_ENC, RAM_UNSORTED_TAILS, RAM_SORTED_TAILS, RAM_CHALLENGES,
- RAM_LHS_Z, RAM_RHS_Z, RAM_INSTANCES, RAM_COMPACT_FORMS, RAM_PUBLIC_INPUTS, RAM_GP_CKPT) = range(12)
+ RAM_LHS_Z, RAM_RHS_Z, RAM_INSTANCES, RAM_COMPACT_FORMS, RAM_PUBLIC_INPUTS, RAM_GP_CKPT, RAM_ND_PREFIX) = range(13)
 
 _vp, _sz, _u32, _u64p, _int = C.c_void_p, C.c_size_t, C.c_uint32, C.c_void_p, C.c_int
 SYMBOLS = [
@@ -1004,7 +1004,7 @@
 
 class RamWitness:
 
-    _DTYPES = {RAM_SORTED_QUERIES: MEM_QUERY, RAM_INSTANCES: RAM_INSTANCE}
+    _DTYPES = {RAM_SORTED_QUERIES: MEM_QUERY, RAM_INSTANCES: RAM_INSTANCE, RAM_ND_PREFIX: np.dtype("<u4")}
 
     def __init__(self, ctx):
         self.ctx = ctx
@@ -1038,7 +1038,8 @@
         t = self.num_items
         shape = {RAM_UNSORTED_ENC: (t, 8), RAM_SORTED_ENC: (t, 8), RAM_UNSORTED_TAILS: (t, 12),
                  RAM_SORTED_TAILS: (t, 12), RAM_CHALLENGES: (-1, 2, 9), RAM_COMPACT_FORMS: (-1, 18),
-                 RAM_PUBLIC_INPUTS: (-1, 4), RAM_GP_CKPT: (self.num_instances, -1, 4)}.get(what)
+                 RAM_PUBLIC_INPUTS: (-1, 4), RAM_GP_CKPT: (self.num_instances, -1, 4),
+                 RAM_ND_PREFIX: (self.num_instances, -1)}.get(what)
         return out.reshape(shape) if shape else out
 
     def free(self):
diff --git a/include/zkw.h b/include/zkw.h
--- a/include/zkw.h
+++ b/include/zkw.h
@@ -151,7 +151,8 @@
     ZKW_RAM_INSTANCES = 8,
     ZKW_RAM_COMPACT_FORMS = 9,
     ZKW_RAM_PUBLIC_INPUTS = 10,
-    ZKW_RAM_GP_CKPT = 11
+    ZKW_RAM_GP_CKPT = 11,
+    ZKW_RAM_ND_PREFIX = 12
 };
 size_t zkw_ram_witness_num_instances(const zkw_ram_witness *w);
 size_t zkw_ram_witness_num_items(const zkw_ram_witness *w);
```

New measurement: 3509, median of 6. 2.5% higher.
